# panthuncia/BasicRenderer

Measured on AMD Instinct MI355X. Metric: shaded Mpixels/s @4K (vis-buffer+resolve), higher is better.
Workload: dtype f32; 1 GPU; bistro-class procedural frame, 3840x2160, 1 directional + 256 point lights, 22669824 instanced tris, 2017 instances (2614016 in 150 meshes), LOD DAGs from the library's cluster-LOD builder, relief slope 1.5; pixels_per_gpu=8294400, visible_clusters_rank0=10118, occlusion_culling=True, visible_clusters_phase2_rank0=0, meshlets_tested_rank0=26713, partition=single GPU, frames_in_flight=3

## Files before the change

basicrenderer_amd/csrc/brmi_api.hip:

```cpp
#include <hip/hip_runtime.h>

#include <algorithm>
#include <cmath>
#include <cstdarg>
#include <cstddef>
#include <cstdio>
#include <cstdlib>
#include <cstring>

#include "brmi_device.h"
#include "brmi_internal.h"

namespace brmi {

__global__ void k_debug_arith(const float* a, const float* b, float* outDiv, float* outSqrt, uint32_t* outHalf, uint32_t n) {
    const uint32_t i = blockIdx.x * blockDim.x + threadIdx.x;
    if (i >= n) return;
    outDiv[i] = a[i] / b[i];
    outSqrt[i] = sqrtf(fabsf(a[i]));
    outHalf[i] = f32_to_f16_bits(a[i]);
}

__global__ void k_debug_arith_in_range(const float* a, float* outRcp, float* outSqrt, float* outNorm, uint32_t n) {
    const uint32_t i = blockIdx.x * blockDim.x + threadIdx.x;
// ... 81 lines not shown
    w.pageTotal = take(16);
    w.lightHitMasks = take((uint64_t)p->numLightClusters * ((std::max(1u, p->scene.lightCount) + 63u) / 64u) * 8);
    p->binsX = (c.width + 255) / 256; p->binsY = (c.height + 15) / 16;
    w.binCounts = take((uint64_t)p->binsX * p->binsY * 4 * BRMI_BIN_COUNT_STRIDE);
    w.binRecords = take((uint64_t)p->binsX * p->binsY * p->binCapacity * 64);
    w.binOverflow = take((uint64_t)CNT_STRIPE_COUNT * p->binOverflowPerStripe * 64);
    p->binItemCapacity = p->binsX * p->binsY * std::max(1u, (p->binCapacity + 31u) / 32u > 256u ? 256u : (p->binCapacity + 31u) / 32u);
    p->binItemCapacity = std::min<uint32_t>(p->binItemCapacity, 1u << 22);
    p->binScratchTiles = (uint32_t)std::max(0l, tuning("bin_scratch_tiles", p->binScratchTiles));
    w.binPlan = take((uint64_t)(16 + 3 * p->binsX * p->binsY) * 4);
    w.binItems = take((uint64_t)p->binItemCapacity * 4);
    w.binScratch = take((uint64_t)std::max(1u, p->binScratchTiles) * 4096 * 8);
    w.clusterSetup = take((uint64_t)c.maxVisibleClusters * sizeof(ClusterSetup));
    p->resolveCapacity = (uint32_t)std::min<uint64_t>((uint64_t)c.maxVisibleClusters, 1ull << 20) * BRMI_MESHLET_MAX_TRIS;
    if (const long v = tuning("resolve_capacity", 0)) p->resolveCapacity = (uint32_t)std::max(1l, v);
    w.resolveVerts = take((uint64_t)p->resolveCapacity * sizeof(ResolveVertex));
    w.resolveTris = take((uint64_t)p->resolveCapacity * sizeof(ResolveTriangle));
    w.shadeTables = take(((uint64_t)2 * c.width + 2 * c.height + 64) * 4);
    w.matWords = take((uint64_t)std::max(1u, p->scene.materialCount) * sizeof(MaterialWords));
    w.layerUniform = take(sizeof(LayerUniform));
    w.frameConst = take(4 * 64);
    w.frameSnapshot = take(sizeof(FrameSnapshot));
    w.matConst = take((uint64_t)std::max(1u, p->scene.openpbrMaterialCount) * sizeof(MatConst));
    w.objConst = take((uint64_t)std::max(1u, p->scene.perObjectCount) * OBJ_CONST_FLOATS * 4);
    p->deferredStripeCapacity = (uint32_t)((((c.dynamicBand ? p->paddedPixels : p->bandPixelCount) / 4096 + CNT_STRIPE_COUNT) / CNT_STRIPE_COUNT) * 4096);
    w.deferredPixels = take((uint64_t)3 * CNT_STRIPE_COUNT * p->deferredStripeCapacity * 4);
    w.lutF = take((uint64_t)(32768 + 1024 + 1024 + 32 + 256) * 4);
    w.shadeRows = take((uint64_t)std::max(1u, p->scene.openpbrMaterialCount) * 256 * 512);
    w.shadeAvgs = take((uint64_t)std::max(1u, p->scene.openpbrMaterialCount) * 256 * 8);
    w.ggxQuads = take(256 * 48);
    w.shadeLights = take((uint64_t)std::max(1u, p->scene.lightCount) * 64);
    w.clusterList = take((uint64_t)p->numLightClusters * 8);
    w.listEntries = take((uint64_t)p->lightPagePool * BRMI_LIGHTS_PER_PAGE * 4 + 256);
    w.listRecords = take((uint64_t)p->lightPagePool * BRMI_LIGHTS_PER_PAGE * 64 + 4096);
    const bool uvs = p->tables.hasTextures || p->tables.hasAlphaTest || p->tables.hasVertexColors;
    w.clusterUv = take(uvs ? (uint64_t)c.maxVisibleClusters * 32 : 16);
    w.resolveColors = take(p->tables.hasVertexColors ? (uint64_t)p->resolveCapacity * 4 : 16);
    w.resolveUVs = take(p->tables.hasTextures ? (uint64_t)p->resolveCapacity * 8 * p->tables.uvSets : 16);
    w.binAlpha = take(p->tables.hasAlphaTest ? (uint64_t)p->binsX * p->binsY * p->binCapacity * 48 : 16);
    w.overflowAlpha = take(p->tables.hasAlphaTest ? (uint64_t)CNT_STRIPE_COUNT * p->binOverflowPerStripe * 48 : 16);
    w.alphaMats = take(p->tables.hasAlphaTest ? (uint64_t)std::max(1u, p->scene.materialCount) * 128 : 16);
    w.meshletBoxes = take((uint64_t)std::max(1u, p->tables.totalBoxes) * sizeof(MeshletBox));
    w.pageBoxBase = take((uint64_t)std::max<size_t>(1, p->tables.pageBoxBase.size()) * 4);
    w.pageRefs = take((uint64_t)std::max<size_t>(1, p->tables.pageRefs.size()) * sizeof(PageRef));
    w.drawList = take(p->holdEnabled ? (uint64_t)c.maxVisibleClusters * 4 : 16);
    w.generalList = take(p->leanMinClusters != 0u ? (uint64_t)c.maxVisibleClusters * 4 : 16);
    w.bigQueue = take(p->leanMinClusters != 0u ? (uint64_t)p->leanQueue * 96 : 16);
    w.bigRuns = take(p->leanMinClusters != 0u ? (uint64_t)p->leanQueue * 8 : 16);
    w.heldRecords = take(p->holdEnabled ? (uint64_t)c.maxVisibleClusters * sizeof(HeldRecord) : 16);
    w.lateList = take(p->holdEnabled ? (uint64_t)c.maxVisibleClusters * 4 : 16);
    w.wideQueue = take((uint64_t)std::max(1u, p->wideCapacity) * 96);
    w.wideAlpha = take(p->tables.hasAlphaTest ? (uint64_t)std::max(1u, p->wideCapacity) * 48 : 16);
    w.total = off;
    p->resNeed[BRMI_RES_WORKSPACE] = w.total;
}

template <typename T>
static int read_back(brmi_pass* p, std::vector<T>& dst, const T* src, size_t n) {
    dst.resize(n);
    if (n == 0) return BRMI_OK;
    if (!src) return fail(p, BRMI_ERR_INVALID, "scene buffer missing");
    BRMI_HIP(p, hipMemcpy(dst.data(), src, n * sizeof(T), hipMemcpyDeviceToHost));
    return BRMI_OK;
}

}

brmi::HzbDesc brmi_pass::hzbDesc() const {
    brmi::HzbDesc d{};
    d.depth = static_cast<const float*>(res[BRMI_RES_LINEAR_DEPTH]); d.mips = static_cast<float*>(res[BRMI_RES_HZB]);
    d.width = cfg.width; d.height = cfg.height; d.tilesX = tilesX; d.mipCount = hzbMipCount; d.rowLo = bandY0; d.rowHi = bandY1; d.stripes = stripes;
    d.paddedW = hzbMipCount ? hzbMipW[0] : 1; d.paddedH = hzbMipCount ? hzbMipH[0] : 1;
    for (uint32_t i = 0; i < brmi::kMaxHzbMips; i++) d.mipOffset[i] = i < hzbMipCount ? (uint32_t)hzbMipOffsets[i] : 0u;
    return d;
}

using namespace brmi;

extern "C" {

uint32_t brmi_abi_version(void) { return BRMI_ABI_VERSION; }
uint32_t brmi_abi_minor(void) { return BRMI_ABI_MINOR; }

void brmi_default_config(brmi_config* cfg, uint32_t width, uint32_t height) {
    if (!cfg) return;
    std::memset(cfg, 0, sizeof(*cfg));
    cfg->structSize = sizeof(brmi_config);
    cfg->width = width; cfg->height = height;
    cfg->maxVisibleClusters = 1u << 22;
    cfg->maxTraversalRecords = 1u << 22;
    cfg->enableOcclusionCulling = 0;
    cfg->enableClusteredLighting = 1;
    cfg->enablePunctualLights = 1;
    cfg->lightClusterSize[0] = 12; cfg->lightClusterSize[1] = 12; cfg->lightClusterSize[2] = 24;
    cfg->phase2ExpansionFactor = 2;
    cfg->collectPassStatistics = 0;
    cfg->maxBvhLevels = 64;
    cfg->keepUniformLayerPlanes = 0;
}

}
namespace brmi {
static bool tuning_lookup(const char* key, long* out) {
    const char* e = std::getenv("BRMI_TUNING");
    if (!e) return false;
    const size_t n = std::strlen(key);
    for (const char* q = e; *q; ) {
        while (*q == ',' || *q == ' ') q++;
        const char* end = std::strchr(q, ',');
        const size_t len = end ? (size_t)(end - q) : std::strlen(q);
        if (len > n && std::strncmp(q, key, n) == 0 && q[n] == '=') { *out = std::strtol(q + n + 1, nullptr, 0); return true; }
        q += len;
    }
    return false;
}
long tuning(const char* key, long def) { long v; return tuning_lookup(key, &v) ? v : def; }
}
extern "C" {

int brmi_create(const brmi_config* cfg, brmi_pass** out) {
    if (!cfg || !out || cfg->structSize != sizeof(brmi_config) || cfg->width == 0 || cfg->height == 0) return BRMI_ERR_INVALID;
    if (cfg->maxVisibleClusters == 0 || cfg->maxVisibleClusters > (1u << 25) - 1u || cfg->maxTraversalRecords == 0) return BRMI_ERR_INVALID;
    if (cfg->lightClusterSize[0] == 0 || cfg->lightClusterSize[1] == 0 || cfg->lightClusterSize[2] == 0) return BRMI_ERR_INVALID;
    if (cfg->lightClusterSize[2] > 62u) return BRMI_ERR_INVALID;
    if ((uint64_t)((cfg->width + 255u) / 256u) * ((cfg->height + 15u) / 16u) > 65535ull) return BRMI_ERR_INVALID;
    if (cfg->stripeCount > 1u) {
        if (cfg->stripeRows == 0u || cfg->stripeRows % 16u || cfg->stripeIndex >= cfg->stripeCount || cfg->bandY0 != 0u || (cfg->bandY1 != 0u && cfg->bandY1 != cfg->height)) return BRMI_ERR_INVALID;
        if (cfg->fullHeight == 0u || cfg->fullHeight % (cfg->stripeRows * cfg->stripeCount) || cfg->height != cfg->fullHeight / cfg->stripeCount) return BRMI_ERR_INVALID;
        if (cfg->dynamicBand) return BRMI_ERR_INVALID;
    }
    if (cfg->dynamicBand && (cfg->bandY0 % 8u || (cfg->bandY1 % 8u && cfg->bandY1 < cfg->height))) return BRMI_ERR_INVALID;
    brmi_pass* p = new brmi_pass();
    p->cfg = *cfg;
    p->totalWords = 1; p->scanBlocks = 1;
    p->forceLevelKernels = tuning("cull_level_kernels", 0) != 0;
    p->packedFlat = tuning("flat_packed", 1) != 0;
    p->flatLevelsMinDraws = (uint32_t)std::max(0l, tuning("flat_levels_min_draws", p->flatLevelsMinDraws));
    p->phase2DirectMax = (uint32_t)std::max(0l, tuning("phase2_direct_max", p->phase2DirectMax));
    p->resolveInlineMode = (int)tuning("resolve_inline", -1);
    p->wideCapacity = (uint32_t)std::min(1l << 20, std::max(0l, tuning("wide_capacity", p->wideCapacity)));
    p->wideMinTriangles = (uint32_t)std::max(0l, tuning("wide_min_triangles", p->wideMinTriangles));
    p->leanMinClusters = (uint32_t)std::max(0l, tuning("lean_min_clusters", p->leanMinClusters));
    if (p->leanMinClusters > cfg->maxVisibleClusters) p->leanMinClusters = 0u;
    p->leanMaxGeneralPct = (uint32_t)std::max(0l, std::min(100l, tuning("lean_max_general_pct", p->leanMaxGeneralPct)));
    p->leanGrid = (uint32_t)std::max(64l, tuning("lean_grid", p->leanGrid));
    p->leanQueue = (uint32_t)std::max(64l, std::min(1l << 24, tuning("lean_queue", p->leanQueue))) & ~63u;
    p->leanWideEntries = (uint32_t)std::max(1l, tuning("lean_wide_entries", p->leanWideEntries));
    p->leanEmitGrid = (uint32_t)std::max(64l, std::min(65536l, tuning("lean_emit_grid", p->leanEmitGrid))) & ~63u;
    p->wideEntries = (uint32_t)std::max(1l, tuning("wide_entries", p->wideEntries));
    p->binMinSlice = (uint32_t)std::max(32l, tuning("bin_min_slice", p->binMinSlice));
    p->binSharedSlice = (uint32_t)std::max(32l, tuning("bin_shared_slice", p->binSharedSlice));
    p->binGrid = (uint32_t)std::min(65535l, std::max(1l, tuning("bin_grid", p->binGrid)));
    p->binOverflowPerStripe = (uint32_t)std::max(0l, tuning("bin_overflow", p->binOverflowPerStripe));
    p->binCapacity = (uint32_t)std::min(65536l, std::max(1l, tuning("bin_capacity", p->binCapacity)));
    if (const long v = tuning("big_tri_area", 0)) p->bigTriArea = p->bigTriAreaAlpha = p->bigTriAreaDense = (int)std::max(1l, v);
    compute_sizes(p);
    *out = p;
    return BRMI_OK;
}

void brmi_destroy(brmi_pass* p) {
    if (!p) return;
    if (p->eventsCreated) for (int i = 0; i < BRMI_STAGE_COUNT; i++) for (uint32_t k = 0; k < brmi_pass::kEventRing; k++) { (void)hipEventDestroy(p->evStart[i][k]); (void)hipEventDestroy(p->evStop[i][k]); }
    (void)brmi_set_history_source(p, nullptr);
    for (brmi_pass* user : p->historyUsers) user->history = nullptr;
    if (p->chainReady) (void)hipEventDestroy(p->chainReady);
    if (p->geometryDone) (void)hipEventDestroy(p->geometryDone);
    if (p->cullDone) (void)hipEventDestroy(p->cullDone);
    if (p->frameDone) (void)hipEventDestroy(p->frameDone);
    if (p->phase2FeedbackHost) (void)hipHostFree(p->phase2FeedbackHost);
    delete p;
}

const char* brmi_last_error(const brmi_pass* p) { return p ? p->err.c_str() : "null pass"; }

int brmi_set_scene(brmi_pass* p, const brmi_scene_buffers* scene) {
    if (!p || !scene) return BRMI_ERR_INVALID;
    p->scene = *scene; p->haveScene = false; p->setupDone = false;
    p->streaming.on = false;
    p->samplerAniso = nullptr;
    const brmi_scene_buffers& sc = p->scene;
    if (!sc.slabs || !sc.perObject || !sc.perMesh || !sc.perMeshInstance || !sc.clodOffsets || !sc.meshMetadata || !sc.lodNodes || !sc.lodGroups ||
        !sc.lodSegments || !sc.groupPageMap || !sc.materials || !sc.openpbrMaterials || !sc.cameras || !sc.cullingCameras || !sc.viewRasterInfo || !sc.perFrame ||
        !sc.normalMatrices || (sc.activeDrawCount && !sc.activeDraws) || (sc.lightCount && (!sc.lights || !sc.activeLightIndices)))
        return fail(p, BRMI_ERR_INVALID, "brmi_set_scene: a required scene buffer is null");
    if (!sc.lutOpaqueDielectricEnergyComplement || !sc.lutOpaqueDielectricAvgEnergyComplement || !sc.lutIdealMetalEnergyComplement || !sc.lutIdealMetalAvgEnergyComplement || !sc.lutFuzzLTC)
        return fail(p, BRMI_ERR_INVALID, "brmi_set_scene: OpenPBR lookup tables must be provided");
    HostScene hs; int rc;
    if ((rc = read_back(p, hs.meshMetadata, sc.meshMetadata, sc.meshMetadataCount))) return rc;
    if ((rc = read_back(p, hs.clodOffsets, sc.clodOffsets, sc.perMeshInstanceCount))) return rc;
    if ((rc = read_back(p, hs.lodNodes, sc.lodNodes, sc.lodNodeCount))) return rc;
    if ((rc = read_back(p, hs.lodSegments, sc.lodSegments, sc.lodSegmentCount))) return rc;
    if ((rc = read_back(p, hs.openpbrMaterials, sc.openpbrMaterials, sc.openpbrMaterialCount))) return rc;
    if ((rc = read_back(p, hs.materials, sc.materials, sc.materialCount))) return rc;
    if ((rc = read_back(p, hs.perMesh, sc.perMesh, sc.perMeshCount))) return rc;
    if ((rc = read_back(p, hs.perMeshInstance, sc.perMeshInstance, sc.perMeshInstanceCount))) return rc;
    if ((rc = read_back(p, hs.activeDraws, sc.activeDraws, sc.activeDrawCount))) return rc;
    if ((rc = read_back(p, hs.groupPageMap, sc.groupPageMap, sc.groupPageMapCount))) return rc;
    if ((rc = read_back(p, hs.lodGroups, sc.lodGroups, sc.lodGroupCount))) return rc;
    if ((rc = read_back(p, hs.slabs, sc.slabs, sc.slabCount))) return rc;
    hs.perObjectCount = sc.perObjectCount; hs.skinningMatrixCount = sc.skinningMatrixCount;
    hs.textureTables = sc.textures && sc.samplers && sc.srgbToLinear && sc.textureCount != 0 && sc.samplerCount != 0;
    const bool flatOn = tuning("flat_traversal", 1) != 0;
    const bool boxesOn = tuning("hold_clusters", 1) != 0 && p->cfg.enableOcclusionCulling && sc.slabCount <= 4096u;
    const auto pageMeshlets = [&](uint32_t slab, uint32_t byteOffset, uint32_t* meshlets) -> int { BRMI_HIP(p, hipMemcpy(meshlets, hs.slabs[slab] + byteOffset, 4, hipMemcpyDeviceToHost)); return BRMI_OK; };
    if ((rc = analyse_scene(hs, flatOn, p->cfg.maxBvhLevels, boxesOn, pageMeshlets, p->tables, p->err))) return rc;
    p->holdEnabled = boxesOn && p->tables.totalBoxes != 0u && p->stripes.count <= 1u;
    p->holdMinClusters = (uint32_t)std::max(0l, tuning("hold_min_clusters", p->holdMinClusters));
    p->lateDirectMax = (uint32_t)std::max(0l, tuning("late_direct_max", p->lateDirectMax));
    p->holdStillMax = (uint32_t)std::max(0l, tuning("hold_still_max", p->holdStillMax));
    p->holdFloor = (uint32_t)std::max(0l, tuning("hold_floor", p->holdFloor));
    p->holdMaxTexels = (uint32_t)std::min(16l, std::max(1l, tuning("hold_max_texels", p->holdMaxTexels)));
    p->retestMaxTexels = (uint32_t)std::min(16l, std::max(1l, tuning("retest_max_texels", p->retestMaxTexels)));
    p->totalWords = (uint32_t)std::max<uint64_t>(1, (p->tables.totalBits + 31) / 32);
    p->scanBlocks = (p->totalWords + 2047u) / 2048u;
    p->maxLevels = std::min(std::max(1u, p->tables.maxDepth), std::max(1u, p->cfg.maxBvhLevels));
    compute_sizes(p);
    p->haveScene = true;
    p->updateSerial++;
    return BRMI_OK;
}

int brmi_set_band(brmi_pass* p, uint32_t bandY0, uint32_t bandY1) {
    if (!p) return BRMI_ERR_INVALID;
    if (!p->cfg.dynamicBand) return fail(p, BRMI_ERR_STATE, "brmi_set_band: the pass was created without brmi_config::dynamicBand");
    if (bandY1 > p->cfg.height) bandY1 = p->cfg.height;
    if (bandY0 % 8u || (bandY1 % 8u && bandY1 != p->cfg.height) || bandY0 >= bandY1) return fail(p, BRMI_ERR_INVALID, "brmi_set_band: rows [%u, %u) -- multiples of 8 inside the frame's %u rows", bandY0, bandY1, p->cfg.height);
    p->bandY0 = bandY0; p->bandY1 = bandY1;
    const uint32_t t0 = bandY0 / 8u, t1 = (bandY1 + 7u) / 8u;
    p->bandFirstPixel = (uint64_t)t0 * p->tilesX * 64; p->bandPixelCount = (uint64_t)(t1 - t0) * p->tilesX * 64;
    p->updated = false;
    return BRMI_OK;
}

int brmi_declare(brmi_pass* p, brmi_declare_cb cb, void* user) {
    if (!p || !cb) return BRMI_ERR_INVALID;
    if (!p->haveScene) return fail(p, BRMI_ERR_STATE, "brmi_declare: call brmi_set_scene first (workspace size depends on the scene)");
    for (uint32_t i = 0; i < BRMI_RES_COUNT; i++) {
        brmi_resource_desc d{};
        d.id = i; d.name = kResNames[i]; d.bytes = p->resNeed[i];
        const bool image = i <= BRMI_RES_HDR_COLOR;
        d.usage = BRMI_USAGE_UNORDERED_ACCESS | BRMI_USAGE_SHADER_RESOURCE | ((i == BRMI_RES_WORKSPACE || i == BRMI_RES_HZB) ? BRMI_USAGE_INTERNAL : 0u);
        d.width = image ? p->cfg.width : 0; d.height = image ? p->cfg.height : 0; d.bytesPerPixel = kResBpp[i];
        d.tileW = image ? 8 : 0; d.tileH = image ? 8 : 0;
        cb(user, &d);
    }
    return BRMI_OK;
}

int brmi_setup(brmi_pass* p, const brmi_resource_binding* b, uint32_t n, brmi_stream stream) {
    if (!p || (!b && n)) return BRMI_ERR_INVALID;
    if (!p->haveScene) return fail(p, BRMI_ERR_STATE, "brmi_setup: call brmi_set_scene first");
    hipStream_t s = static_cast<hipStream_t>(stream);
    for (uint32_t i = 0; i < n; i++) {
        if (b[i].id >= BRMI_RES_COUNT) return fail(p, BRMI_ERR_INVALID, "brmi_setup: unknown resource id %u", b[i].id);
        p->res[b[i].id] = b[i].ptr; p->resBytes[b[i].id] = b[i].bytes;
    }
    for (uint32_t i = 0; i < BRMI_RES_COUNT; i++) {
        if (!p->res[i]) return fail(p, BRMI_ERR_INVALID, "brmi_setup: resource %s not bound", kResNames[i]);
        if (p->resBytes[i] < p->resNeed[i]) return fail(p, BRMI_ERR_CAPACITY, "brmi_setup: resource %s is %llu B, needs %llu B", kResNames[i], (unsigned long long)p->resBytes[i], (unsigned long long)p->resNeed[i]);
        if ((reinterpret_cast<uintptr_t>(p->res[i]) & 15u) != 0) return fail(p, BRMI_ERR_INVALID, "brmi_setup: resource %s must be 16-byte aligned", kResNames[i]);
    }
    BRMI_HIP(p, hipMemsetAsync(p->res[BRMI_RES_WORKSPACE], 0, p->ws.total, s));
    if (p->cfg.enableOcclusionCulling && p->resNeed[BRMI_RES_HZB] >= 4) BRMI_HIP(p, hipMemsetD32Async(reinterpret_cast<hipDeviceptr_t>(p->res[BRMI_RES_HZB]), (int)BRMI_DEPTH_EMPTY_BITS, p->resNeed[BRMI_RES_HZB] / 4, s));
    p->hzbValid = false;
    if (!p->tables.instanceBitBase.empty()) BRMI_HIP(p, hipMemcpyAsync(p->wsPtr<uint32_t>(p->ws.instanceBitBase), p->tables.instanceBitBase.data(), p->tables.instanceBitBase.size() * 4, hipMemcpyHostToDevice, s));
    if (!p->tables.segPrefix.empty()) BRMI_HIP(p, hipMemcpyAsync(p->wsPtr<uint32_t>(p->ws.segPrefix), p->tables.segPrefix.data(), p->tables.segPrefix.size() * 4, hipMemcpyHostToDevice, s));
    if (!p->tables.meshLevelWidth.empty()) BRMI_HIP(p, hipMemcpyAsync(p->wsPtr<uint32_t>(p->ws.meshLevelWidth), p->tables.meshLevelWidth.data(), p->tables.meshLevelWidth.size() * 4, hipMemcpyHostToDevice, s));
    if (!p->tables.flatNodes.empty()) BRMI_HIP(p, hipMemcpyAsync(p->wsPtr<FlatNode>(p->ws.flatNodes), p->tables.flatNodes.data(), p->tables.flatNodes.size() * sizeof(FlatNode), hipMemcpyHostToDevice, s));
    if (!p->tables.flatLeaves.empty()) BRMI_HIP(p, hipMemcpyAsync(p->wsPtr<FlatLeaf>(p->ws.flatLeaves), p->tables.flatLeaves.data(), p->tables.flatLeaves.size() * sizeof(FlatLeaf), hipMemcpyHostToDevice, s));
    if (!p->tables.instanceWalk.empty()) BRMI_HIP(p, hipMemcpyAsync(p->wsPtr<InstanceWalk>(p->ws.instanceWalk), p->tables.instanceWalk.data(), p->tables.instanceWalk.size() * sizeof(InstanceWalk), hipMemcpyHostToDevice, s));
    if (!p->tables.pageBoxBase.empty()) BRMI_HIP(p, hipMemcpyAsync(p->wsPtr<uint32_t>(p->ws.pageBoxBase), p->tables.pageBoxBase.data(), p->tables.pageBoxBase.size() * 4, hipMemcpyHostToDevice, s));
    if (!p->tables.pageRefs.empty()) BRMI_HIP(p, hipMemcpyAsync(p->wsPtr<PageRef>(p->ws.pageRefs), p->tables.pageRefs.data(), p->tables.pageRefs.size() * sizeof(PageRef), hipMemcpyHostToDevice, s));
    { int rc = launch_expand_luts(p, s); if (rc) return rc; }
    { int rc = launch_meshlet_boxes(p, s); if (rc) return rc; }
    BRMI_HIP(p, hipStreamSynchronize(s));
    if (p->cfg.collectPassStatistics && !p->eventsCreated) {
        for (int i = 0; i < BRMI_STAGE_COUNT; i++) for (uint32_t k = 0; k < brmi_pass::kEventRing; k++) { BRMI_HIP(p, hipEventCreate(&p->evStart[i][k])); BRMI_HIP(p, hipEventCreate(&p->evStop[i][k])); }
        p->eventsCreated = true;
    }
    p->setupDone = true;
    p->layerPlanesDirty = true;
    p->constantsSerial = 0;
    return BRMI_OK;
}

int brmi_update(brmi_pass* p, const brmi_frame_update* u, brmi_stream stream) {
    if (!p || !u || !u->mainCameraHost || !u->perFrameHost) return BRMI_ERR_INVALID;
    if (!p->setupDone) return fail(p, BRMI_ERR_STATE, "brmi_update: call brmi_setup first");
    if (p->env.on && u->perFrameHost->activeEnvironmentIndex >= p->env.b.environmentCount)
        return fail(p, BRMI_ERR_INVALID, "brmi_update: perFrame.activeEnvironmentIndex %u, the bound environment table has %u entries", u->perFrameHost->activeEnvironmentIndex, p->env.b.environmentCount);
    p->camHost = *u->mainCameraHost; p->pfHost = *u->perFrameHost;
    const brmi_per_frame& pf = p->pfHost;
    if (pf.lightClusterGridSizeX != p->cfg.lightClusterSize[0] || pf.lightClusterGridSizeY != p->cfg.lightClusterSize[1] || pf.lightClusterGridSizeZ != p->cfg.lightClusterSize[2])
        return fail(p, BRMI_ERR_INVALID, "brmi_update: per-frame light cluster grid differs from the configured lightClusterSize");
    if (pf.screenResX != p->cfg.width || pf.screenResY != p->frameHeight()) return fail(p, BRMI_ERR_INVALID, "brmi_update: per-frame screen size differs from the configured target size");
    const float zNear = p->camHost.zNear, zFar = p->camHost.zFar, zSplit = pf.clusterZSplitDepth;
    const uint32_t gz = pf.lightClusterGridSizeZ, nearSlices = pf.nearClusterCount;
    p->planesHost.resize(2 * gz);
    for (uint32_t sliceZ = 0; sliceZ < gz; sliceZ++) {
        float pn, pfar;
        if (sliceZ < nearSlices) {
            const float sliceSize = (zSplit - zNear) / (float)nearSlices;
            pn = -(zNear + (float)sliceZ * sliceSize);
            pfar = -(zNear + (float)(sliceZ + 1) * sliceSize);
        } else {
// ... 112 lines not shown
    if ((!e->environments && e->environmentCount) || (!e->cubemaps && e->cubemapCount)) return brmi::fail(p, BRMI_ERR_INVALID, "brmi_set_environment: a null table with a non-zero count");
    if (e->environmentCount == 0u || !e->environments) return brmi::fail(p, BRMI_ERR_INVALID, "brmi_set_environment: environmentCount is 0 (NULL unbinds)");
    if (p->updated && p->pfHost.activeEnvironmentIndex >= e->environmentCount)
        return brmi::fail(p, BRMI_ERR_INVALID, "brmi_set_environment: the last brmi_update's activeEnvironmentIndex is %u, the table has %u entries", p->pfHost.activeEnvironmentIndex, e->environmentCount);
    p->env.b = environment_struct_of(e); p->env.on = true;
    p->updateSerial++;
    return BRMI_OK;
}
static int skybox_refusal(brmi_pass* p) {
    if (!p->setupDone) return brmi::fail(p, BRMI_ERR_STATE, "brmi_skybox: call brmi_setup first");
    if (!p->updated) return brmi::fail(p, BRMI_ERR_STATE, "brmi_skybox: call brmi_update first (the environment is perFrame.activeEnvironmentIndex of the last update)");
    if (!p->env.on || !p->env.b.skybox) return brmi::fail(p, BRMI_ERR_STATE, "brmi_skybox: no environment with `skybox` set is bound (brmi_set_environment)");
    if (!p->res[BRMI_RES_LINEAR_DEPTH] || !p->res[BRMI_RES_HDR_COLOR] || !p->res[BRMI_RES_GBUF_MOTION_VECTORS]) return brmi::fail(p, BRMI_ERR_STATE, "brmi_skybox: the depth, HDR or motion-vector surface is not bound");
    return BRMI_OK;
}
int brmi_skybox(brmi_pass* p, brmi_stream stream) {
    if (!p) return BRMI_ERR_INVALID;
    if (int rc = skybox_refusal(p)) return rc;
    return brmi::launch_skybox(p, static_cast<hipStream_t>(stream));
}

static bool env_size_ok(uint32_t size) { return size != 0u && size <= 16384u; }
int brmi_env_convert(const brmi_texture_desc* equirect, const brmi_texture_desc* cube, uint32_t size, uint32_t cubeFormat, brmi_stream stream) {
    if (!equirect || !cube || !env_size_ok(size) || cubeFormat != BRMI_TEXTURE_FORMAT_RGBA16_FLOAT) return BRMI_ERR_INVALID;
    return brmi::launch_env_convert(equirect, cube, size, static_cast<hipStream_t>(stream));
}
int brmi_env_project_sh(const brmi_texture_desc* cubemaps, uint32_t cubemapCount, brmi_environment_info* environments, uint32_t environmentCount, uint32_t environmentIndex, uint32_t size, brmi_stream stream) {
    if (!cubemaps || cubemapCount == 0u || !environments || environmentIndex >= environmentCount || !env_size_ok(size)) return BRMI_ERR_INVALID;
    return brmi::launch_env_project_sh(cubemaps, cubemapCount, environments + environmentIndex, size, static_cast<hipStream_t>(stream));
}
int brmi_env_prefilter(const brmi_texture_desc* sourceCube, const brmi_texture_desc* prefiltered, uint32_t size, uint32_t levels, uint32_t prefilteredFormat, brmi_stream stream) {
    if (!sourceCube || !prefiltered || !env_size_ok(size) || levels == 0u || levels > BRMI_TEXTURE_MAX_MIPS || prefilteredFormat != BRMI_TEXTURE_FORMAT_RGBA8_UNORM) return BRMI_ERR_INVALID;
    return brmi::launch_env_prefilter(sourceCube, prefiltered, size, levels, static_cast<hipStream_t>(stream));
}
uint64_t brmi_env_build_bytes(uint32_t size, uint32_t levels, uint64_t* cubeBytes, uint64_t* prefilteredBytes) {
    if (cubeBytes) *cubeBytes = 0; if (prefilteredBytes) *prefilteredBytes = 0;
    if (!env_size_ok(size) || levels == 0u || levels > BRMI_TEXTURE_MAX_MIPS) return 0;
    const uint64_t cube = 6ull * size * size * 8ull;
    uint64_t chain = 0;
    for (uint32_t m = 0; m < levels; m++) { const uint64_t s = std::max(1u, size >> m); chain += s * s; }
    chain *= 6ull * 4ull;
    if (cubeBytes) *cubeBytes = cube; if (prefilteredBytes) *prefilteredBytes = chain;
    return cube + chain;
}
int brmi_debug_env_lookup(const brmi_texture_desc* cubemaps, uint32_t cubemapCount, uint32_t cubemapIndex, const float* directions, const float* lods, float* outRGBA, uint32_t n, brmi_stream stream) {
    if (!cubemaps || !directions || !lods || !outRGBA) return BRMI_ERR_INVALID;
    if (n == 0u) return BRMI_OK;
    return brmi::launch_debug_env_lookup(cubemaps, cubemapCount, cubemapIndex, directions, lods, outRGBA, n, static_cast<hipStream_t>(stream));
}
int brmi_streaming_feedback(brmi_pass* p, brmi_stream stream) {
    CHECK_READY(p);
    if (!p->streaming.on) return brmi::fail(p, BRMI_ERR_STATE, "brmi_streaming_feedback: no streaming buffers bound (brmi_set_streaming)");
    return brmi::launch_streaming_feedback(p, static_cast<hipStream_t>(stream));
}
uint64_t brmi_debug_view_bytes(uint32_t width, uint32_t height) { return (uint64_t)((width + 7u) / 8u) * ((height + 7u) / 8u) * 64u * 8u; }
int brmi_set_debug_view(brmi_pass* p, const brmi_debug_view_buffers* b) {
    if (!p) return BRMI_ERR_INVALID;
    if (!b) { p->debugView.on = false; return BRMI_OK; }
    if (b->structSize != sizeof(brmi_debug_view_buffers)) return brmi::fail(p, BRMI_ERR_INVALID, "brmi_set_debug_view: structSize %u, expected %zu", b->structSize, sizeof(brmi_debug_view_buffers));
    if (p->stripes.count > 1u) return brmi::fail(p, BRMI_ERR_INVALID, "brmi_set_debug_view: not with the interleaved partition (stripeCount %u): the compact surfaces' pixel rows are not the frame's", p->stripes.count);
    if (!b->payload) return brmi::fail(p, BRMI_ERR_INVALID, "brmi_set_debug_view: the payload pointer is null");
    if (reinterpret_cast<uintptr_t>(b->payload) & 15u) return brmi::fail(p, BRMI_ERR_INVALID, "brmi_set_debug_view: the payload must be 16 B aligned");
    const uint64_t need = brmi_debug_view_bytes(p->cfg.width, p->cfg.height), needImage = (uint64_t)p->cfg.width * p->cfg.height * 4u;
    if (b->payloadBytes < need) return brmi::fail(p, BRMI_ERR_INVALID, "brmi_set_debug_view: the payload holds %llu bytes, %u x %u pixels need %llu", (unsigned long long)b->payloadBytes, p->cfg.width, p->cfg.height, (unsigned long long)need);
    if (b->image && ((reinterpret_cast<uintptr_t>(b->image) & 3u) || b->imageBytes < needImage))
        return brmi::fail(p, BRMI_ERR_INVALID, "brmi_set_debug_view: the image holds %llu bytes (4 B aligned), %u x %u pixels need %llu", (unsigned long long)b->imageBytes, p->cfg.width, p->cfg.height, (unsigned long long)needImage);
    p->debugView.b = *b; p->debugView.on = true;
    return BRMI_OK;
}
static int debug_view_refusal(brmi_pass* p) {
    const uint32_t mode = p->pfHost.outputType;
    if (!brmi::debug_view_mode_built(mode)) return brmi::fail(p, BRMI_ERR_INVALID, "brmi_debug_view: outputType %u is not a debug view of this path (brmi_output_type lists the ones it builds)", mode);
    if ((mode == BRMI_OUTPUT_LIGHT_CLUSTER_ID || mode == BRMI_OUTPUT_LIGHT_CLUSTER_LIGHT_COUNT) && !p->cfg.enableClusteredLighting)
        return brmi::fail(p, BRMI_ERR_INVALID, "brmi_debug_view: outputType %u needs enableClusteredLighting", mode);
    if (!p->debugView.on) return brmi::fail(p, BRMI_ERR_STATE, "brmi_debug_view: no debug target bound (brmi_set_debug_view)");
    if (p->stripes.count > 1u) return brmi::fail(p, BRMI_ERR_INVALID, "brmi_debug_view: not with the interleaved partition");
    return BRMI_OK;
}
int brmi_debug_view(brmi_pass* p, brmi_stream stream) {
    if (!p) return BRMI_ERR_INVALID;
    if (!p->setupDone) return brmi::fail(p, BRMI_ERR_STATE, "brmi_debug_view: call brmi_setup first");
    if (!p->updated) return brmi::fail(p, BRMI_ERR_STATE, "brmi_debug_view: call brmi_update first (the view is perFrame.outputType of the last update)");
    if (p->pfHost.outputType == BRMI_OUTPUT_COLOR) return BRMI_OK;
    if (int rc = debug_view_refusal(p)) return rc;
    return brmi::launch_debug_view(p, static_cast<hipStream_t>(stream));
}
int brmi_build_hzb(brmi_pass* p, brmi_stream stream) {
    CHECK_READY(p); hipStream_t s = static_cast<hipStream_t>(stream);
    if (!p->cfg.enableOcclusionCulling) return brmi::fail(p, BRMI_ERR_STATE, "brmi_build_hzb: the pass was created without enableOcclusionCulling");
    STAGE_BEGIN(p, BRMI_STAGE_HZB, s); int rc = launch_hzb(p, s, false, false); STAGE_END(p, BRMI_STAGE_HZB, s);
    if (rc == BRMI_OK) p->hzbValid = true;
    return rc;
}
static int build_hzb_fused(brmi_pass* p, hipStream_t s, bool fromVisibility, bool onlyIfPhase2Drew) {
    STAGE_BEGIN(p, BRMI_STAGE_HZB, s); int rc = launch_hzb(p, s, fromVisibility, onlyIfPhase2Drew); STAGE_END(p, BRMI_STAGE_HZB, s);
    if (rc == BRMI_OK) p->hzbValid = true;
    return rc;
}
int brmi_invalidate_hzb(brmi_pass* p) {
    if (!p) return BRMI_ERR_INVALID;
    p->hzbValid = false;
    if (p->history) p->history->hzbValid = false;
    return BRMI_OK;
}
int brmi_set_history_source(brmi_pass* p, brmi_pass* source) {
    if (!p) return BRMI_ERR_INVALID;
    if (source == p) source = nullptr;
    if (source) {
        if (!p->setupDone || !source->setupDone) return brmi::fail(p, BRMI_ERR_STATE, "brmi_set_history_source: both passes need brmi_setup first");
        if (!p->cfg.enableOcclusionCulling || !source->cfg.enableOcclusionCulling) return brmi::fail(p, BRMI_ERR_STATE, "brmi_set_history_source: both passes need enableOcclusionCulling (there is no history otherwise)");
        if (p->cfg.width != source->cfg.width || p->cfg.height != source->cfg.height || ((p->bandY0 != source->bandY0 || p->bandY1 != source->bandY1) && !(p->cfg.dynamicBand && source->cfg.dynamicBand)))
            return brmi::fail(p, BRMI_ERR_INVALID, "brmi_set_history_source: the passes differ in size or band (%ux%u rows %u-%u against %ux%u rows %u-%u)", p->cfg.width, p->cfg.height, p->bandY0, p->bandY1,
                              source->cfg.width, source->cfg.height, source->bandY0, source->bandY1);
    }
    if (p->history) { auto& u = p->history->historyUsers; u.erase(std::remove(u.begin(), u.end(), p), u.end()); }
    p->history = source;
    if (source) source->historyUsers.push_back(p);
    return BRMI_OK;
}
int brmi_gbuffer(brmi_pass* p, brmi_stream stream) {
    CHECK_READY(p); hipStream_t s = static_cast<hipStream_t>(stream);
    STAGE_BEGIN(p, BRMI_STAGE_GBUFFER, s); int rc = launch_gbuffer(p, s); STAGE_END(p, BRMI_STAGE_GBUFFER, s); return rc;
}
int brmi_light_clustering(brmi_pass* p, brmi_stream stream) {
    CHECK_READY(p); hipStream_t s = static_cast<hipStream_t>(stream);
    STAGE_BEGIN(p, BRMI_STAGE_LIGHT_CLUSTER, s); int rc = launch_light_clustering(p, s); STAGE_END(p, BRMI_STAGE_LIGHT_CLUSTER, s); return rc;
}
int brmi_set_shade_slabs(brmi_pass* p, uint32_t slabs, brmi_slab_fn fn, void* user) {
    if (!p) return BRMI_ERR_INVALID;
    p->shadeSlabs = (fn && slabs > 1u) ? slabs : 0u; p->shadeSlabFn = p->shadeSlabs ? fn : nullptr; p->shadeSlabUser = p->shadeSlabs ? user : nullptr;
    return BRMI_OK;
}
int brmi_shade(brmi_pass* p, brmi_stream stream) {
    CHECK_READY(p); hipStream_t s = static_cast<hipStream_t>(stream);
    STAGE_BEGIN(p, BRMI_STAGE_SHADE, s); int rc = launch_shade(p, s); STAGE_END(p, BRMI_STAGE_SHADE, s); return rc;
}

int brmi_execute(brmi_pass* p, brmi_stream stream) { return brmi_execute_split(p, stream, stream); }

int brmi_execute_split(brmi_pass* p, brmi_stream stream, brmi_stream shadeStream) {
    CHECK_READY(p);
    int rc;
    const bool debugView = p->debugView.on && p->pfHost.outputType != BRMI_OUTPUT_COLOR;
    if (debugView && (rc = debug_view_refusal(p))) return rc;
    const bool skybox = p->env.on && p->env.b.skybox;
    if (skybox && (rc = skybox_refusal(p))) return rc;
    p->executesSinceTimes++;
    const bool split = shadeStream != stream;
    p->splitFrame = split;
    struct FrameScope { brmi_pass* p; ~FrameScope() { p->splitFrame = false; p->shadeSharesChip = false; p->frameWaitsIssued = false; p->clearFrameStateWithConstants = false; p->fuseFrameClear = false; p->seedInHzbTail = false; } } frameScope{p};
    p->resolveSetupDone = false; p->depthFinal = false;
    if ((rc = wait_for_frames_in_flight(p, stream))) return rc;
    p->frameWaitsIssued = true;
    const bool rides = p->constantsSerial != p->updateSerial && p->tables.minLevelWidth <= 1024u  && !p->forceLevelKernels && p->scene.activeDrawCount != 0u;
    p->lightGridDone = false;
    const bool sideRiders = rides && split && (p->bandPixelCount & 1ull) == 0ull;
    if (sideRiders) {
        p->clearFrameStateWithConstants = true; p->clearVisibilityWithClusterCull = true;
        rc = brmi_cull(p, 1, stream);
        p->clearFrameStateWithConstants = false;
        if (rc == BRMI_OK && p->clearVisibilityWithClusterCull) { p->clearVisibilityWithClusterCull = false; return brmi::fail(p, BRMI_ERR_STATE, "brmi_execute: the cluster culling did not carry the visibility clear"); }
        if (rc) { p->clearVisibilityWithClusterCull = false; return rc; }
    } else if (rides) {
        p->clearFrameStateWithConstants = true; p->clearVisibilityWithTraversal = true;
        rc = brmi_cull(p, 1, stream);
        p->clearFrameStateWithConstants = false;
        if (rc == BRMI_OK && p->clearVisibilityWithTraversal) { p->clearVisibilityWithTraversal = false; return brmi::fail(p, BRMI_ERR_STATE, "brmi_execute: the traversal did not carry the visibility clear"); }
        if (rc) { p->clearVisibilityWithTraversal = false; return rc; }
    } else {
    p->fuseFrameClear = true;
    rc = brmi_clear_visibility(p, stream);
    p->fuseFrameClear = false;
    if (rc) return rc;
    if ((rc = brmi_cull(p, 1, stream))) return rc;
    }
    if (split) {
        if (!p->cullDone) BRMI_HIP(p, hipEventCreateWithFlags(&p->cullDone, hipEventDisableTiming));
        BRMI_HIP(p, hipEventRecord(p->cullDone, static_cast<hipStream_t>(stream)));
        BRMI_HIP(p, hipStreamWaitEvent(static_cast<hipStream_t>(shadeStream), p->cullDone, 0));
        if (sideRiders) { if ((rc = brmi::launch_light_clustering(p, static_cast<hipStream_t>(shadeStream)))) return rc; p->lightGridDone = true; }
        if ((rc = launch_resolve_setup(p, static_cast<hipStream_t>(shadeStream), 1u))) return rc;
    }
    if ((rc = brmi_raster(p, 1, stream))) return rc;
    if (p->cfg.enableOcclusionCulling) {
        p->seedInHzbTail = true;
        rc = build_hzb_fused(p, static_cast<hipStream_t>(stream), true, false);
        p->seedInHzbTail = false;
        if (rc) return rc;
        if ((rc = brmi_cull(p, 2, stream))) return rc;
        if ((rc = brmi_raster(p, 2, stream))) return rc;
        if ((rc = build_hzb_fused(p, static_cast<hipStream_t>(stream), true, true))) return rc;
        if (!p->chainReady) BRMI_HIP(p, hipEventCreateWithFlags(&p->chainReady, hipEventDisableTiming));
        BRMI_HIP(p, hipEventRecord(p->chainReady, static_cast<hipStream_t>(stream)));
        p->chainRecorded = true; p->chainStream = stream;
    }
    if (p->streaming.on && (rc = brmi_streaming_feedback(p, stream))) return rc;
    if (split) {
        if ((rc = launch_resolve_setup(p, static_cast<hipStream_t>(stream), 2u))) return rc;
        p->resolveSetupDone = true;
        if (!p->geometryDone) BRMI_HIP(p, hipEventCreateWithFlags(&p->geometryDone, hipEventDisableTiming));
        if (!p->frameDone) BRMI_HIP(p, hipEventCreateWithFlags(&p->frameDone, hipEventDisableTiming));
        BRMI_HIP(p, hipEventRecord(p->geometryDone, static_cast<hipStream_t>(stream)));
        BRMI_HIP(p, hipStreamWaitEvent(static_cast<hipStream_t>(shadeStream), p->geometryDone, 0));
        stream = shadeStream;
    }
    const bool lightsDone = p->lightGridDone;
    p->lightGridDone = false;
    p->depthFinal = p->cfg.enableOcclusionCulling != 0;
    p->shadeSharesChip = split;
    rc = brmi_gbuffer(p, stream);
    p->shadeSharesChip = false;
    p->depthFinal = false;
    if (rc) return rc;
    if (!lightsDone && (rc = brmi_light_clustering(p, stream))) return rc;
    p->shadeSharesChip = split;
    rc = brmi_shade(p, stream);
    p->shadeSharesChip = false;
    if (rc) return rc;
    if (skybox && (rc = brmi_skybox(p, stream))) return rc;
    if (debugView && (rc = brmi_debug_view(p, stream))) return rc;
    if (split) { BRMI_HIP(p, hipEventRecord(p->frameDone, static_cast<hipStream_t>(stream))); p->frameDoneRecorded = true; }
    p->splitFrame = false;
    return BRMI_OK;
}

int brmi_read_counters(brmi_pass* p, brmi_counters* out, brmi_stream stream) {
    if (!p || !out) return BRMI_ERR_INVALID;
    if (!p->setupDone) return brmi::fail(p, BRMI_ERR_STATE, "brmi_read_counters: setup not done");
    hipStream_t s = static_cast<hipStream_t>(stream);
    uint32_t c[CNT_WORDS];
    BRMI_HIP(p, hipMemcpyAsync(c, p->counters(), sizeof(c), hipMemcpyDeviceToHost, s));
    BRMI_HIP(p, hipStreamSynchronize(s));
    std::memset(out, 0, sizeof(*out));
    out->instancesTested = c[CNT_INSTANCES_TESTED]; out->instancesVisible = c[CNT_INSTANCES_VISIBLE];
    out->nodesVisited = c[CNT_NODES_VISITED];
    uint32_t overflowQueued = 0;
    for (uint32_t st = 0; st < CNT_STRIPE_COUNT; st++) {
        const uint32_t* sp = c + CNT_STRIPES + st * CNT_STRIPE_WORDS;
        out->instancesTested += sp[0]; out->instancesVisible += sp[1]; out->nodesVisited += sp[2];
        overflowQueued += sp[STRIPE_OVERFLOW];
    } out->bucketRecords = c[CNT_BUCKETS]; out->meshletsTested = c[CNT_MESHLETS_TESTED];
    for (uint32_t st = 0; st < CNT_STRIPE_COUNT; st++) out->meshletsTested += c[CNT_STRIPES + st * CNT_STRIPE_WORDS + STRIPE_MESHLETS_TESTED];
    out->visibleClusters = c[CNT_VISIBLE]; out->visibleClustersPhase2 = c[CNT_VISIBLE2];
    out->droppedRecords = c[CNT_DROPPED_RECORDS]; out->droppedClusters = c[CNT_DROPPED_CLUSTERS]; out->lightPagesUsed = c[CNT_LIGHT_PAGES];
    out->reserved[0] = c[CNT_SUM_VERTS_LO]; out->reserved[2] = c[CNT_SUM_VERTS_HI];
    out->reserved[1] = std::min(c[CNT_HELD1], p->cfg.maxVisibleClusters); out->reserved[3] = std::min(c[CNT_LATE1], p->cfg.maxVisibleClusters);
    out->reserved[4] = c[CNT_RASTER_CLUSTERS]; out->reserved[5] = c[CNT_BIN_OVERFLOW] + overflowQueued;
    out->replayNodes = c[CNT_REPLAY_NODES]; out->replayMeshlets = c[CNT_REPLAY_MESHLETS];
    return BRMI_OK;
}

int brmi_set_timed_stages(brmi_pass* p, uint32_t stageMask) {
    if (!p) return BRMI_ERR_INVALID;
    p->timedStages = stageMask;
    return BRMI_OK;
}

int brmi_stage_times(brmi_pass* p, float* ms) {
    if (!p || !ms) return BRMI_ERR_INVALID;
    if (!p->eventsCreated) return brmi::fail(p, BRMI_ERR_STATE, "brmi_stage_times: collectPassStatistics is off");
    for (int i = 0; i < BRMI_STAGE_COUNT; i++) {
        ms[i] = 0.0f;
        const uint32_t perFrame = (i == BRMI_STAGE_HZB && p->executesSinceTimes != 0u && p->evCount[i] == 2u * p->executesSinceTimes) ? 2u : 1u;
        uint32_t n = std::min(p->evCount[i], brmi_pass::kEventRing);
        n -= n % perFrame;
        if (n == 0) continue;
        double sum = 0.0;
        for (uint32_t k = 0; k < n; k++) {
            const uint32_t slot = (p->evCount[i] - 1 - k) % brmi_pass::kEventRing;
            float t = 0.0f;
            BRMI_HIP(p, hipEventSynchronize(p->evStop[i][slot]));
            BRMI_HIP(p, hipEventElapsedTime(&t, p->evStart[i][slot], p->evStop[i][slot]));
            sum += t;
        }
        ms[i] = (float)(sum / (n / perFrame));
        p->evCount[i] = 0;
    }
    p->executesSinceTimes = 0;
    return BRMI_OK;
}

int brmi_algorithmic_bytes(brmi_pass* p, uint64_t* perStage, uint64_t* total) {
    if (!p || !perStage || !total) return BRMI_ERR_INVALID;
    BRMI_HIP(p, hipDeviceSynchronize());
    brmi_counters c; int rc = brmi_read_counters(p, &c, nullptr); if (rc) return rc;
    const uint64_t P = (uint64_t)p->cfg.width * (p->bandY1 - p->bandY0);
    uint64_t sumV = c.reserved[0], sumT = c.reserved[2], nClusters = c.reserved[4];
    if (c.reserved[1] != 0u) {
        uint32_t vt[2];
        BRMI_HIP(p, hipMemcpy(vt, p->counters() + CNT_DRAWN_VT, 8, hipMemcpyDeviceToHost));
        sumV = vt[0]; sumT = vt[1]; nClusters -= c.reserved[1] - c.reserved[3];
    }
    for (int i = 0; i < BRMI_STAGE_COUNT; i++) perStage[i] = 0;
    perStage[BRMI_STAGE_CLEAR] = 8 * P;
    perStage[BRMI_STAGE_CULL] = 64ull * c.meshletsTested + 16ull * (c.visibleClusters + c.visibleClustersPhase2) + 64ull * c.nodesVisited;
    perStage[BRMI_STAGE_RASTER] = 8 * P + 144ull * nClusters + 12ull * sumV + 3ull * sumT;
    if (p->cfg.enableOcclusionCulling) {
        perStage[BRMI_STAGE_DEPTH_COPY] = 12 * P;
        perStage[BRMI_STAGE_HZB] = 2 * (4 * P + 4 * P / 3);
    }
    perStage[BRMI_STAGE_GBUFFER] = (8 + 52 + 4) * P;
    perStage[BRMI_STAGE_SHADE] = (4 + 48 + 8) * P;
    *total = 0; for (int i = 0; i < BRMI_STAGE_COUNT; i++) *total += perStage[i];
    return BRMI_OK;
}

int brmi_algorithmic_bytes_launched(brmi_pass* p, uint64_t* perStage, uint64_t* total) {
    if (int rc = brmi_algorithmic_bytes(p, perStage, total)) return rc;
    if (!p->tables.hasCoat && !p->tables.hasFuzz) {
        const uint64_t P = (uint64_t)p->cfg.width * (p->bandY1 - p->bandY0);
        *total -= perStage[BRMI_STAGE_SHADE]; perStage[BRMI_STAGE_SHADE] = 44ull * P; *total += perStage[BRMI_STAGE_SHADE];
    }
    return BRMI_OK;
}

int brmi_debug_read_held(brmi_pass* p, uint32_t* held, uint32_t heldCapacity, uint32_t* heldCount, uint32_t* late, uint32_t lateCapacity, uint32_t* lateCount) {
    if (!p || !heldCount || !lateCount || !p->setupDone) return BRMI_ERR_INVALID;
    BRMI_HIP(p, hipDeviceSynchronize());
    uint32_t nh = 0, nl = 0;
    BRMI_HIP(p, hipMemcpy(&nh, p->counters() + CNT_HELD1, 4, hipMemcpyDeviceToHost));
    BRMI_HIP(p, hipMemcpy(&nl, p->counters() + CNT_LATE1, 4, hipMemcpyDeviceToHost));
// ... 91 lines not shown
```

basicrenderer_amd/csrc/brmi_cull.hip:

```cpp
#include <type_traits>
#include "brmi_device.h"
#include "brmi_internal.h"
#include "brmi_lightgrid.h"
#include "brmi_texture.h"

namespace brmi {

struct CullArgs {
    brmi_scene_buffers sc;
    uint32_t* counters;
    const uint32_t* instanceBitBase;
    const uint32_t* segPrefix;
    uint32_t recordCapacity, visibleCapacity, factor, phase;
    uint32_t occlusion;
    uint32_t frontier0Counter, bucketCounter;
    NodeRecord* replayNodes; BucketRecord* replayBuckets;
    HzbDesc hzb;
    uint32_t bandActive; float bandTop[3], bandBottom[3];
    const float4* bandPlanes;
    StripeMap stripes;
    const uint32_t* meshLevelWidth; uint32_t levelKernelsWidthLo;
    const FlatNode* flatNodes; const FlatLeaf* flatLeaves; const InstanceWalk* instanceWalk;
    uint32_t* feedback;
    uint32_t wideFlat;
// ... 53 lines not shown
BRMI_DEV bool flat_refined_child_holds(const FlatNode& fn, const FlatLeaf& fl, const m4& model, float scale, f3 camPos, float zNear, float threshold, bool ortho) {
    if (!((fn.info >> 1) & 1u)) return false;
    const f3 cc = xyz(mul_point(f3{fl.child[0], fl.child[1], fl.child[2]}, model));
    const float ce = projected_error(cc, fl.child[3] * scale, fl.childParentError, scale, camPos, zNear, ortho);
    return !(ce < threshold);
}
template <typename Residency>
BRMI_DEV bool flat_leaf_cut(const Residency& res, const FlatNode& fn, const FlatLeaf& fl, const m4& model, float scale, f3 camPos, float zNear, float threshold, bool ortho) {
    if (!(flat_leaf_eod(fn, fl, model, scale, camPos, zNear, ortho) >= threshold)) return false;
    if (flat_refined_child_holds(fn, fl, model, scale, camPos, zNear, threshold, ortho) && res.resident(fl.childGlobal)) return false;
    return res.resident(fl.ownerGlobal);
}
BRMI_DEV void flat_leaf_touch(const StreamArgs& st, const FlatNode& fn, const FlatLeaf& fl, uint32_t instIndex, const m4& model, float scale, f3 camPos, float zNear, float threshold, bool ortho) {
    const float eod = flat_leaf_eod(fn, fl, model, scale, camPos, zNear, ortho);
    if (!(eod >= threshold)) return;
    st.touch(fl.ownerGlobal, instIndex, eod);
    if (flat_refined_child_holds(fn, fl, model, scale, camPos, zNear, threshold, ortho)) st.touch(fl.childGlobal, instIndex, eod);
}

BRMI_DEV uint32_t ceil_log2_clamped(float x, uint32_t maxMip) {
    if (!(x > 1.0f)) return 0u;
    const uint32_t u = __float_as_uint(x);
    const uint32_t m = ((u >> 23) & 0xFFu) - 127u + ((u & 0x7FFFFFu) ? 1u : 0u);
    return m < maxMip ? m : maxMip;
}

BRMI_DEV float hzb_load(const HzbDesc& h, uint32_t mip, uint32_t x, uint32_t y, uint32_t mipW) {
    if (mip == 0u) return (x < h.width && y >= h.rowLo && y < h.rowHi) ? h.depth[tiled_index(x, y, h.tilesX)] : __uint_as_float(BRMI_DEPTH_EMPTY_BITS);
    return h.mips[h.mipOffset[mip] + (size_t)y * mipW + x];
}

BRMI_DEV bool occlusion_culled(const HzbDesc& hzb, const brmi_camera* cam, float p00, float p11, f3 centerVS, float sphereDepth, float radius) {
    const float viewW = (float)cam->depthResX, viewH = (float)cam->depthResY;
    const float px = centerVS.x, py = -centerVS.y, pz = centerVS.z;
    const float rad2 = radius * radius, d = pz * radius;
    const float hv = sqrtf(px * px + pz * pz - rad2);
    const float ha = px * hv, hb = px * radius, hc = pz * hv;
    float L = (ha - d) * p00 / (hc + hb);
    float R = (ha + d) * p00 / (hc - hb);
    const float vv = sqrtf(py * py + pz * pz - rad2);
    const float va = py * vv, vb = py * radius, vc = pz * vv;
    const float B = (va - d) * p11 / (vc + vb);
    const float T = (va + d) * p11 / (vc - vb);
    L = -L; R = -R;
    const float u0 = sat(L * 0.5f + 0.5f), v0 = sat(T * -0.5f + 0.5f), u1 = sat(R * 0.5f + 0.5f), v1 = sat(B * -0.5f + 0.5f);
    const float ax0 = u0 * viewW, ay0 = v0 * viewH, ax1 = u1 * viewW, ay1 = v1 * viewH;
    const float ex = ax1 - ax0, ey = ay1 - ay0;
    const uint32_t mip = ceil_log2_clamped(max2(ex, ey), cam->numDepthMips - 1u);
    const float sx = cam->UVScaleToNextPowerOf2[0], sy = cam->UVScaleToNextPowerOf2[1];
    const float pu0 = u0 * sx, pv0 = v0 * sy, pu1 = u1 * sx, pv1 = v1 * sy;
    const float ssx = max2(sx, 1e-6f), ssy = max2(sy, 1e-6f);
    uint32_t hzbW = (uint32_t)rintf(viewW / ssx), hzbH = (uint32_t)rintf(viewH / ssy);
    hzbW = max(hzbW, 1u); hzbH = max(hzbH, 1u);
    const uint32_t mw = max(hzbW >> mip, 1u), mh = max(hzbH >> mip, 1u);
    uint32_t x0 = min((uint32_t)floorf(pu0 * (float)mw), mw - 1u), y0 = min((uint32_t)floorf(pv0 * (float)mh), mh - 1u);
    uint32_t x1 = min((uint32_t)floorf(pu1 * (float)mw), mw - 1u), y1 = min((uint32_t)floorf(pv1 * (float)mh), mh - 1u);
    if (stripe_on(hzb.stripes)) {
        const uint32_t H = hzb.stripes.fullHeight;
        const uint32_t r0 = min((uint32_t)floorf(ay0), H - 1u), r1 = min((uint32_t)floorf(ay1), H - 1u);
        const uint32_t f = stripe_first_owned(hzb.stripes, r0), l = stripe_last_owned(hzb.stripes, r1);
        if (l == 0xFFFFFFFFu || f > l) return false;
        const uint32_t vy0 = stripe_vrow(hzb.stripes, f), vy1 = stripe_vrow(hzb.stripes, l);
        const uint32_t smip = ceil_log2_clamped(max2(fabsf(ex) + 1.0f, (float)(vy1 - vy0 + 1u)), hzb.mipCount - 1u);
        const uint32_t smw = max(hzb.paddedW >> smip, 1u), smh = max(hzb.paddedH >> smip, 1u);
        const uint32_t px0 = min((uint32_t)floorf(min2(ax0, ax1)), hzb.width - 1u), px1 = min((uint32_t)floorf(max2(ax0, ax1)), hzb.width - 1u);
        x0 = min(px0 >> smip, smw - 1u); x1 = min(px1 >> smip, smw - 1u); y0 = min(vy0 >> smip, smh - 1u); y1 = min(vy1 >> smip, smh - 1u);
        const float e0 = hzb_load(hzb, smip, x0, y0, smw), e1 = hzb_load(hzb, smip, x1, y0, smw), e2 = hzb_load(hzb, smip, x1, y1, smw), e3 = hzb_load(hzb, smip, x0, y1, smw);
        return max2(max2(e0, e1), max2(e2, e3)) < sphereDepth - radius;
    }
    if (mip >= hzb.mipCount) return false;
    const float d0 = hzb_load(hzb, mip, x0, y0, mw), d1 = hzb_load(hzb, mip, x1, y0, mw), d2 = hzb_load(hzb, mip, x1, y1, mw), d3 = hzb_load(hzb, mip, x0, y1, mw);
    const float mx = max2(max2(d0, d1), max2(d2, d3));
    return mx < sphereDepth - radius;
}

BRMI_DEV bool occlusion_test(const CullArgs& a, const brmi_camera* cam, bool replay, f3 localCenter, float localRadius, f3 currentVS, float currentRadius,
                             const brmi_per_object* obj) {
    if (replay) return occlusion_culled(a.hzb, cam, cam->projection[0][0], cam->projection[1][1], currentVS, -currentVS.z, currentRadius);
    const m4 prevModel = load_m4(&obj->prevModel[0][0]);
    const f3 pc = to_view_space(localCenter, prevModel, load_m4(&cam->prevView[0][0]));
    return occlusion_culled(a.hzb, cam, cam->prevUnjitteredProjection[0][0], cam->prevUnjitteredProjection[1][1], pc, -pc.z, localRadius * max_axis_scale(prevModel));
}

BRMI_DEV bool occlusion_test_prev(const CullArgs& a, const brmi_camera* cam, f3 localCenter, float localRadius, const m4& prevModel) {
    const f3 pc = to_view_space(localCenter, prevModel, load_m4(&cam->prevView[0][0]));
    return occlusion_culled(a.hzb, cam, cam->prevUnjitteredProjection[0][0], cam->prevUnjitteredProjection[1][1], pc, -pc.z, localRadius * max_axis_scale(prevModel));
}

BRMI_DEV void flat_internal_verdict(const CullArgs& a, const brmi_camera* cam, const FlatNode& fn, f3 cullC, float cullR, const m4& model, const m4& prevModel, float scale,
                                    f3 camPos, float zNear, float threshold, bool ortho, bool& pre, bool& hidden, bool& expand) {
    const f3 lc = xyz(mul_point(f3{fn.lod[0], fn.lod[1], fn.lod[2]}, model));
    const float e = projected_error(lc, fn.lod[3] * scale, fn.maxQuadricError, scale, camPos, zNear, ortho);
    pre = e >= threshold;
    if (pre) { hidden = a.occlusion && occlusion_test_prev(a, cam, cullC, cullR, prevModel); expand = !hidden; }
}

BRMI_DEV bool stripe_rejects(const StripeMap& m, const brmi_camera* cam, f3 centerVS, float radius) {
    const float pz = centerVS.z;
    if (!(-pz - radius > cam->zNear)) return false;
    const float py = -centerVS.y, p11 = cam->projection[1][1];
    const float rad2 = radius * radius, d = pz * radius;
    const float vv = sqrtf(py * py + pz * pz - rad2);
    const float va = py * vv, vb = py * radius, vc = pz * vv;
    const float B = (va - d) * p11 / (vc + vb), T = (va + d) * p11 / (vc - vb);
    const float v0 = sat(T * -0.5f + 0.5f), v1 = sat(B * -0.5f + 0.5f);
    if (!(v0 <= v1)) return false;
    const float H = (float)m.fullHeight;
    const int r0 = max(to_int_sat(floorf(v0 * H)) - 2, 0), r1 = min(to_int_sat(floorf(v1 * H)) + 2, (int)m.fullHeight - 1);
    return stripe_first_owned(m, (uint32_t)r0) > (uint32_t)r1;
}

BRMI_DEV bool sphere_culled(const CullArgs& a, const brmi_camera* cam, f3 c, float r) {
    if (sphere_outside_frustum(c, r, cam->clippingPlanes)) return true;
    if (a.bandActive) {
        const float4 top = a.bandPlanes[0], bottom = a.bandPlanes[1];
        if ((top.x * c.x + top.y * c.y) + top.z * c.z < -r || (bottom.x * c.x + bottom.y * c.y) + bottom.z * c.z < -r) return true;
    }
    return stripe_on(a.stripes) && stripe_rejects(a.stripes, cam, c, r);
}

__global__ void __launch_bounds__(256) k_cull_instances(CullArgs a, NodeRecord* frontier0) {
    const brmi_scene_buffers& sc = a.sc;
    const uint32_t viewId = sc.perFrame->mainCameraIndex;
    const brmi_camera* cam = sc.cameras + viewId;
    const m4 view = load_m4(&cam->view[0][0]);
    for (uint32_t d = blockIdx.x * blockDim.x + threadIdx.x; d < ((sc.activeDrawCount + 63u) & ~63u); d += gridDim.x * blockDim.x) {
        bool visible = false;
        uint32_t ii = 0, root = 0;
        if (d < sc.activeDrawCount && (a.levelKernelsWidthLo == 0u || a.meshLevelWidth[sc.clodOffsets[sc.activeDraws[d]].clodMeshMetadataIndex] >= a.levelKernelsWidthLo)) {
            ii = sc.activeDraws[d];
            const brmi_per_mesh_instance inst = sc.perMeshInstance[ii];
            const m4 model = load_m4(&sc.perObject[inst.perObjectBufferIndex].model[0][0]);
            const f3 c = to_view_space(f3{inst.boundingSphere[0], inst.boundingSphere[1], inst.boundingSphere[2]}, model, view);
            const float r = inst.boundingSphere[3] * max_axis_scale(model);
            const bool bad = isnan(c.x) || isnan(c.y) || isnan(c.z) || isinf(c.x) || isinf(c.y) || isinf(c.z) || isnan(r) || isinf(r);
            visible = !bad && !sphere_culled(a, cam, c, r);
            root = sc.meshMetadata[sc.clodOffsets[ii].clodMeshMetadataIndex].rootNode;
            atomicAdd(&a.counters[CNT_INSTANCES_TESTED], 1u);
            if (visible) atomicAdd(&a.counters[CNT_INSTANCES_VISIBLE], 1u);
        }
        const uint32_t slot = wave_append(&a.counters[CNT_FRONTIER0], visible);
        if (visible) {
            if (slot < a.recordCapacity) frontier0[slot] = NodeRecord{ii, (1u << 30) | (root & 0x3FFFFFFFu)};
            else atomicAdd(&a.counters[CNT_DROPPED_RECORDS], 1u);
        }
    }
}

#ifndef BRMI_HIER_STAGE_WIDE
#define BRMI_HIER_STAGE_WIDE 128
#endif
constexpr uint32_t HIER_CAP_MAX = 1024;
struct NoSide {};
struct SideJobs { ulonglong2* vis2; uint64_t n2; uint32_t walkBlocks, clearBlocks; ClusterArgs lc; };
constexpr uint32_t FLAT_WIDE_MAX = 8192;
struct LcRide { uint32_t mainBlocks; ClusterArgs lc; };
struct ClearRide { uint32_t mainBlocks; ulonglong2* vis2; uint64_t n2; uint32_t clearBlocks; };

BRMI_DEV float4 skinned_meshlet_bounds(const brmi_scene_buffers& sc, const brmi_meshlet_descriptor* desc, const brmi_page_header* hdr, const uint8_t* page, uint32_t slot, float4 staticBounds) {
    const uint32_t boneCount = desc->boneCount;
    if (slot == 0xFFFFFFFFu || boneCount == 0u || sc.skinningMatrices == nullptr) return staticBounds;
    const uint32_t* boneList = reinterpret_cast<const uint32_t*>(page + hdr->boneIndexStreamOffset + desc->boneListOffset * 4u);
    const f3 c0{staticBounds.x, staticBounds.y, staticBounds.z};
    f3 mc{0.0f, 0.0f, 0.0f}; float mr = 0.0f; bool init = false;
    for (uint32_t b = 0; b < boneCount; b++) {
        const m4 m = load_bone_skin_matrix(sc.skinningMatrices, slot, boneList[b]);
        const f3 tc = xyz(mul_point(c0, m));
        const float tr = staticBounds.w * max_axis_scale(m);
        if (!init) { mc = tc; mr = tr; init = true; continue; }
        const f3 delta = tc - mc;
        const float dist = length3(delta);
        if (dist + tr <= mr) continue;
        if (dist + mr <= tr) { mc = tc; mr = tr; continue; }
        const float newRadius = 0.5f * (dist + mr + tr);
        const float t = (newRadius - mr) / max2(dist, 1e-12f);
        mc = mc + delta * t;
        mr = newRadius;
    }
    if (!init) return staticBounds;
    return make_float4(mc.x, mc.y, mc.z, mr * (1.0f + 1e-5f));
}

template <typename Residency>
__global__ void __launch_bounds__(256) k_traverse(CullArgs a, uint32_t level, const NodeRecord* frontierIn, NodeRecord* frontierOut, BucketRecord* buckets, Residency res) {
    const brmi_scene_buffers& sc = a.sc;
    const uint32_t inputCount = min(a.counters[level == 0 ? a.frontier0Counter : CNT_FRONTIER0 + level], a.recordCapacity);
    const uint32_t viewId = sc.perFrame->mainCameraIndex;
    const brmi_camera* cam = sc.cameras + viewId;
    const brmi_culling_camera* lodCam = sc.cullingCameras + viewId;
    const bool ortho = cam->isOrtho != 0;
    const f3 camPos{lodCam->positionWorldSpace[0], lodCam->positionWorldSpace[1], lodCam->positionWorldSpace[2]};
    const float zNear = lodCam->zNear, threshold = lodCam->errorOverDistanceThreshold;
    const m4 view = load_m4(&cam->view[0][0]);
    uint32_t* nextCount = &a.counters[CNT_FRONTIER0 + level + 1];
    const uint32_t rounded = (inputCount + 63u) & ~63u;
    for (uint32_t idx = blockIdx.x * blockDim.x + threadIdx.x; idx < rounded; idx += gridDim.x * blockDim.x) {
        bool have = idx < inputCount;
        if (have && level == 0u && a.phase == 2u && a.levelKernelsWidthLo != 0u &&
            a.meshLevelWidth[sc.clodOffsets[frontierIn[idx].instanceIndex].clodMeshMetadataIndex] < a.levelKernelsWidthLo) have = false;
        bool isInternal = false, emitLeaf = false, replay = false, occluded = false;
        uint32_t occludedNode = 0;
        uint32_t instIndex = 0, childBase = 0, childCount = 0, lodNodesBase = 0;
        uint32_t segFirst = 0, segCount = 0, ownerGroup = 0, slabDesc = 0, slabOff = 0, firstBit = 0;
        bool skinned = false;
        m4 model{}; float scale = 0.0f;
        f3 instC{0, 0, 0}; float instR = 0.0f;
        if (have) {
            const NodeRecord rec = frontierIn[idx];
            instIndex = rec.instanceIndex;
            replay = (rec.nodeIdPacked >> 31) != 0;
            const bool allowRefine = ((rec.nodeIdPacked >> 30) & 1u) != 0;
            const uint32_t nodeId = rec.nodeIdPacked & 0x3FFFFFFFu;
            const brmi_per_mesh_instance inst = sc.perMeshInstance[instIndex];
            const brmi_clod_mesh_metadata md = sc.meshMetadata[sc.clodOffsets[instIndex].clodMeshMetadataIndex];
            skinned = (sc.perMesh[inst.perMeshBufferIndex].vertexFlags & BRMI_VERTEX_SKINNED) != 0;
            model = load_m4(&sc.perObject[inst.perObjectBufferIndex].model[0][0]);
            scale = max_axis_scale(model);
            instC = f3{inst.boundingSphere[0], inst.boundingSphere[1], inst.boundingSphere[2]}; instR = inst.boundingSphere[3];
            lodNodesBase = md.lodNodesBase;
            const brmi_lod_node node = sc.lodNodes[md.lodNodesBase + nodeId];
            const f3 cullC = skinned ? instC : f3{node.cullCenterAndRadius[0], node.cullCenterAndRadius[1], node.cullCenterAndRadius[2]};
            const float cullR = skinned ? instR : node.cullCenterAndRadius[3];
            const f3 cVS = to_view_space(cullC, model, view);
            const float rW = cullR * scale;
            const bool culled = !replay && sphere_culled(a, cam, cVS, rW);
            if (!culled) {
                if (node.isLeaf != BRMI_NODE_INTERNAL) {
                    if (node_leaf_cut(res, sc, md, node, instIndex, model, scale, camPos, zNear, threshold, ortho, allowRefine)) {
                        const brmi_lod_segment seg = sc.lodSegments[md.segmentsBase + node.indexOrOffset];
                        const brmi_group_page_map_entry pe = sc.groupPageMap[md.pageMapBase + seg.pageIndex];
                        if (seg.meshletCount != 0u && pe.slabDescriptorIndex != 0u) {
                            emitLeaf = true;
                            segFirst = seg.firstMeshletInPage; segCount = seg.meshletCount; ownerGroup = node.ownerGroupId;
                            slabDesc = pe.slabDescriptorIndex; slabOff = pe.slabByteOffset;
                            firstBit = a.instanceBitBase[instIndex] + a.segPrefix[md.segmentsBase + node.indexOrOffset];
                        }
                    }
                } else {
                    const f3 lc = xyz(mul_point(f3{node.lodCenterAndRadius[0], node.lodCenterAndRadius[1], node.lodCenterAndRadius[2]}, model));
                    const float lr = node.lodCenterAndRadius[3] * scale;
                    const float nodeEod = projected_error(lc, lr, node.maxQuadricError, scale, camPos, zNear, ortho);
                    if (allowRefine && (nodeEod >= threshold)) {
                        if (a.occlusion && occlusion_test(a, cam, replay, cullC, cullR, cVS, rW, sc.perObject + inst.perObjectBufferIndex)) {
                            occluded = !replay; occludedNode = nodeId;
                        } else {
                            isInternal = true;
                            childBase = node.indexOrOffset;
                            childCount = min(node.countMinusOne + 1u, BRMI_BVH_MAX_CHILDREN);
                        }
                    }
                }
            }
        }
        {
            const uint64_t hm = __ballot(have);
            if (hm != 0ull && (threadIdx.x & 63u) == 0u) atomicAdd(&a.counters[CNT_STRIPES + (blockIdx.x & (CNT_STRIPE_COUNT - 1u)) * CNT_STRIPE_WORDS + 2u], (uint32_t)__popcll(hm));
        }
        if (a.occlusion && a.phase == 1u) {
            const uint32_t slot = wave_append(&a.counters[CNT_REPLAY_NODES], occluded);
            if (occluded) {
                if (slot < a.recordCapacity) a.replayNodes[slot] = NodeRecord{instIndex, 0x80000000u | (1u << 30) | (occludedNode & 0x3FFFFFFFu)};
                else atomicAdd(&a.counters[CNT_DROPPED_RECORDS], 1u);
            }
        }
        {
            const uint32_t nChunks = emitLeaf ? (segCount + a.factor - 1u) / a.factor : 0u;
            uint32_t waveMax = nChunks;
#pragma unroll
            for (int o = 32; o > 0; o >>= 1) waveMax = max(waveMax, (uint32_t)__shfl_xor((int)waveMax, o));
            for (uint32_t k = 0; k < waveMax; k++) {
                const bool emit = k < nChunks;
                const uint32_t slot = wave_append(&a.counters[a.bucketCounter], emit);
                if (emit) {
                    if (slot < a.recordCapacity) {
                        const uint32_t first = segFirst + k * a.factor;
                        const uint32_t cnt = min(a.factor, segCount - k * a.factor);
                        BucketRecord b;
                        b.instanceIndex = instIndex; b.groupIdPacked = (replay ? 0x80000000u : 0u) | (ownerGroup & 0x7FFFFFFFu);
                        b.meshletIndexAndCount = (cnt << 16) | (first & 0xFFFFu);
                        b.pageSlabDescriptorIndex = slabDesc; b.pageSlabByteOffset = slabOff;
                        b.firstBit = firstBit + k * a.factor; b.pad0 = 0; b.pad1 = 0;
                        buckets[slot] = b;
                    } else atomicAdd(&a.counters[CNT_DROPPED_RECORDS], 1u);
                }
            }
        }
        {
            uint32_t waveMax = isInternal ? childCount : 0u;
#pragma unroll
            for (int o = 32; o > 0; o >>= 1) waveMax = max(waveMax, (uint32_t)__shfl_xor((int)waveMax, o));
            for (uint32_t k = 0; k < waveMax; k++) {
                bool emit = false;
                uint32_t childId = 0;
                if (isInternal && k < childCount) {
                    childId = childBase + k;
                    const brmi_lod_node* ch = sc.lodNodes + (lodNodesBase + childId);
                    const f3 cc = skinned ? instC : f3{ch->cullCenterAndRadius[0], ch->cullCenterAndRadius[1], ch->cullCenterAndRadius[2]};
                    const float cr = skinned ? instR : ch->cullCenterAndRadius[3];
                    const f3 ccVS = to_view_space(cc, model, view);
                    emit = replay || !sphere_culled(a, cam, ccVS, cr * scale);
                    if (emit && ch->isLeaf == BRMI_NODE_INTERNAL) {
                        const f3 wc = xyz(mul_point(f3{ch->lodCenterAndRadius[0], ch->lodCenterAndRadius[1], ch->lodCenterAndRadius[2]}, model));
                        const float e = projected_error(wc, ch->lodCenterAndRadius[3] * scale, ch->maxQuadricError, scale, camPos, zNear, ortho);
                        if (e < threshold) emit = false;
                    }
                }
                const uint32_t slot = wave_append(nextCount, emit);
                if (emit) {
                    if (slot < a.recordCapacity) frontierOut[slot] = NodeRecord{instIndex, (replay ? 0x80000000u : 0u) | (1u << 30) | (childId & 0x3FFFFFFFu)};
                    else atomicAdd(&a.counters[CNT_DROPPED_RECORDS], 1u);
                }
            }
        }
    }
}

template <bool REPLAY, uint32_t HIER_CAP, uint32_t HIER_STAGE, bool SIDE, typename Residency>
__global__ void __launch_bounds__(64) k_cull_hierarchy(CullArgs a, BucketRecord* buckets, const uint32_t* meshLevelWidth, uint32_t widthLo, uint32_t widthHi, uint32_t spillAbove, NodeRecord* spillOut,
                                                       typename std::conditional<SIDE, SideJobs, NoSide>::type sj, Residency res) {
    uint32_t walkBlocks = gridDim.x;
    if constexpr (SIDE) {
        walkBlocks = sj.walkBlocks;
        if (blockIdx.x >= sj.walkBlocks + sj.clearBlocks) { lc_count_wave(sj.lc, blockIdx.x - sj.walkBlocks - sj.clearBlocks, threadIdx.x); return; }
        if (blockIdx.x >= sj.walkBlocks) {
            const uint64_t stride = (uint64_t)sj.clearBlocks * 64u;
            for (uint64_t i = (uint64_t)(blockIdx.x - sj.walkBlocks) * 64u + threadIdx.x; i < sj.n2; i += stride) sj.vis2[i] = make_ulonglong2(BRMI_VIS_EMPTY, BRMI_VIS_EMPTY);
            return;
        }
    }
    __shared__ uint32_t frontier[2][HIER_CAP];
    __shared__ uint32_t counts[2];
    __shared__ uint32_t childOff[65], childFirst[64];
    __shared__ BucketRecord stage[HIER_STAGE];
    const brmi_scene_buffers& sc = a.sc;
    const uint32_t lane = threadIdx.x;
    const uint32_t viewId = sc.perFrame->mainCameraIndex;
    const brmi_camera* cam = sc.cameras + viewId;
    const brmi_culling_camera* lodCam = sc.cullingCameras + viewId;
    const bool ortho = cam->isOrtho != 0;
    const f3 camPos{lodCam->positionWorldSpace[0], lodCam->positionWorldSpace[1], lodCam->positionWorldSpace[2]};
    const float zNear = lodCam->zNear, threshold = lodCam->errorOverDistanceThreshold;
    const m4 view = load_m4(&cam->view[0][0]);
    const uint32_t seeds = REPLAY ? min(a.counters[CNT_REPLAY_NODES], a.recordCapacity) : sc.activeDrawCount;
    uint32_t nTested = 0, nVisible = 0, nNodes = 0;
    uint32_t staged = 0;
    auto flush = [&]() {
        if (staged == 0u) return;
        uint32_t baseSlot = 0;
        if (lane == 0) baseSlot = atomicAdd(&a.counters[a.bucketCounter], staged);
        baseSlot = (uint32_t)__shfl((int)baseSlot, 0);
        __syncthreads();
        for (uint32_t k = lane; k < staged; k += 64u) {
            if (baseSlot + k < a.recordCapacity) buckets[baseSlot + k] = stage[k];
            else atomicAdd(&a.counters[CNT_DROPPED_RECORDS], 1u);
        }
        __syncthreads();
        staged = 0u;
    };
    uint32_t firstSeed = blockIdx.x, seedStride = walkBlocks;
    if (!REPLAY && a.packedFlat) {
        const uint32_t packedWaves = (seeds + 7u) >> 3;
        if (blockIdx.x < packedWaves) {
            const uint32_t g8 = lane & ~7u, j = lane & 7u;
            const uint32_t seed = blockIdx.x * 8u + (lane >> 3);
            const bool haveSeed = seed < seeds;
            const uint32_t instIndex = haveSeed ? sc.activeDraws[seed] : 0u;
            brmi_per_mesh_instance inst{}; InstanceWalk iw{0u, 0u, 0u, 0u};
            if (haveSeed) { inst = sc.perMeshInstance[instIndex]; iw = a.instanceWalk[instIndex]; }
            const bool small = haveSeed && iw.flatCount >= 1u && iw.flatCount <= 8u;
            const brmi_per_object* obj = sc.perObject + (small ? inst.perObjectBufferIndex : 0u);
            const bool mine = small && j < iw.flatCount;
            FlatNode fn{}; FlatLeaf fl{};
            if (mine) { fn = a.flatNodes[iw.flatBase + j]; fl = a.flatLeaves[iw.flatBase + j]; }
            m4 model = load_m4(&obj->model[0][0]);
            m4 prevModel = model;
            if (a.occlusion && mine && ((fn.info & 1u))) prevModel = load_m4(&obj->prevModel[0][0]);
            const float scale = max_axis_scale(model);
            const f3 instC{inst.boundingSphere[0], inst.boundingSphere[1], inst.boundingSphere[2]}; const float instR = inst.boundingSphere[3];
            bool instVisible = false;
            {
                const f3 c = to_view_space(instC, model, view);
                const float r = instR * scale;
                const bool bad = isnan(c.x) || isnan(c.y) || isnan(c.z) || isinf(c.x) || isinf(c.y) || isinf(c.z) || isnan(r) || isinf(r);
                instVisible = small && !bad && !sphere_culled(a, cam, c, r);
            }
            nTested += (uint32_t)__popcll(__ballot(small && j == 0u)); nVisible += (uint32_t)__popcll(__ballot(instVisible && j == 0u));
            const bool skinned = iw.skinned != 0u;
            const bool internal = (fn.info & 1u);
            const f3 cullC = skinned ? instC : f3{fn.cull[0], fn.cull[1], fn.cull[2]};
            const float cullR = skinned ? instR : fn.cull[3];
            const f3 cVS = to_view_space(cullC, model, view);
            const float rW = cullR * scale;
            const bool inFrustum = mine && instVisible && !sphere_culled(a, cam, cVS, rW);
            bool pre = inFrustum, expand = false, hidden = false, leafOk = false;
            uint32_t slabDesc = 0, slabOff = 0;
            if (inFrustum && internal) flat_internal_verdict(a, cam, fn, cullC, cullR, model, prevModel, scale, camPos, zNear, threshold, ortho, pre, hidden, expand);
            else if (inFrustum && flat_leaf_cut(res, fn, fl, model, scale, camPos, zNear, threshold, ortho) && ((fn.info >> 2) & 1u)) {
                const brmi_group_page_map_entry pe = sc.groupPageMap[fn.pageMapIndex];
                slabDesc = pe.slabDescriptorIndex; slabOff = pe.slabByteOffset;
                leafOk = slabDesc != 0u;
            }
            const uint64_t expandM = __ballot(expand);
            const uint32_t parentLane = g8 | ((fn.info >> 8) & 7u);
            uint64_t reached = __ballot(mine && instVisible && j == 0u);
            for (;;) {
                const bool r = mine && instVisible && (j == 0u || (pre && ((reached >> parentLane) & 1ull) && ((expandM >> parentLane) & 1ull)));
                const uint64_t next = __ballot(r);
                if (next == reached) break;
                reached = next;
            }
            const bool here = (reached >> lane) & 1ull;
            nNodes += here ? 1u : 0u;
            if constexpr (Residency::kTracks) { if (here && inFrustum && !internal) flat_leaf_touch(res, fn, fl, instIndex, model, scale, camPos, zNear, threshold, ortho); }
            const bool replayIt = a.occlusion && here && hidden;
            const uint64_t replayM = __ballot(replayIt);
            const bool emitLeaf = here && leafOk;
            const uint32_t segFirst = fn.segFirstCount & 0xFFFFu, segCount = fn.segFirstCount >> 16;
            const uint32_t nChunks = emitLeaf ? (segCount + a.factor - 1u) / a.factor : 0u;
            uint32_t incl = nChunks;
#pragma unroll
            for (int o = 1; o < 64; o <<= 1) { const uint32_t v = (uint32_t)__shfl_up((int)incl, o); if (lane >= (uint32_t)o) incl += v; }
            const uint32_t nBuckets = (uint32_t)__shfl((int)incl, 63), nReplay = (uint32_t)__popcll(replayM);
            uint32_t replayBase = 0, bucketBase = 0;
            if (lane == 0) {
                if (nReplay != 0u) replayBase = atomicAdd(&a.counters[CNT_REPLAY_NODES], nReplay);
                if (nBuckets != 0u) bucketBase = atomicAdd(&a.counters[a.bucketCounter], nBuckets);
            }
            replayBase = (uint32_t)__shfl((int)replayBase, 0); bucketBase = (uint32_t)__shfl((int)bucketBase, 0);
            if (replayIt) {
                const uint32_t slot = replayBase + (uint32_t)__popcll(replayM & ((1ull << lane) - 1ull));
                if (slot < a.recordCapacity) a.replayNodes[slot] = NodeRecord{instIndex, 0x80000000u | (1u << 30) | (fn.nodeId & 0x3FFFFFFFu)};
                else atomicAdd(&a.counters[CNT_DROPPED_RECORDS], 1u);
            }
            for (uint32_t k = 0; k < nChunks; k++) {
                const uint32_t slot = bucketBase + (incl - nChunks) + k;
                if (slot >= a.recordCapacity) { atomicAdd(&a.counters[CNT_DROPPED_RECORDS], 1u); continue; }
                BucketRecord b;
                b.instanceIndex = instIndex; b.groupIdPacked = fn.ownerGroup & 0x7FFFFFFFu;
                b.meshletIndexAndCount = (min(a.factor, segCount - k * a.factor) << 16) | ((segFirst + k * a.factor) & 0xFFFFu);
                b.pageSlabDescriptorIndex = slabDesc; b.pageSlabByteOffset = slabOff;
                b.firstBit = iw.bitBase + fn.firstBitRel + k * a.factor; b.pad0 = 0; b.pad1 = 0;
                buckets[slot] = b;
            }
            firstSeed = seeds;
        } else { firstSeed = blockIdx.x - packedWaves; seedStride = walkBlocks - packedWaves; }
    }
    for (uint32_t seed = firstSeed; seed < seeds; seed += seedStride) {
        uint32_t instIndex, startNode;
        if (REPLAY) { const NodeRecord rec = a.replayNodes[seed]; instIndex = rec.instanceIndex; startNode = rec.nodeIdPacked & 0x3FFFFFFFu; }
        else instIndex = sc.activeDraws[seed];
        const brmi_per_mesh_instance inst = sc.perMeshInstance[instIndex];
        if (!REPLAY) {
            const InstanceWalk iw = a.instanceWalk[instIndex];
            if (a.packedFlat && iw.flatCount >= 1u && iw.flatCount <= 8u) continue;
            if (iw.flatCount > 256u && a.wideFlat) continue;
            if (iw.flatCount != 0u && iw.flatCount <= 256u) {
                constexpr uint32_t FLAT_CHUNKS = 4;
                const uint32_t chunks = (iw.flatCount + 63u) >> 6;
                const brmi_per_object* obj = sc.perObject + inst.perObjectBufferIndex;
                uint32_t nodeIdA[FLAT_CHUNKS] = {}, parentA[FLAT_CHUNKS] = {}, ownerGroupA[FLAT_CHUNKS] = {}, segFirstCountA[FLAT_CHUNKS] = {}, firstBitRelA[FLAT_CHUNKS] = {};
                const m4 model = load_m4(&obj->model[0][0]);
                const m4 prevModel = a.occlusion ? load_m4(&obj->prevModel[0][0]) : model;
                const float scale = max_axis_scale(model);
                const f3 instC{inst.boundingSphere[0], inst.boundingSphere[1], inst.boundingSphere[2]}; const float instR = inst.boundingSphere[3];
                {
                    const f3 c = to_view_space(instC, model, view);
                    const float r = instR * scale;
                    const bool bad = isnan(c.x) || isnan(c.y) || isnan(c.z) || isinf(c.x) || isinf(c.y) || isinf(c.z) || isnan(r) || isinf(r);
                    nTested++;
                    if (bad || sphere_culled(a, cam, c, r)) continue;
                    nVisible++;
                }
                const bool skinned = iw.skinned != 0u;
                uint64_t preM[FLAT_CHUNKS] = {}, expandM[FLAT_CHUNKS] = {}, hiddenM[FLAT_CHUNKS] = {}, leafM[FLAT_CHUNKS] = {}, reached[FLAT_CHUNKS] = {};
                uint32_t slabDescA[FLAT_CHUNKS] = {}, slabOffA[FLAT_CHUNKS] = {};
                [[maybe_unused]] uint64_t seenLeafM[FLAT_CHUNKS] = {};
#pragma unroll
                for (uint32_t c = 0; c < FLAT_CHUNKS; c++) if (c < chunks) {
                    const bool mine = c * 64u + lane < iw.flatCount;
                    FlatNode fn{}; FlatLeaf fl{};
                    if (mine) { fn = a.flatNodes[iw.flatBase + c * 64u + lane]; fl = a.flatLeaves[iw.flatBase + c * 64u + lane]; }
// ... 365 lines not shown
                    buckets[slotB] = b;
                }
            }
        }
    }
#pragma unroll
    for (int o = 32; o > 0; o >>= 1) nNodes += (uint32_t)__shfl_xor((int)nNodes, o);
    if (lane == 0) {
        uint32_t* stripe = a.counters + CNT_STRIPES + ((blockIdx.x * 16u + wave) & (CNT_STRIPE_COUNT - 1u)) * CNT_STRIPE_WORDS;
        if (nTested) atomicAdd(&stripe[0], nTested);
        if (nVisible) atomicAdd(&stripe[1], nVisible);
        if (nNodes) atomicAdd(&stripe[2], nNodes);
    }
}

template <bool FIRST, typename Residency>
__global__ void __launch_bounds__(256) k_cull_flat_level(CullArgs a, uint32_t level, const NodeRecord* in, NodeRecord* out, BucketRecord* buckets, Residency res) {
    __shared__ uint32_t waveTot[3][4], bases[3];
    const brmi_scene_buffers& sc = a.sc;
    const uint32_t t = threadIdx.x, lane = t & 63u, wave = t >> 6;
    const uint32_t viewId = sc.perFrame->mainCameraIndex;
    const brmi_camera* cam = sc.cameras + viewId;
    const brmi_culling_camera* lodCam = sc.cullingCameras + viewId;
    const bool ortho = cam->isOrtho != 0;
    const f3 camPos{lodCam->positionWorldSpace[0], lodCam->positionWorldSpace[1], lodCam->positionWorldSpace[2]};
    const float zNear = lodCam->zNear, threshold = lodCam->errorOverDistanceThreshold;
    const m4 view = load_m4(&cam->view[0][0]);
    const uint32_t count = FIRST ? sc.activeDrawCount : min(a.counters[CNT_FRONTIER0 + level], a.recordCapacity);
    uint32_t* nextCount = &a.counters[CNT_FRONTIER0 + level + 1u];
    const uint32_t rounded = (count + 255u) & ~255u;
    uint32_t nTested = 0, nVisible = 0, nNodes = 0;
    for (uint32_t idx = blockIdx.x * 256u + t; idx < rounded; idx += gridDim.x * 256u) {
        bool have = idx < count;
        uint32_t instIndex = 0, pos = 0;
        InstanceWalk iw{0u, 0u, 0u, 0u}; brmi_per_mesh_instance inst{};
        if (have) {
            if (FIRST) instIndex = sc.activeDraws[idx];
            else { const NodeRecord rec = in[idx]; instIndex = rec.instanceIndex; pos = rec.nodeIdPacked; }
            iw = a.instanceWalk[instIndex]; inst = sc.perMeshInstance[instIndex];
            if (iw.flatCount == 0u) have = false;
        }
        bool hidden = false, leafOk = false;
        uint32_t childMask = 0, firstChild = 0, nChunks = 0, slabDesc = 0, slabOff = 0;
        FlatNode fn{};
        if (have) {
            const brmi_per_object* obj = sc.perObject + inst.perObjectBufferIndex;
            const m4 model = load_m4(&obj->model[0][0]);
            const float scale = max_axis_scale(model);
            const f3 instC{inst.boundingSphere[0], inst.boundingSphere[1], inst.boundingSphere[2]}; const float instR = inst.boundingSphere[3];
            if (FIRST) {
                const f3 c = to_view_space(instC, model, view);
                const float r = instR * scale;
                const bool bad = isnan(c.x) || isnan(c.y) || isnan(c.z) || isinf(c.x) || isinf(c.y) || isinf(c.z) || isnan(r) || isinf(r);
                nTested++;
                if (bad || sphere_culled(a, cam, c, r)) have = false; else nVisible++;
            }
            if (have) {
                nNodes++;
                fn = a.flatNodes[iw.flatBase + pos];
                const bool skinned = iw.skinned != 0u;
                const bool internal = (fn.info & 1u);
                const f3 cullC = skinned ? instC : f3{fn.cull[0], fn.cull[1], fn.cull[2]};
                const float cullR = skinned ? instR : fn.cull[3];
                const f3 cVS = to_view_space(cullC, model, view);
                const float rW = cullR * scale;
                const bool inFrustum = !sphere_culled(a, cam, cVS, rW);
                if (inFrustum && internal) {
                    const f3 lc = xyz(mul_point(f3{fn.lod[0], fn.lod[1], fn.lod[2]}, model));
                    const float e = projected_error(lc, fn.lod[3] * scale, fn.maxQuadricError, scale, camPos, zNear, ortho);
                    if (e >= threshold) {
                        hidden = a.occlusion && occlusion_test_prev(a, cam, cullC, cullR, load_m4(&obj->prevModel[0][0]));
                        if (!hidden) {
                            firstChild = fn.children & 0xFFFFu;
                            const uint32_t cc = min(fn.children >> 16, BRMI_BVH_MAX_CHILDREN);
#pragma unroll
                            for (uint32_t c = 0; c < BRMI_BVH_MAX_CHILDREN; c++) if (c < cc) {
                                const FlatNode* ch = a.flatNodes + (iw.flatBase + firstChild + c);
                                const float4 cs = *reinterpret_cast<const float4*>(ch->cull), ls = *reinterpret_cast<const float4*>(ch->lod);
                                const float chErr = ch->maxQuadricError; const uint32_t chInfo = ch->info;
                                const f3 ccVS = to_view_space(skinned ? instC : f3{cs.x, cs.y, cs.z}, model, view);
                                bool pre = !sphere_culled(a, cam, ccVS, (skinned ? instR : cs.w) * scale);
                                if (pre && (chInfo & 1u)) {
                                    const f3 wc = xyz(mul_point(f3{ls.x, ls.y, ls.z}, model));
                                    pre = projected_error(wc, ls.w * scale, chErr, scale, camPos, zNear, ortho) >= threshold;
                                }
                                childMask |= pre ? (1u << c) : 0u;
                            }
                        }
                    }
                } else if (inFrustum) {
                    const FlatLeaf fl = a.flatLeaves[iw.flatBase + pos];
                    if constexpr (Residency::kTracks) flat_leaf_touch(res, fn, fl, instIndex, model, scale, camPos, zNear, threshold, ortho);
                    if (flat_leaf_cut(res, fn, fl, model, scale, camPos, zNear, threshold, ortho) && ((fn.info >> 2) & 1u)) {
                        const brmi_group_page_map_entry pe = sc.groupPageMap[fn.pageMapIndex];
                        slabDesc = pe.slabDescriptorIndex; slabOff = pe.slabByteOffset;
                        leafOk = slabDesc != 0u;
                        nChunks = leafOk ? ((fn.segFirstCount >> 16) + a.factor - 1u) / a.factor : 0u;
                    }
                }
            }
        }
        const uint32_t mine[3] = {(uint32_t)__popc(childMask), nChunks, hidden ? 1u : 0u};
        uint32_t incl[3] = {mine[0], mine[1], mine[2]};
#pragma unroll
        for (int o = 1; o < 64; o <<= 1) {
#pragma unroll
            for (int q = 0; q < 3; q++) { const uint32_t v = (uint32_t)__shfl_up((int)incl[q], o); if (lane >= (uint32_t)o) incl[q] += v; }
        }
        __syncthreads();
        if (lane == 63u) { waveTot[0][wave] = incl[0]; waveTot[1][wave] = incl[1]; waveTot[2][wave] = incl[2]; }
        __syncthreads();
        if (t < 3u) {
            const uint32_t total = waveTot[t][0] + waveTot[t][1] + waveTot[t][2] + waveTot[t][3];
            uint32_t* counter = t == 0u ? nextCount : (t == 1u ? &a.counters[a.bucketCounter] : &a.counters[CNT_REPLAY_NODES]);
            bases[t] = total ? atomicAdd(counter, total) : 0u;
        }
        __syncthreads();
        uint32_t slot[3];
#pragma unroll
        for (int q = 0; q < 3; q++) { uint32_t wb = 0; for (uint32_t w = 0; w < 4u; w++) if (w < wave) wb += waveTot[q][w]; slot[q] = bases[q] + wb + incl[q] - mine[q]; }
        for (uint32_t m = childMask; m != 0u; m &= m - 1u, slot[0]++) {
            if (slot[0] < a.recordCapacity) out[slot[0]] = NodeRecord{instIndex, firstChild + (uint32_t)__ffs((int)m) - 1u};
            else atomicAdd(&a.counters[CNT_DROPPED_RECORDS], 1u);
        }
        if (nChunks != 0u) {
            const uint32_t segFirst = fn.segFirstCount & 0xFFFFu, segCount = fn.segFirstCount >> 16;
            for (uint32_t k = 0; k < nChunks; k++, slot[1]++) {
                if (slot[1] >= a.recordCapacity) { atomicAdd(&a.counters[CNT_DROPPED_RECORDS], 1u); continue; }
                BucketRecord b;
                b.instanceIndex = instIndex; b.groupIdPacked = fn.ownerGroup & 0x7FFFFFFFu;
                b.meshletIndexAndCount = (min(a.factor, segCount - k * a.factor) << 16) | ((segFirst + k * a.factor) & 0xFFFFu);
                b.pageSlabDescriptorIndex = slabDesc; b.pageSlabByteOffset = slabOff;
                b.firstBit = iw.bitBase + fn.firstBitRel + k * a.factor; b.pad0 = 0; b.pad1 = 0;
                buckets[slot[1]] = b;
            }
        }
        if (hidden) {
            if (slot[2] < a.recordCapacity) a.replayNodes[slot[2]] = NodeRecord{instIndex, 0x80000000u | (1u << 30) | (fn.nodeId & 0x3FFFFFFFu)};
            else atomicAdd(&a.counters[CNT_DROPPED_RECORDS], 1u);
        }
    }
#pragma unroll
    for (int o = 32; o > 0; o >>= 1) { nNodes += (uint32_t)__shfl_xor((int)nNodes, o); nTested += (uint32_t)__shfl_xor((int)nTested, o); nVisible += (uint32_t)__shfl_xor((int)nVisible, o); }
    if (lane == 0) {
        uint32_t* stripe = a.counters + CNT_STRIPES + ((blockIdx.x * 4u + wave) & (CNT_STRIPE_COUNT - 1u)) * CNT_STRIPE_WORDS;
        if (nTested) atomicAdd(&stripe[0], nTested);
        if (nVisible) atomicAdd(&stripe[1], nVisible);
        if (nNodes) atomicAdd(&stripe[2], nNodes);
    }
}

template <int SIDE, typename Residency>
__global__ void __launch_bounds__(256) k_cull_clusters(CullArgs a, const BucketRecord* buckets, TempVisible* temp, uint32_t* bitmask, uint8_t* blockDirty,
                                                       typename std::conditional<SIDE == 1, LcRide, typename std::conditional<SIDE == 2, ClearRide, NoSide>::type>::type ride, Residency res) {
    uint32_t mainBlocks = gridDim.x;
    if constexpr (SIDE == 1) {
        mainBlocks = ride.mainBlocks;
        if (blockIdx.x >= ride.mainBlocks) { lc_fill_block(ride.lc, blockIdx.x - ride.mainBlocks, threadIdx.x); return; }
    }
    if constexpr (SIDE == 2) {
        mainBlocks = ride.mainBlocks;
        if (blockIdx.x >= ride.mainBlocks) {
            const uint64_t stride = (uint64_t)ride.clearBlocks * 256u;
            for (uint64_t i = (uint64_t)(blockIdx.x - ride.mainBlocks) * 256u + threadIdx.x; i < ride.n2; i += stride) ride.vis2[i] = make_ulonglong2(BRMI_VIS_EMPTY, BRMI_VIS_EMPTY);
            return;
        }
    }
    const brmi_scene_buffers& sc = a.sc;
    const uint32_t bucketCount = min(a.counters[a.bucketCounter], a.recordCapacity);
    if (a.feedback && blockIdx.x == 0u && threadIdx.x == 0u) __hip_atomic_store(a.feedback + (a.phase == 1u ? 2 : 4), bucketCount, __ATOMIC_RELAXED, __HIP_MEMORY_SCOPE_SYSTEM);
    const uint32_t viewId = sc.perFrame->mainCameraIndex;
    const brmi_camera* cam = sc.cameras + viewId;
    const brmi_culling_camera* lodCam = sc.cullingCameras + viewId;
    const bool ortho = cam->isOrtho != 0;
    const f3 camPos{lodCam->positionWorldSpace[0], lodCam->positionWorldSpace[1], lodCam->positionWorldSpace[2]};
    const float zNear = lodCam->zNear, threshold = lodCam->errorOverDistanceThreshold;
    const m4 view = load_m4(&cam->view[0][0]);
    uint32_t* tempCount = &a.counters[a.phase == 2 ? CNT_TEMP_VISIBLE2 : CNT_TEMP_VISIBLE];
    const uint64_t totalLanes = (uint64_t)bucketCount * a.factor;
    const uint64_t rounded = (totalLanes + 255ull) & ~255ull;
    __shared__ uint32_t waveSurv[4], waveOccl[4], blockSlots[2];
    for (uint64_t idx = (uint64_t)blockIdx.x * blockDim.x + threadIdx.x; idx < rounded; idx += (uint64_t)mainBlocks * blockDim.x) {
        bool survives = false, occluded = false, tested = false;
        uint4 packed = make_uint4(0, 0, 0, 0);
        uint32_t bit = 0;
        uint4 againLo = make_uint4(0u, 0u, 0u, 0u); uint2 againHi = make_uint2(0u, 0u);
        if (idx < totalLanes) {
            const uint32_t bi = (uint32_t)(idx / a.factor), m = (uint32_t)(idx % a.factor);
            const BucketRecord b = buckets[bi];
            const uint32_t count = b.meshletIndexAndCount >> 16, first = b.meshletIndexAndCount & 0xFFFFu;
            if (m < count && b.pageSlabDescriptorIndex != 0u) {
                tested = true;
                const bool replay = (b.groupIdPacked >> 31) != 0;
                const uint32_t lm = first + m;
                const uint8_t* slab = sc.slabs[b.pageSlabDescriptorIndex];
                const brmi_page_header* hdr = reinterpret_cast<const brmi_page_header*>(slab + b.pageSlabByteOffset);
                if (lm < hdr->meshletCount) {
                    const brmi_meshlet_descriptor* desc = reinterpret_cast<const brmi_meshlet_descriptor*>(slab + b.pageSlabByteOffset + hdr->descriptorOffset + lm * 64u);
                    float4 bounds = *reinterpret_cast<const float4*>(desc->bounds);
                    const uint32_t triAndRefined = desc->triangleCountAndRefinedGroup;
                    const brmi_per_mesh_instance inst = sc.perMeshInstance[b.instanceIndex];
                    if ((sc.perMesh[inst.perMeshBufferIndex].vertexFlags & BRMI_VERTEX_SKINNED) != 0u)
                        bounds = skinned_meshlet_bounds(sc, desc, hdr, slab + b.pageSlabByteOffset, inst.skinningInstanceSlot, bounds);
                    const brmi_clod_mesh_metadata* md = sc.meshMetadata + sc.clodOffsets[b.instanceIndex].clodMeshMetadataIndex;
                    const m4 model = load_m4(&sc.perObject[inst.perObjectBufferIndex].model[0][0]);
                    const float scale = max_axis_scale(model);
                    const f3 cVS = to_view_space(f3{bounds.x, bounds.y, bounds.z}, model, view);
                    const float rW = bounds.w * scale;
                    survives = replay || !sphere_outside_frustum(cVS, rW, cam->clippingPlanes);
                    if (survives && refined_meshlets_replace(res, sc, md->groupsBase, triAndRefined >> 16, b.groupIdPacked & 0x7FFFFFFFu, b.instanceIndex, model, scale, camPos, zNear, threshold, ortho)) survives = false;
                    if (survives && a.bandActive) {
                        if (dot3(f3{a.bandTop[0], a.bandTop[1], a.bandTop[2]}, cVS) < -rW || dot3(f3{a.bandBottom[0], a.bandBottom[1], a.bandBottom[2]}, cVS) < -rW) survives = false;
                    }
                    if (survives && stripe_on(a.stripes) && stripe_rejects(a.stripes, cam, cVS, rW)) survives = false;
                    if (survives && a.occlusion &&
                        occlusion_test(a, cam, replay, f3{bounds.x, bounds.y, bounds.z}, bounds.w, cVS, rW, sc.perObject + inst.perObjectBufferIndex)) {
                        survives = false;
                        if (!replay) {
                            occluded = true;
                            againLo = make_uint4(b.instanceIndex, 0x80000000u | (b.groupIdPacked & 0x7FFFFFFFu), (1u << 16) | (lm & 0xFFFFu), b.pageSlabDescriptorIndex);
                            againHi = make_uint2(b.pageSlabByteOffset, b.firstBit + m);
                        }
                    }
                    if (survives) {
                        packed = pack_visible_cluster(viewId, b.instanceIndex, lm, b.groupIdPacked & 0x7FFFFFFFu, b.pageSlabDescriptorIndex, b.pageSlabByteOffset);
                        bit = b.firstBit + m;
                    }
                }
            }
        }
        {
            const uint64_t tm = __ballot(tested);
            if (tm != 0ull && (threadIdx.x & 63u) == 0u) atomicAdd(&a.counters[CNT_STRIPES + (blockIdx.x & (CNT_STRIPE_COUNT - 1u)) * CNT_STRIPE_WORDS + STRIPE_MESHLETS_TESTED], (uint32_t)__popcll(tm));
        }
        occluded = occluded && a.occlusion && a.phase == 1u;
        const uint64_t survM = __ballot(survives), occlM = __ballot(occluded);
        const uint32_t wv = threadIdx.x >> 6;
        __syncthreads();
        if ((threadIdx.x & 63u) == 0u) { waveSurv[wv] = (uint32_t)__popcll(survM); waveOccl[wv] = (uint32_t)__popcll(occlM); }
        __syncthreads();
        if (threadIdx.x < 2u) {
            const uint32_t* ws = threadIdx.x == 0u ? waveSurv : waveOccl;
            const uint32_t total = ws[0] + ws[1] + ws[2] + ws[3];
            blockSlots[threadIdx.x] = total ? atomicAdd(threadIdx.x == 0u ? tempCount : &a.counters[CNT_REPLAY_MESHLETS], total) : 0u;
        }
        __syncthreads();
        uint32_t slot = blockSlots[0] + lane_rank(survM), rs = blockSlots[1] + lane_rank(occlM);
        for (uint32_t w = 0; w < wv; w++) { slot += waveSurv[w]; rs += waveOccl[w]; }
        if (occluded) {
            if (rs < a.recordCapacity) { uint4* dst = reinterpret_cast<uint4*>(&a.replayBuckets[rs]); dst[0] = againLo; dst[1] = make_uint4(againHi.x, againHi.y, 0u, 0u); }
            else atomicAdd(&a.counters[CNT_DROPPED_RECORDS], 1u);
        }
        if (survives) {
            if (slot < a.visibleCapacity) {
                TempVisible t; t.packed = packed; t.bit = bit; t.pad0 = t.pad1 = t.pad2 = 0;
                temp[slot] = t;
                atomicOr(&bitmask[bit >> 5], 1u << (bit & 31u));
                blockDirty[bit >> 16] = 1;
            } else atomicAdd(&a.counters[CNT_DROPPED_CLUSTERS], 1u);
        }
    }
}

constexpr uint32_t SCAN_BLOCK_WORDS = 2048;

__global__ void __launch_bounds__(256) k_scan_reduce(const uint32_t* bitmask, uint32_t totalWords, uint32_t* blockSums, const uint8_t* blockDirty) {
    __shared__ uint32_t partial[4];
    if (blockDirty[blockIdx.x] == 0) { if (threadIdx.x == 0) blockSums[blockIdx.x] = 0u; return; }
    const uint32_t base = blockIdx.x * SCAN_BLOCK_WORDS;
    uint32_t s = 0;
    for (uint32_t i = threadIdx.x; i < SCAN_BLOCK_WORDS; i += 256) { const uint32_t w = base + i; if (w < totalWords) s += __popc(bitmask[w]); }
#pragma unroll
    for (int o = 32; o > 0; o >>= 1) s += __shfl_xor((int)s, o);
    if ((threadIdx.x & 63u) == 0) partial[threadIdx.x >> 6] = s;
    __syncthreads();
    if (threadIdx.x == 0) blockSums[blockIdx.x] = partial[0] + partial[1] + partial[2] + partial[3];
}

__global__ void __launch_bounds__(1024) k_scan_blocks(uint32_t* blockSums, uint32_t nBlocks, uint32_t* counters, uint32_t outIndex, uint32_t capacity, uint32_t usedIndex, uint32_t* hostFeedback) {
    __shared__ uint32_t waveTotals[16];
    __shared__ uint32_t carry;
    if (threadIdx.x == 0) carry = 0;
    __syncthreads();
    for (uint32_t base = 0; base < nBlocks; base += 1024) {
        const uint32_t i = base + threadIdx.x;
        const uint32_t v = i < nBlocks ? blockSums[i] : 0u;
        uint32_t incl = v;
#pragma unroll
        for (int o = 1; o < 64; o <<= 1) { const uint32_t t = (uint32_t)__shfl_up((int)incl, o); if ((threadIdx.x & 63u) >= (uint32_t)o) incl += t; }
        if ((threadIdx.x & 63u) == 63u) waveTotals[threadIdx.x >> 6] = incl;
        __syncthreads();
        uint32_t waveBase = 0;
        for (uint32_t w = 0; w < (threadIdx.x >> 6); w++) waveBase += waveTotals[w];
        const uint32_t c = carry;
        if (i < nBlocks) blockSums[i] = c + waveBase + incl - v;
        __syncthreads();
        if (threadIdx.x == 1023) carry = c + waveBase + incl;
        __syncthreads();
    }
    if (threadIdx.x == 0) {
        const uint32_t placed = min(carry, capacity - (usedIndex == 0xFFFFFFFFu ? 0u : min(counters[usedIndex], capacity)));
        counters[outIndex] = placed;
        if (hostFeedback) __hip_atomic_store(hostFeedback, placed, __ATOMIC_RELAXED, __HIP_MEMORY_SCOPE_SYSTEM);
    }
}

__global__ void __launch_bounds__(256) k_scan_words(const uint32_t* bitmask, uint32_t totalWords, const uint32_t* blockSums, uint32_t* wordPrefix, const uint8_t* blockDirty) {
    __shared__ uint32_t waveTotals[4];
    __shared__ uint32_t carry;
    if (blockDirty[blockIdx.x] == 0) return;
    if (threadIdx.x == 0) carry = blockSums[blockIdx.x];
    __syncthreads();
    const uint32_t base = blockIdx.x * SCAN_BLOCK_WORDS;
    for (uint32_t chunk = 0; chunk < SCAN_BLOCK_WORDS; chunk += 256) {
        const uint32_t w = base + chunk + threadIdx.x;
        const uint32_t v = w < totalWords ? __popc(bitmask[w]) : 0u;
        uint32_t incl = v;
#pragma unroll
        for (int o = 1; o < 64; o <<= 1) { const uint32_t t = (uint32_t)__shfl_up((int)incl, o); if ((threadIdx.x & 63u) >= (uint32_t)o) incl += t; }
        if ((threadIdx.x & 63u) == 63u) waveTotals[threadIdx.x >> 6] = incl;
        __syncthreads();
        uint32_t waveBase = 0;
        for (uint32_t k = 0; k < (threadIdx.x >> 6); k++) waveBase += waveTotals[k];
        const uint32_t c = carry;
        if (w < totalWords) wordPrefix[w] = c + waveBase + incl - v;
        __syncthreads();
        if (threadIdx.x == 255) carry = c + waveBase + incl;
        __syncthreads();
    }
}

constexpr uint32_t SCAN_CHAIN_BLOCKS = 64;
__global__ void __launch_bounds__(256) k_scan_chained(const uint32_t* bitmask, uint32_t totalWords, unsigned long long* agg, uint32_t epoch, uint32_t* wordPrefix,
                                                     uint32_t* counters, uint32_t outIndex, uint32_t capacity, uint32_t usedIndex, uint32_t* hostFeedback) {
    __shared__ uint32_t waveTotals[4];
    __shared__ uint32_t blockPrefix, ticket;
    if (threadIdx.x == 0) ticket = (uint32_t)__hip_atomic_fetch_add(&agg[SCAN_CHAIN_BLOCKS], 1ull, __ATOMIC_RELAXED, __HIP_MEMORY_SCOPE_AGENT);
    __syncthreads();
    const uint32_t block = ticket;
    const uint32_t base = block * SCAN_BLOCK_WORDS + threadIdx.x * 8u;
    uint32_t pc[8], sum = 0;
#pragma unroll
    for (uint32_t k = 0; k < 8u; k++) { const uint32_t w = base + k; pc[k] = w < totalWords ? (uint32_t)__popc(bitmask[w]) : 0u; sum += pc[k]; }
    uint32_t incl = sum;
#pragma unroll
    for (int o = 1; o < 64; o <<= 1) { const uint32_t t = (uint32_t)__shfl_up((int)incl, o); if ((threadIdx.x & 63u) >= (uint32_t)o) incl += t; }
    if ((threadIdx.x & 63u) == 63u) waveTotals[threadIdx.x >> 6] = incl;
    __syncthreads();
    uint32_t waveBase = 0, blockSum = 0;
    for (uint32_t k = 0; k < 4u; k++) { if (k < (threadIdx.x >> 6)) waveBase += waveTotals[k]; blockSum += waveTotals[k]; }
    if (threadIdx.x == 0) __hip_atomic_store(&agg[block], ((unsigned long long)epoch << 32) | blockSum, __ATOMIC_RELAXED, __HIP_MEMORY_SCOPE_AGENT);
    if (threadIdx.x < 64u) {
        uint32_t mine = 0;
        if (threadIdx.x < block) {
            unsigned long long v;
            do { v = __hip_atomic_load(&agg[threadIdx.x], __ATOMIC_RELAXED, __HIP_MEMORY_SCOPE_AGENT); } while ((uint32_t)(v >> 32) != epoch);
            mine = (uint32_t)v;
        }
#pragma unroll
        for (int o = 32; o > 0; o >>= 1) mine += (uint32_t)__shfl_xor((int)mine, o);
        if (threadIdx.x == 0) blockPrefix = mine;
    }
    __syncthreads();
    uint32_t run = blockPrefix + waveBase + incl - sum;
#pragma unroll
    for (uint32_t k = 0; k < 8u; k++) { const uint32_t w = base + k; if (w < totalWords) wordPrefix[w] = run; run += pc[k]; }
    if (block == gridDim.x - 1u && threadIdx.x == 0) {
        __hip_atomic_store(&agg[SCAN_CHAIN_BLOCKS], 0ull, __ATOMIC_RELAXED, __HIP_MEMORY_SCOPE_AGENT);
        const uint32_t placed = min(blockPrefix + blockSum, capacity - (usedIndex == 0xFFFFFFFFu ? 0u : min(counters[usedIndex], capacity)));
        counters[outIndex] = placed;
        if (hostFeedback) __hip_atomic_store(hostFeedback, placed, __ATOMIC_RELAXED, __HIP_MEMORY_SCOPE_SYSTEM);
    }
}

#ifndef BRMI_LOCAL_RANK_WORDS
#define BRMI_LOCAL_RANK_WORDS 8192
#endif
constexpr uint32_t LOCAL_RANK_WORDS = BRMI_LOCAL_RANK_WORDS;
struct LocalRank { uint32_t totalWords, outIndex, usedIndex; uint32_t* hostFeedback; };
struct DrawLists {
    uint32_t* drawList; HeldRecord* held; uint32_t countAll;
    const MeshletBox* boxes; const uint32_t* pageBoxBase; const float* objConst; uint32_t maxTexels; BoxViewport vp; HzbDesc hzb;
};
template <bool LOCAL_RANK, bool HOLD>
__global__ void __launch_bounds__(256) k_scatter_visible(const TempVisible* temp, uint32_t* counters, uint32_t tempCountIndex, const uint32_t* bitmask,
                                                        const uint32_t* wordPrefix, uint4* visible, uint32_t baseIndexCounter, uint32_t capacity, uint32_t visibleCapacity,
                                                        brmi_scene_buffers sc, ClusterSetup* setup, uint32_t resolveCapacity, ClusterUv* clusterUv, LocalRank lr, DrawLists dl) {
    const uint8_t* const* slabs = sc.slabs;
    const uint32_t n = min(counters[tempCountIndex], visibleCapacity);
    const uint32_t base = baseIndexCounter == 0xFFFFFFFFu ? 0u : counters[baseIndexCounter];
    const uint32_t rounded = (n + 63u) & ~63u;
    __shared__ uint32_t prefixLds[LOCAL_RANK ? LOCAL_RANK_WORDS : 1];
    __shared__ uint32_t waveTotals[4];
    if (LOCAL_RANK) {
        if (blockIdx.x != 0u && blockIdx.x * blockDim.x >= rounded) return;
        const uint32_t span = (lr.totalWords + 255u) / 256u;
        const uint32_t w0 = threadIdx.x * span, w1 = min(w0 + span, lr.totalWords);
        uint32_t sum = 0;
        for (uint32_t w = w0; w < w1; w++) sum += __popc(bitmask[w]);
        uint32_t incl = sum;
#pragma unroll
        for (int o = 1; o < 64; o <<= 1) { const uint32_t t = (uint32_t)__shfl_up((int)incl, o); if ((threadIdx.x & 63u) >= (uint32_t)o) incl += t; }
        if ((threadIdx.x & 63u) == 63u) waveTotals[threadIdx.x >> 6] = incl;
        __syncthreads();
        uint32_t waveBase = 0, all = 0;
        for (uint32_t w = 0; w < 4; w++) { if (w < (threadIdx.x >> 6)) waveBase += waveTotals[w]; all += waveTotals[w]; }
        uint32_t run = waveBase + incl - sum;
        for (uint32_t w = w0; w < w1; w++) { prefixLds[w] = run; run += __popc(bitmask[w]); }
        if (blockIdx.x == 0u && threadIdx.x == 0u) {
            const uint32_t placed = min(all, capacity - (lr.usedIndex == 0xFFFFFFFFu ? 0u : min(counters[lr.usedIndex], capacity)));
            counters[lr.outIndex] = placed;
            if (lr.hostFeedback) __hip_atomic_store(lr.hostFeedback, placed, __ATOMIC_RELAXED, __HIP_MEMORY_SCOPE_SYSTEM);
        }
        __syncthreads();
    }
    __shared__ unsigned long long blockBase;
    __shared__ uint32_t waveV[4], waveT[4], waveD[4], waveH[4], blockDraw, blockHeld;
    unsigned long long drawnVT = 0ull;
    if (blockIdx.x == 0u && threadIdx.x == 0u) { const uint32_t room = base < capacity ? capacity - base : 0u; atomicAdd(&counters[CNT_RASTER_CLUSTERS], min(n, room)); if (resolveCapacity == 0u && n != 0u) atomicOr(&counters[CNT_RESOLVE_SPILL], 1u); }
    const uint32_t rounded256 = (n + 255u) & ~255u;
    for (uint32_t i = blockIdx.x * blockDim.x + threadIdx.x; i < rounded256; i += gridDim.x * blockDim.x) {
        uint32_t verts = 0, tris = 0, placed = 0, dst = 0;
        TempVisible t{};
        const uint8_t* slab = nullptr; uint32_t pageOff = 0;
        const brmi_page_header* hdr = nullptr; const brmi_meshlet_descriptor* desc = nullptr;
        uint32_t held = 0u, boxIndex = 0xFFFFFFFFu, perObject = 0u;
        if (i < n) {
            t = temp[i];
            const uint32_t w = t.bit >> 5, b = t.bit & 31u;
            const uint32_t rank = (LOCAL_RANK ? prefixLds[w] : wordPrefix[w]) + __popc(bitmask[w] & ((1u << b) - 1u));
            dst = base + rank;
            if (dst < capacity) {
                visible[dst] = t.packed;
                slab = slabs[vc_slab(t.packed)];
                pageOff = vc_page_offset(t.packed);
                hdr = reinterpret_cast<const brmi_page_header*>(slab + pageOff);
                desc = reinterpret_cast<const brmi_meshlet_descriptor*>(slab + pageOff + hdr->descriptorOffset + vc_meshlet(t.packed) * 64u);
                verts = min((desc->bitsAndVertexCount >> 24) & 0xFFu, BRMI_MESHLET_MAX_VERTS);
                tris = min(desc->triangleCountAndRefinedGroup & 0xFFFFu, BRMI_MESHLET_MAX_TRIS);
                placed = 1;
                if (HOLD) {
                    const brmi_per_mesh_instance inst = sc.perMeshInstance[vc_instance(t.packed)];
                    perObject = inst.perObjectBufferIndex;
                    const uint32_t boxBase = dl.pageBoxBase[(size_t)vc_slab(t.packed) * 1024u + (pageOff >> 18)];
                    if (boxBase != 0xFFFFFFFFu && (sc.perMesh[inst.perMeshBufferIndex].vertexFlags & BRMI_VERTEX_SKINNED) == 0u) {
                        boxIndex = boxBase + vc_meshlet(t.packed);
                        const MeshletBox bx = dl.boxes[boxIndex];
                        const float* oc = dl.objConst + (size_t)perObject * OBJ_CONST_FLOATS;
                        if (bx.valid && box_behind_chain(dl.hzb, bx, oc + 36, oc + 52, dl.vp, dl.maxTexels)) held = 1u;
                    }
                }
            }
        }
        uint32_t inclV = verts, inclT = tris;
#pragma unroll
        for (int o = 1; o < 64; o <<= 1) {
            const uint32_t v = (uint32_t)__shfl_up((int)inclV, o), tt = (uint32_t)__shfl_up((int)inclT, o);
            if ((threadIdx.x & 63u) >= (uint32_t)o) { inclV += v; inclT += tt; }
        }
        const bool isHeld = HOLD && placed != 0u && held != 0u, isDraw = HOLD && placed != 0u && !isHeld;
        const uint64_t drawM = __ballot(isDraw), heldM = __ballot(isHeld);
        __syncthreads();
        if ((threadIdx.x & 63u) == 63u) { waveV[threadIdx.x >> 6] = inclV; waveT[threadIdx.x >> 6] = inclT; waveD[threadIdx.x >> 6] = (uint32_t)__popcll(drawM); waveH[threadIdx.x >> 6] = (uint32_t)__popcll(heldM); }
        __syncthreads();
        if (threadIdx.x == 0u) {
            const unsigned long long totV = (unsigned long long)waveV[0] + waveV[1] + waveV[2] + waveV[3], totT = (unsigned long long)waveT[0] + waveT[1] + waveT[2] + waveT[3];
            blockBase = (totV | totT) ? atomicAdd(reinterpret_cast<unsigned long long*>(&counters[CNT_SUM_VERTS_LO]), totV | (totT << 32)) : 0ull;
        }
        if (HOLD && threadIdx.x == 64u) { const uint32_t tot = waveD[0] + waveD[1] + waveD[2] + waveD[3]; blockDraw = tot ? atomicAdd(&counters[CNT_DRAW1], tot) : 0u; }
        if (HOLD && threadIdx.x == 128u) { const uint32_t tot = waveH[0] + waveH[1] + waveH[2] + waveH[3]; blockHeld = tot ? atomicAdd(&counters[CNT_HELD1], tot) : 0u; }
        __syncthreads();
        if (dl.countAll && placed) drawnVT += (unsigned long long)verts | ((unsigned long long)tris << 32);
        if (isDraw || isHeld) {
            uint32_t slot = (isDraw ? blockDraw : blockHeld) + lane_rank(isDraw ? drawM : heldM);
            for (uint32_t w = 0; w < (threadIdx.x >> 6); w++) slot += isDraw ? waveD[w] : waveH[w];
            if (isDraw) { dl.drawList[slot] = dst; drawnVT += (unsigned long long)verts | ((unsigned long long)tris << 32); }
            else dl.held[slot] = HeldRecord{dst, boxIndex, perObject, verts | (tris << 16)};
        }
        unsigned long long baseV = (uint32_t)blockBase, baseT = blockBase >> 32;
        for (uint32_t w = 0; w < (threadIdx.x >> 6); w++) { baseV += waveV[w]; baseT += waveT[w]; }
        if (placed) {
            const uint32_t instanceIndex = vc_instance(t.packed);
            const brmi_per_mesh_instance inst = sc.perMeshInstance[instanceIndex];
            const brmi_per_object* obj = sc.perObject + inst.perObjectBufferIndex;
            ClusterSetup cs;
            cs.posBase = slab + pageOff + hdr->positionBitstreamOffset + desc->positionBitOffset;
            cs.triBase = slab + pageOff + hdr->triangleStreamOffset + desc->triangleByteOffset;
            cs.nrmBase = slab + pageOff + hdr->normalArrayOffset + desc->vertexAttributeOffset * 4u;
            const brmi_per_mesh* pm = sc.perMesh + inst.perMeshBufferIndex;
            cs.counts = verts | (tris << 8) | ((hdr->compressedPositionQuantExp & 0xFFu) << 16) | (((obj->objectFlags & BRMI_OBJECT_FLAG_REVERSE_WINDING) != 0 ? 1u : 0u) << 24)
                      | ((pm->vertexFlags & BRMI_VERTEX_SKINNED) ? BRMI_CS_SKINNED : 0u) | ((hdr->attributeMask & BRMI_PAGE_ATTRIBUTE_JOINTS) ? BRMI_CS_JOINTS : 0u)
                      | ((hdr->attributeMask & BRMI_PAGE_ATTRIBUTE_WEIGHTS) ? BRMI_CS_WEIGHTS : 0u);
            if (clusterUv) {
                const uint32_t mflags = sc.materials[pm->materialDataIndex].materialFlags;
                const bool layerTextures = openpbr_has_textures(sc.openpbrMaterials + sc.materials[pm->materialDataIndex].openPBRMaterialDataIndex);
                cs.counts |= ((mflags & BRMI_MATERIAL_ALPHA_TEST) ? BRMI_CS_ALPHA : 0u) | (((mflags & BRMI_MATERIAL_ANY_TEXTURE) || layerTextures) ? BRMI_CS_TEXTURED : 0u);
                ClusterUv cu{nullptr, nullptr, nullptr, 0, 0u};
                if (hdr->attributeMask & BRMI_PAGE_ATTRIBUTE_COLOR) { cs.counts |= BRMI_CS_COLOR; cu.color = slab + pageOff + hdr->colorArrayOffset + desc->vertexAttributeOffset * 4u; }
                if (hdr->uvSetCount != 0u) {
                    cu.desc = slab + pageOff + hdr->uvDescriptorOffset + (vc_meshlet(t.packed) * hdr->uvSetCount) * 32u;
                    cu.stream = slab + pageOff + *reinterpret_cast<const uint32_t*>(slab + pageOff + hdr->uvBitstreamDirectoryOffset);
                    cu.directory = (int32_t)hdr->uvBitstreamDirectoryOffset - (int32_t)(hdr->uvDescriptorOffset + (vc_meshlet(t.packed) * hdr->uvSetCount) * 32u);
                    cu.setCount = hdr->uvSetCount;
                }
                clusterUv[dst] = cu;
            }
            cs.jointDelta = (int32_t)(hdr->jointArrayOffset + desc->vertexAttributeOffset * 32u) - (int32_t)(hdr->normalArrayOffset + desc->vertexAttributeOffset * 4u);
            cs.weightDelta = (int32_t)(hdr->weightArrayOffset + desc->vertexAttributeOffset * 32u) - (int32_t)(hdr->normalArrayOffset + desc->vertexAttributeOffset * 4u);
            cs.perObjectIndex = inst.perObjectBufferIndex; cs.instanceIndex = instanceIndex; cs.viewId = vc_view(t.packed);
            cs.materialDataIndex = pm->materialDataIndex; cs.normalMatrixIndex = obj->normalMatrixBufferIndex;
            const unsigned long long v0 = baseV + (inclV - verts), t0 = baseT + (inclT - tris);
            const bool fits = v0 + verts <= resolveCapacity && t0 + tris <= resolveCapacity;
            cs.vertBase = fits ? (uint32_t)v0 : BRMI_ARENA_NONE; cs.triBase32 = fits ? (uint32_t)t0 : BRMI_ARENA_NONE;
            if (!fits && resolveCapacity != 0u) atomicOr(&counters[CNT_RESOLVE_SPILL], 1u);
            setup[dst] = cs;
        }
    }
    if (HOLD || dl.countAll) {
#pragma unroll
        for (int o = 32; o > 0; o >>= 1) drawnVT += (unsigned long long)__shfl_xor((long long)drawnVT, o);
        if ((threadIdx.x & 63u) == 0u && drawnVT != 0ull) atomicAdd(reinterpret_cast<unsigned long long*>(&counters[CNT_DRAWN_VT]), drawnVT);
    }
}

static inline uint32_t grid_for(uint64_t items, uint32_t block, uint32_t maxBlocks) {
    uint64_t g = (items + block - 1) / block;
    if (g < 1) g = 1;
    if (g > maxBlocks) g = maxBlocks;
    return (uint32_t)g;
}

__global__ void k_seed_phase2(uint32_t* counters, uint32_t capacity) { seed_phase2(counters, capacity, threadIdx.x); }

int launch_cull(brmi_pass* p, uint32_t phase, hipStream_t s) {
    if (int rc = ensure_frame_constants(p, s)) return rc;
    if (phase != 1 && phase != 2) return fail(p, BRMI_ERR_INVALID, "brmi_cull: phase %u (1 or 2)", phase);
    if (phase == 2 && !p->cfg.enableOcclusionCulling) return fail(p, BRMI_ERR_STATE, "brmi_cull: phase 2 needs a pass created with enableOcclusionCulling");
    if (phase == 2 && !p->hzbValid) return fail(p, BRMI_ERR_STATE, "brmi_cull: phase 2 needs brmi_build_hzb on the phase-1 depth first");
    CullArgs a;
    a.sc = p->scene; a.counters = p->counters();
    a.instanceBitBase = p->wsPtr<uint32_t>(p->ws.instanceBitBase); a.segPrefix = p->wsPtr<uint32_t>(p->ws.segPrefix);
    a.flatNodes = p->wsPtr<FlatNode>(p->ws.flatNodes); a.flatLeaves = p->wsPtr<FlatLeaf>(p->ws.flatLeaves); a.instanceWalk = p->wsPtr<InstanceWalk>(p->ws.instanceWalk);
    a.recordCapacity = p->cfg.maxTraversalRecords; a.visibleCapacity = p->cfg.maxVisibleClusters;
    uint32_t f = p->cfg.phase2ExpansionFactor; f = f < 1 ? 1 : (f > 64 ? 64 : f);
    { uint32_t n = 1; for (uint32_t c = 2; c <= 64; c <<= 1) if (c <= f) n = c; f = n; }
    a.factor = f; a.phase = phase; a.packedFlat = 0u; a.wideFlat = 0u;
    a.feedback = p->ensureFeedback() ? p->phase2FeedbackDev : nullptr;

    const bool symmetricPerspective = p->camHost.isOrtho == 0 && p->camHost.projection[2][0] == 0.0f && p->camHost.projection[2][1] == 0.0f &&
                                      p->camHost.projection[3][0] == 0.0f && p->camHost.projection[3][1] == 0.0f;
    a.bandActive = ((p->bandY0 != 0 || p->bandY1 != p->cfg.height) && symmetricPerspective) ? 1u : 0u;
    for (int k = 0; k < 3; k++) { a.bandTop[k] = p->bandPlaneTop[k]; a.bandBottom[k] = p->bandPlaneBottom[k]; }
    a.bandPlanes = reinterpret_cast<const float4*>(p->wsPtr<m4>(p->ws.frameConst) + 3);
    a.stripes = p->stripes;
    const brmi_pass* chain = p->chainOwner(phase);
    a.occlusion = (p->cfg.enableOcclusionCulling && chain->hzbValid && p->camHost.isOrtho == 0) ? 1u : 0u;
    a.replayNodes = p->wsPtr<NodeRecord>(p->ws.replayNodes); a.replayBuckets = p->wsPtr<BucketRecord>(p->ws.replayBuckets);
    a.hzb = chain->hzbDesc();
    if (phase == 1) {
        const uint32_t lastVisible = p->phase2FeedbackHost ? reinterpret_cast<volatile uint32_t*>(p->phase2FeedbackHost)[3] : 0u;
        const uint32_t lastPhase2 = p->phase2FeedbackHost ? reinterpret_cast<volatile uint32_t*>(p->phase2FeedbackHost)[0] : 0xFFFFFFFFu;
        p->holdThisFrame = p->holdEnabled && a.occlusion != 0u && (p->holdMinClusters == 0u || (lastVisible != 0xFFFFFFFFu && lastVisible >= p->holdMinClusters) ||
                                                                  (p->holdStillMax != 0u && lastPhase2 < p->holdStillMax && lastVisible != 0xFFFFFFFFu && lastVisible >= p->holdFloor));
    }
    a.frontier0Counter = phase == 1 ? (uint32_t)CNT_FRONTIER0 : (uint32_t)CNT_REPLAY_NODES;
    a.bucketCounter = CNT_BUCKETS;
    NodeRecord* fa = p->wsPtr<NodeRecord>(p->ws.frontierA); NodeRecord* fb = p->wsPtr<NodeRecord>(p->ws.frontierB);
    BucketRecord* buckets = phase == 1 ? p->wsPtr<BucketRecord>(p->ws.buckets) : a.replayBuckets;
    TempVisible* temp = p->wsPtr<TempVisible>(p->ws.tempVisible);
    uint32_t* bitmask = p->wsPtr<uint32_t>(phase == 1 ? p->ws.bitmask1 : p->ws.bitmask2);
    uint8_t* blockDirty = p->wsPtr<uint8_t>(p->ws.blockDirty) + (phase == 1 ? 0u : p->scanBlocks + 1u);
    uint32_t* wordPrefix = p->wsPtr<uint32_t>(p->ws.wordPrefix); uint32_t* blockSums = p->wsPtr<uint32_t>(p->ws.blockSums);

    auto with_residency = [&](auto launch) { if (p->streaming.on) launch(stream_args_of(p)); else launch(AllResident{}); };
    const uint32_t maxBlocks = 1024;
    bool lightGridRides = false;
    bool flatLevels = false;
    const bool hierarchy = p->tables.minLevelWidth <= HIER_CAP_MAX && !p->forceLevelKernels;
    const bool levelKernels = p->tables.maxLevelWidth > p->tables.spillWidth || p->forceLevelKernels;
    const uint32_t* meshWidth = p->wsPtr<uint32_t>(p->ws.meshLevelWidth);
    const bool spillMode = hierarchy && levelKernels;
    a.meshLevelWidth = meshWidth; a.levelKernelsWidthLo = 0u;
    if (spillMode) a.frontier0Counter = CNT_FRONTIER0;
    const uint32_t widthAll = spillMode ? 0xFFFFFFFFu : 0u, spillAbove = spillMode ? p->tables.spillWidth : 0xFFFFFFFFu;
    if (phase == 1) {
        if (!p->frameStateCleared) BRMI_HIP(p, hipMemsetAsync(p->counters(), 0, p->ws.frameClearBytes, s));
        p->frameStateCleared = false;
        if (p->streaming.on) BRMI_HIP(p, hipMemsetAsync(p->streaming.b.scratch, 0, stream_scratch_layout(p->streaming.groupCount).frameBytes, s));
        a.packedFlat = (hierarchy && !p->tables.flatNodes.empty() && p->packedFlat) ? 1u : 0u;
        a.wideFlat = (hierarchy && p->tables.anyWideFlat && !p->splitFrame) ? 1u : 0u;
        const uint32_t draws = p->scene.activeDrawCount, minDraws = std::max(1u, p->flatLevelsMinDraws);
        flatLevels = hierarchy && p->tables.allMeshesFlat && !p->forceLevelKernels && (draws >= minDraws || (p->splitFrame && p->tables.maxLevelWidth > 256u && draws >= std::max(1u, minDraws / 4u)));
        if (flatLevels) {
            if (p->clearVisibilityWithTraversal && (p->bandPixelCount & 1ull) == 0ull) { p->clearVisibilityWithTraversal = false; p->clearVisibilityWithClusterCull = true; }
            else if (p->clearVisibilityWithTraversal) flatLevels = false;
        }
        if (flatLevels) {
            with_residency([&](auto res) { hipLaunchKernelGGL((k_cull_flat_level<true, decltype(res)>), dim3(grid_for(p->scene.activeDrawCount, 256, 8192)), dim3(256), 0, s, a, 0u, (const NodeRecord*)nullptr, fb, buckets, res); });
            for (uint32_t level = 1; level < p->tables.flatMaxDepth; level++)
                with_residency([&](auto res) { hipLaunchKernelGGL((k_cull_flat_level<false, decltype(res)>), dim3(2048), dim3(256), 0, s, a, level, (const NodeRecord*)((level & 1u) ? fb : fa), (level & 1u) ? fa : fb, buckets, res); });
            BRMI_LAUNCH_CHECK(p, "k_cull_flat_level");
        }
        const dim3 hgrid(std::min(std::max(1u, p->scene.activeDrawCount), 16384u) + (a.packedFlat ? (p->scene.activeDrawCount + 7u) / 8u : 0u));
        if (hierarchy && !flatLevels) {
            const bool wide = p->tables.maxLevelWidth > 256u;
            const uint32_t widthHi = spillMode ? widthAll : (wide ? HIER_CAP_MAX : 256u);
            if (p->clearVisibilityWithTraversal) {
                SideJobs sj{reinterpret_cast<ulonglong2*>(static_cast<unsigned long long*>(p->res[BRMI_RES_VISIBILITY]) + p->bandFirstPixel), p->bandPixelCount >> 1, hgrid.x, p->clearRiderBlocks, cluster_args_of(p)};
                const dim3 grid(hgrid.x + sj.clearBlocks + p->numLightClusters);
                if (wide) with_residency([&](auto res) { hipLaunchKernelGGL((k_cull_hierarchy<false, 1024, BRMI_HIER_STAGE_WIDE, true, decltype(res)>), grid, dim3(64), 0, s, a, buckets, meshWidth, 0u, widthHi, spillAbove, fa, sj, res); });
                else with_residency([&](auto res) { hipLaunchKernelGGL((k_cull_hierarchy<false, 256, 128, true, decltype(res)>), grid, dim3(64), 0, s, a, buckets, meshWidth, 0u, widthHi, spillAbove, fa, sj, res); });
                p->clearVisibilityWithTraversal = false; lightGridRides = true;
            } else if (wide) with_residency([&](auto res) { hipLaunchKernelGGL((k_cull_hierarchy<false, 1024, BRMI_HIER_STAGE_WIDE, false, decltype(res)>), hgrid, dim3(64), 0, s, a, buckets, meshWidth, 0u, widthHi, spillAbove, fa, NoSide{}, res); });
            else with_residency([&](auto res) { hipLaunchKernelGGL((k_cull_hierarchy<false, 256, 128, false, decltype(res)>), hgrid, dim3(64), 0, s, a, buckets, meshWidth, 0u, widthHi, spillAbove, fa, NoSide{}, res); });
        }
        if (a.wideFlat && !flatLevels) with_residency([&](auto res) { hipLaunchKernelGGL((k_cull_flat_wide<decltype(res)>), dim3(std::min(std::max(1u, p->scene.activeDrawCount), 4096u)), dim3(1024), 0, s, a, buckets, res); });
        if (levelKernels && !spillMode && !flatLevels) hipLaunchKernelGGL(k_cull_instances, dim3(grid_for(p->scene.activeDrawCount, 256, maxBlocks)), dim3(256), 0, s, a, fa);
        BRMI_LAUNCH_CHECK(p, "k_cull_instances");
    } else {
        if (!p->phase2Seeded) hipLaunchKernelGGL(k_seed_phase2, dim3(1), dim3(128), 0, s, p->counters(), a.recordCapacity);
        p->phase2Seeded = false;
        const NoSide none{};
        if (hierarchy && p->tables.maxLevelWidth <= 256u) with_residency([&](auto res) { hipLaunchKernelGGL((k_cull_hierarchy<true, 256, 128, false, decltype(res)>), dim3(2048), dim3(64), 0, s, a, buckets, meshWidth, 0u, 256u, spillAbove, fa, none, res); });
        else if (hierarchy) with_residency([&](auto res) { hipLaunchKernelGGL((k_cull_hierarchy<true, 1024, BRMI_HIER_STAGE_WIDE, false, decltype(res)>), dim3(2048), dim3(64), 0, s, a, buckets, meshWidth, 0u, spillMode ? widthAll : HIER_CAP_MAX, spillAbove, fa, none, res); });
    }
    const uint32_t travGrid = grid_for(std::min<uint64_t>(p->cfg.maxTraversalRecords, (uint64_t)p->scene.lodNodeCount * 4 + 4096), 256, maxBlocks);
    const uint32_t levelLaunches = spillMode ? std::min(p->maxLevels, std::max(1u, p->tables.spillLevels)) : p->maxLevels;
    const bool flatCoversPhase1 = phase == 1 && hierarchy && spillMode && p->tables.allMeshesFlat && a.wideFlat != 0u && !p->forceLevelKernels;
    for (uint32_t level = 0; level < levelLaunches && levelKernels && !flatCoversPhase1 && !flatLevels; level++) {
        const NodeRecord* in = level == 0 ? ((phase == 1 || spillMode) ? fa : a.replayNodes) : ((level & 1u) ? fb : fa);
        with_residency([&](auto res) { hipLaunchKernelGGL((k_traverse<decltype(res)>), dim3(travGrid), dim3(256), 0, s, a, level, in, (level & 1u) ? fa : fb, buckets, res); });
        BRMI_LAUNCH_CHECK(p, "k_traverse");
    }
    uint32_t smallGrid = phase == 1 ? 512u : 128u, scatterGrid = smallGrid;
    if (p->phase2FeedbackHost) {
        const uint32_t lastBuckets = reinterpret_cast<volatile uint32_t*>(p->phase2FeedbackHost)[phase == 1 ? 2 : 4];
        const uint32_t lastVisible = reinterpret_cast<volatile uint32_t*>(p->phase2FeedbackHost)[phase == 1 ? 3 : 0];
        smallGrid = std::max(smallGrid, grid_for((uint64_t)std::min<uint32_t>(lastBuckets, p->cfg.maxTraversalRecords) * f, 256, 8192));
        scatterGrid = std::max(scatterGrid, grid_for(std::min<uint32_t>(lastVisible, p->cfg.maxVisibleClusters), 256, 8192));
    }
    if (lightGridRides) {
        with_residency([&](auto res) { hipLaunchKernelGGL((k_cull_clusters<1, decltype(res)>), dim3(smallGrid + (p->numLightClusters + 3u) / 4u), dim3(256), 0, s, a, (const BucketRecord*)buckets, temp, bitmask, blockDirty, LcRide{smallGrid, cluster_args_of(p)}, res); });
        p->lightGridDone = true;
    } else if (phase == 1 && p->clearVisibilityWithClusterCull) {
        const uint32_t clearBlocks = 2048;
        with_residency([&](auto res) { hipLaunchKernelGGL((k_cull_clusters<2, decltype(res)>), dim3(smallGrid + clearBlocks), dim3(256), 0, s, a, (const BucketRecord*)buckets, temp, bitmask, blockDirty, ClearRide{smallGrid, reinterpret_cast<ulonglong2*>(static_cast<unsigned long long*>(p->res[BRMI_RES_VISIBILITY]) + p->bandFirstPixel), p->bandPixelCount >> 1, clearBlocks}, res); });
        p->clearVisibilityWithClusterCull = false;
    } else with_residency([&](auto res) { hipLaunchKernelGGL((k_cull_clusters<0, decltype(res)>), dim3(smallGrid), dim3(256), 0, s, a, (const BucketRecord*)buckets, temp, bitmask, blockDirty, NoSide{}, res); });
    BRMI_LAUNCH_CHECK(p, "k_cull_clusters");
    const uint32_t outIndex = phase == 1 ? CNT_VISIBLE : CNT_VISIBLE2, usedIndex = phase == 1 ? 0xFFFFFFFFu : (uint32_t)CNT_VISIBLE;
    if (phase == 2 && p->phase2DirectMax != 0u) (void)p->ensureFeedback();
    uint32_t* feedback = phase == 2 ? p->phase2FeedbackDev : (p->phase2FeedbackDev ? p->phase2FeedbackDev + 3 : nullptr);
    const bool localRank = p->totalWords <= LOCAL_RANK_WORDS && !p->forceLevelKernels;
    if (localRank) {
    } else {
        if (p->scanBlocks <= SCAN_CHAIN_BLOCKS) {
            if (++p->scanEpoch == 0u) p->scanEpoch = 1u;
            hipLaunchKernelGGL(k_scan_chained, dim3(p->scanBlocks), dim3(256), 0, s, bitmask, p->totalWords, p->wsPtr<unsigned long long>(p->ws.scanAgg), p->scanEpoch, wordPrefix,
                               p->counters(), outIndex, p->cfg.maxVisibleClusters, usedIndex, feedback);
        } else {
            hipLaunchKernelGGL(k_scan_reduce, dim3(p->scanBlocks), dim3(256), 0, s, bitmask, p->totalWords, blockSums, blockDirty);
            hipLaunchKernelGGL(k_scan_blocks, dim3(1), dim3(1024), 0, s, blockSums, p->scanBlocks, p->counters(), outIndex, p->cfg.maxVisibleClusters, usedIndex, feedback);
            hipLaunchKernelGGL(k_scan_words, dim3(p->scanBlocks), dim3(256), 0, s, bitmask, p->totalWords, blockSums, wordPrefix, blockDirty);
        }
    }
    if (phase == 1) p->inlineResolve = resolve_inline_frame(p);
    const uint32_t arenaCapacity = p->inlineResolve ? 0u : p->resolveCapacity;
    auto scatter = [&](auto kernel) {
        hipLaunchKernelGGL(kernel, dim3(scatterGrid), dim3(256), 0, s, temp, p->counters(), (uint32_t)(phase == 1 ? CNT_TEMP_VISIBLE : CNT_TEMP_VISIBLE2), bitmask, wordPrefix,
                           static_cast<uint4*>(p->res[BRMI_RES_VISIBLE_CLUSTERS]), phase == 1 ? 0xFFFFFFFFu : (uint32_t)CNT_VISIBLE, p->cfg.maxVisibleClusters, p->cfg.maxVisibleClusters, p->scene, p->wsPtr<ClusterSetup>(p->ws.clusterSetup), arenaCapacity,
                           (p->tables.hasTextures || p->tables.hasAlphaTest || p->tables.hasVertexColors) ? p->wsPtr<ClusterUv>(p->ws.clusterUv) : nullptr, LocalRank{p->totalWords, outIndex, usedIndex, feedback},
                           (phase == 1 && p->holdThisFrame) ? DrawLists{p->wsPtr<uint32_t>(p->ws.drawList), p->wsPtr<HeldRecord>(p->ws.heldRecords), 0u, p->wsPtr<MeshletBox>(p->ws.meshletBoxes), p->wsPtr<uint32_t>(p->ws.pageBoxBase),
                                                                      p->wsPtr<float>(p->ws.objConst), p->holdMaxTexels, BoxViewport{(float)p->cfg.width, (float)p->cfg.height, 0.0f, 0.0f, 0, (int)p->bandY0, (int)p->cfg.width - 1, (int)p->bandY1 - 1}, a.hzb}
                                                          : DrawLists{nullptr, nullptr, p->holdThisFrame ? 1u : 0u, nullptr, nullptr, nullptr, 0u, BoxViewport{}, HzbDesc{}});
    };
    const bool holdLists = phase == 1 && p->holdThisFrame;
    if (localRank) { if (holdLists) scatter(k_scatter_visible<true, true>); else scatter(k_scatter_visible<true, false>); }
    else { if (holdLists) scatter(k_scatter_visible<false, true>); else scatter(k_scatter_visible<false, false>); }
    BRMI_LAUNCH_CHECK(p, "compaction");
    return BRMI_OK;
}


__global__ void __launch_bounds__(256) k_meshlet_boxes(const uint8_t* const* slabs, const PageRef* pages, MeshletBox* boxes) {
    const PageRef pr = pages[blockIdx.x];
    const uint8_t* page = slabs[pr.slab] + pr.byteOffset;
    const brmi_page_header* hdr = reinterpret_cast<const brmi_page_header*>(page);
    const uint32_t lane = threadIdx.x & 63u;
    const bool float3 = (hdr->compressedPositionQuantExp & 0xFFu) == BRMI_POSITION_FORMAT_FLOAT3;
    for (uint32_t m = threadIdx.x >> 6; m < pr.meshletCount; m += 4u) {
        const brmi_meshlet_descriptor* desc = reinterpret_cast<const brmi_meshlet_descriptor*>(page + hdr->descriptorOffset + m * 64u);
        const uint32_t verts = min((desc->bitsAndVertexCount >> 24) & 0xFFu, BRMI_MESHLET_MAX_VERTS);
        f3 lo{3.0e38f, 3.0e38f, 3.0e38f}, hi{-3.0e38f, -3.0e38f, -3.0e38f};
        bool finite = true;
        if (float3) for (uint32_t v = lane; v < verts; v += 64u) {
            const float* pp = reinterpret_cast<const float*>(page + hdr->positionBitstreamOffset + desc->positionBitOffset + v * 12u);
            const f3 q{pp[0], pp[1], pp[2]};
            finite = finite && fabsf(q.x) < 1.0e30f && fabsf(q.y) < 1.0e30f && fabsf(q.z) < 1.0e30f;
            lo = min3v(lo, q); hi = max3v(hi, q);
        }
#pragma unroll
        for (int o = 32; o > 0; o >>= 1) {
            lo.x = min2(lo.x, __shfl_xor(lo.x, o)); lo.y = min2(lo.y, __shfl_xor(lo.y, o)); lo.z = min2(lo.z, __shfl_xor(lo.z, o));
            hi.x = max2(hi.x, __shfl_xor(hi.x, o)); hi.y = max2(hi.y, __shfl_xor(hi.y, o)); hi.z = max2(hi.z, __shfl_xor(hi.z, o));
        }
        finite = __all(finite);
        if (lane == 0u) boxes[pr.boxBase + m] = MeshletBox{{lo.x, lo.y, lo.z}, (float3 && verts != 0u && finite) ? 1u : 0u, {hi.x, hi.y, hi.z}, 0u};
    }
}

int launch_meshlet_boxes(brmi_pass* p, hipStream_t s) {
    if (p->tables.pageRefs.empty()) return BRMI_OK;
    hipLaunchKernelGGL(k_meshlet_boxes, dim3((uint32_t)p->tables.pageRefs.size()), dim3(256), 0, s, p->scene.slabs, p->wsPtr<PageRef>(p->ws.pageRefs), p->wsPtr<MeshletBox>(p->ws.meshletBoxes));
    BRMI_LAUNCH_CHECK(p, "k_meshlet_boxes");
    return BRMI_OK;
}

BRMI_DEV uint32_t block_exclusive_scan_1024(uint32_t v, uint32_t* waveTotals , uint32_t& total) {
    const uint32_t lane = threadIdx.x & 63u, wave = threadIdx.x >> 6;
    uint32_t incl = v;
#pragma unroll
    for (int o = 1; o < 64; o <<= 1) { const uint32_t t = (uint32_t)__shfl_up((int)incl, o); if (lane >= (uint32_t)o) incl += t; }
    __syncthreads();
    if (lane == 63u) waveTotals[wave] = incl;
    __syncthreads();
    uint32_t base = 0, all = 0;
    for (uint32_t w = 0; w < 16u; w++) { if (w < wave) base += waveTotals[w]; all += waveTotals[w]; }
    total = all;
    return base + incl - v;
}

__global__ void __launch_bounds__(1024) k_stream_feedback(StreamArgs st, uint32_t* listA, uint32_t* listB, brmi_streaming_request* loadRequests, uint32_t requestCapacity,
                                                          uint32_t* touchedGroups, uint32_t touchedCapacity, uint32_t* counts, const brmi_per_mesh_instance* instances, uint32_t instanceCount,
                                                          const brmi_per_frame* perFrame) {
    __shared__ uint32_t waveTotals[17], digitBase[256], digitHist[256];
    __shared__ uint16_t waveDigit[16][256];
    const uint32_t t = threadIdx.x, lane = t & 63u, wave = t >> 6;
    const uint32_t groups = st.groupCount, words = (groups + 31u) >> 5;
    uint32_t carry = 0;
    for (uint32_t base = 0; base < words; base += 1024u) {
        const uint32_t w = base + t;
        uint32_t bits = w < words ? st.touchedBits[w] : 0u;
        if (w == words - 1u && (groups & 31u)) bits &= (1u << (groups & 31u)) - 1u;
        uint32_t total;
        uint32_t slot = carry + block_exclusive_scan_1024((uint32_t)__popc(bits), waveTotals, total);
        for (; bits != 0u; bits &= bits - 1u, slot++) if (slot < touchedCapacity) touchedGroups[slot] = w * 32u + (uint32_t)__ffs((int)bits) - 1u;
        carry += total;
    }
    if (t == 0) counts[1] = carry;
    uint32_t requests = 0;
    for (uint32_t base = 0; base < groups; base += 1024u) {
        const uint32_t g = base + t;
        const bool has = g < groups && st.requestKeys[g] != 0ull;
        uint32_t total;
        const uint32_t slot = requests + block_exclusive_scan_1024(has ? 1u : 0u, waveTotals, total);
        if (has) listA[slot] = g;
        requests += total;
    }
    if (t == 0) counts[0] = requests;
    uint32_t* src = listA; uint32_t* dst = listB;
    for (uint32_t shift = 0; shift < 16u; shift += 8u) {
        __syncthreads();
        __threadfence_block();
        if (t < 256u) digitHist[t] = 0u;
        __syncthreads();
        for (uint32_t i = t; i < requests; i += 1024u) atomicAdd(&digitHist[((0xFFFFu - ((uint32_t)(st.requestKeys[src[i]] >> 32) & 0xFFFFu)) >> shift) & 0xFFu], 1u);
        __syncthreads();
        if (wave == 0u) {
            const uint32_t c0 = digitHist[lane * 4u], c1 = digitHist[lane * 4u + 1u], c2 = digitHist[lane * 4u + 2u], c3 = digitHist[lane * 4u + 3u];
            uint32_t incl = c0 + c1 + c2 + c3;
#pragma unroll
            for (int o = 1; o < 64; o <<= 1) { const uint32_t v = (uint32_t)__shfl_up((int)incl, o); if (lane >= (uint32_t)o) incl += v; }
            const uint32_t excl = incl - (c0 + c1 + c2 + c3);
            digitBase[lane * 4u] = excl; digitBase[lane * 4u + 1u] = excl + c0; digitBase[lane * 4u + 2u] = excl + c0 + c1; digitBase[lane * 4u + 3u] = excl + c0 + c1 + c2;
        }
        for (uint32_t base = 0; base < requests; base += 1024u) {
            __syncthreads();
            for (uint32_t k = t; k < 16u * 256u; k += 1024u) (&waveDigit[0][0])[k] = 0;
            __syncthreads();
            const uint32_t i = base + t;
            const bool valid = i < requests;
            const uint32_t g = valid ? src[i] : 0u;
            const uint32_t d = valid ? ((0xFFFFu - ((uint32_t)(st.requestKeys[g] >> 32) & 0xFFFFu)) >> shift) & 0xFFu : 0u;
            uint64_t same = __ballot(valid);
#pragma unroll
            for (uint32_t b = 0; b < 8u; b++) { const uint64_t m = __ballot(valid && ((d >> b) & 1u)); same &= ((d >> b) & 1u) ? m : ~m; }
            const uint32_t rankInWave = (uint32_t)__popcll(same & ((1ull << lane) - 1ull));
            if (valid && rankInWave == 0u) waveDigit[wave][d] = (uint16_t)__popcll(same);
            __syncthreads();
            if (valid) {
                uint32_t before = 0;
                for (uint32_t w = 0; w < wave; w++) before += waveDigit[w][d];
                dst[digitBase[d] + before + rankInWave] = g;
            }
            __syncthreads();
            if (t < 256u) { uint32_t all = 0; for (uint32_t w = 0; w < 16u; w++) all += waveDigit[w][t]; digitBase[t] += all; }
        }
        uint32_t* x = src; src = dst; dst = x;
    }
    __syncthreads();
    __threadfence_block();
    const uint32_t view = perFrame->mainCameraIndex;
    for (uint32_t i = t; i < min(requests, requestCapacity); i += 1024u) {
        const uint32_t g = src[i];
        const unsigned long long key = st.requestKeys[g];
        const uint32_t inst = ~(uint32_t)key, priority16 = (uint32_t)(key >> 32) & 0xFFFFu;
        brmi_streaming_request r;
        r.groupGlobalIndex = g; r.meshInstanceIndex = inst; r.meshBufferIndex = inst < instanceCount ? instances[inst].perMeshBufferIndex : 0u;
        r.viewId = (priority16 << 16) | (view & 0xFFFFu);
        loadRequests[i] = r;
    }
}

int launch_streaming_feedback(brmi_pass* p, hipStream_t s) {
    const StreamScratchLayout l = stream_scratch_layout(p->streaming.groupCount);
    uint8_t* scratch = static_cast<uint8_t*>(p->streaming.b.scratch);
    hipLaunchKernelGGL(k_stream_feedback, dim3(1), dim3(1024), 0, s, stream_args_of(p), reinterpret_cast<uint32_t*>(scratch + l.listA), reinterpret_cast<uint32_t*>(scratch + l.listB),
                       p->streaming.b.loadRequests, p->streaming.b.requestCapacity, p->streaming.b.touchedGroups, p->streaming.b.touchedCapacity, p->streaming.b.counts,
                       p->scene.perMeshInstance, p->scene.perMeshInstanceCount, p->scene.perFrame);
    BRMI_LAUNCH_CHECK(p, "k_stream_feedback");
    return BRMI_OK;
}

}
```

basicrenderer_amd/csrc/brmi_internal.h:

```cpp
#ifndef BRMI_INTERNAL_H
#define BRMI_INTERNAL_H

#include <hip/hip_runtime.h>

#include <string>
#include <vector>

#include "brmi.h"
#include "brmi_device.h"
#include "brmi_scene_tables.h"

#ifndef BRMI_BIN_COUNT_STRIDE
#define BRMI_BIN_COUNT_STRIDE 32
#endif
namespace brmi {

enum CounterIndex : uint32_t {
    CNT_VISIBLE = 3,
    CNT_VISIBLE2,
    CNT_DROPPED_RECORDS,
    CNT_DROPPED_CLUSTERS,
    CNT_INSTANCES_TESTED,
    CNT_INSTANCES_VISIBLE,
    CNT_NODES_VISITED,
    CNT_MESHLETS_TESTED,
    CNT_LIGHT_PAGES,
    CNT_SUM_VERTS_LO = 14, CNT_SUM_VERTS_HI,
    CNT_SUM_TRIS_LO, CNT_SUM_TRIS_HI,
    CNT_RASTER_CLUSTERS,
    CNT_BIN_OVERFLOW,
    CNT_DEFERRED_PIXELS_B,
    CNT_DEFERRED_PIXELS,
    CNT_RESOLVE_SPILL,
    CNT_RESERVED_37,
    CNT_DEFERRED_DROPPED,
    CNT_TILE_OVERFLOW,
    CNT_STRIPE_COUNT = 64, CNT_STRIPE_WORDS = 32,
    STRIPE_DEFERRED_A = 4, STRIPE_DEFERRED_B = 8,
    STRIPE_OVERFLOW = 3,
    STRIPE_MESHLETS_TESTED = 12,
    CNT_BUCKETS = 128 + 64 * 32,
    CNT_TEMP_VISIBLE = CNT_BUCKETS + 32,
    CNT_TEMP_VISIBLE2 = CNT_BUCKETS + 64,
    CNT_REPLAY_NODES = CNT_BUCKETS + 96,
    CNT_REPLAY_MESHLETS = CNT_BUCKETS + 128,
    CNT_DRAW1 = CNT_BUCKETS + 160,
    CNT_HELD1 = CNT_BUCKETS + 192,
    CNT_LATE1 = CNT_BUCKETS + 224,
    CNT_DRAWN_VT = CNT_BUCKETS + 256,
    CNT_WIDE1 = CNT_BUCKETS + 288, CNT_WIDE1B = CNT_BUCKETS + 320, CNT_WIDE2 = CNT_BUCKETS + 352,
    CNT_GENERAL1 = CNT_BUCKETS + 384,
    CNT_BIG1 = CNT_BUCKETS + 416,
    CNT_WORDS = CNT_BUCKETS + 416 + 64 * 32
};
static_assert((CNT_DRAWN_VT & 1u) == 0u, "64-bit counter");

__device__ inline void seed_phase2(uint32_t* counters, uint32_t capacity, uint32_t t) {
    if (t == 0) { counters[CNT_REPLAY_NODES] = min(counters[CNT_REPLAY_NODES], capacity); counters[CNT_BUCKETS] = min(counters[CNT_REPLAY_MESHLETS], capacity); counters[CNT_TEMP_VISIBLE2] = 0; counters[CNT_VISIBLE2] = 0; }
    if (t < CNT_STRIPES - CNT_FRONTIER0) counters[CNT_FRONTIER0 + t] = 0;
    if (t < CNT_STRIPE_COUNT) {
        uint32_t* q = &counters[CNT_STRIPES + t * CNT_STRIPE_WORDS + STRIPE_OVERFLOW];
        if (*q) atomicAdd(&counters[CNT_BIN_OVERFLOW], *q);
        *q = 0u;
    }
}

struct NodeRecord { uint32_t instanceIndex, nodeIdPacked; };
struct BucketRecord {
    uint32_t instanceIndex, groupIdPacked, meshletIndexAndCount, pageSlabDescriptorIndex;
    uint32_t pageSlabByteOffset, firstBit, pad0, pad1;
};
struct TempVisible { uint4 packed; uint32_t bit, pad0, pad1, pad2; };
struct MeshletBox { float lo[3]; uint32_t valid; float hi[3]; uint32_t pad; };
struct HeldRecord { uint32_t clusterIndex, boxIndex, perObjectIndex, vertsTris ; };
static_assert(sizeof(MeshletBox) == 32 && sizeof(HeldRecord) == 16, "draw-list records");
constexpr uint32_t OBJ_CONST_FLOATS = 56;

struct ClusterSetup {
    const uint8_t* posBase; const uint8_t* triBase; const uint8_t* nrmBase;
    uint32_t counts;
    uint32_t perObjectIndex, instanceIndex, viewId, materialDataIndex, normalMatrixIndex;
    uint32_t vertBase, triBase32;
    int32_t jointDelta, weightDelta;
};
constexpr uint32_t BRMI_CS_SKINNED = 1u << 25, BRMI_CS_JOINTS = 1u << 26, BRMI_CS_WEIGHTS = 1u << 27;
constexpr uint32_t BRMI_CS_ALPHA = 1u << 28, BRMI_CS_TEXTURED = 1u << 29, BRMI_CS_COLOR = 1u << 30;
struct AxisEntry { float uv; uint32_t tile; };
struct ShadeTables { AxisEntry* x; AxisEntry* y; float* sliceStart; };
struct MatConst {
    float baseWeight, specularWeight, specR, specG, specB, weightedSpecularIor, dielF0Scalar, coatF0Scalar, coatIor, coatDarkening, baseDiffuseRoughness, f90Diel;
    float fonA, fonK[4], eonSingleScale , eonAvgE, eonOneMinusAvgE, eonInvDen , dielF0[3];
};
static_assert(sizeof(MatConst) == 96, "six float4");
constexpr uint32_t BRMI_ARENA_NONE = 0xFFFFFFFFu;
struct ResolveVertex { float px, py, pz, nx, ny, nz; };
struct ResolveTriangle { float n0x, n0y, invW0, ddx[3], ddy[3], ddxSum, ddySum; uint32_t indices; };
struct MaterialWords { uint32_t albedo, metallicRoughness; unsigned long long coat, emissive, fuzz; float opIndexF; uint32_t pad; };
static_assert(sizeof(ResolveVertex) == 24 && sizeof(ResolveTriangle) == 48 && sizeof(MaterialWords) == 40, "table layouts");
static_assert(sizeof(ClusterSetup) == 64, "one cache line");

constexpr uint32_t kMaxHzbMips = 16;
struct HzbDesc {
    const float* depth; float* mips;
    uint32_t width, height, tilesX, mipCount, paddedW, paddedH;
    uint32_t rowLo, rowHi;
    StripeMap stripes;
    uint32_t mipOffset[kMaxHzbMips];
};

#ifndef BRMI_BOX_ROWS
#define BRMI_BOX_ROWS 2
#endif
struct BoxViewport { float width, height, minX, minY; int x0, y0, x1, y1; };
__device__ __forceinline__ bool box_behind_chain(const HzbDesc& hzb, const MeshletBox& bx, const float* mvpRows , const float* mvzRow ,
                                                 const BoxViewport& vp, uint32_t maxTexels) {
    float X[2][4], Y[2][4], Z[2][4];
    const int col[3] = {0, 1, 3};
    float magC = 0.0f, mag = fabsf(mvzRow[3]);
#pragma unroll
    for (int s = 0; s < 2; s++) {
        const float px = s ? bx.hi[0] : bx.lo[0], py = s ? bx.hi[1] : bx.lo[1], pz = s ? bx.hi[2] : bx.lo[2];
#pragma unroll
        for (int c = 0; c < 3; c++) {
            X[s][c] = px * mvpRows[0 + col[c]]; Y[s][c] = py * mvpRows[4 + col[c]]; Z[s][c] = pz * mvpRows[8 + col[c]] + mvpRows[12 + col[c]];
            magC = fmaxf(magC, fmaxf(fmaxf(fabsf(X[s][c]), fabsf(Y[s][c])), fmaxf(fabsf(pz * mvpRows[8 + col[c]]), fabsf(mvpRows[12 + col[c]]))));
        }
        X[s][3] = px * mvzRow[0]; Y[s][3] = py * mvzRow[1]; Z[s][3] = pz * mvzRow[2] + mvzRow[3];
        mag = fmaxf(mag, fmaxf(fmaxf(fabsf(X[s][3]), fabsf(Y[s][3])), fabsf(pz * mvzRow[2])));
    }
    float sx0 = 3.0e38f, sy0 = 3.0e38f, sx1 = -3.0e38f, sy1 = -3.0e38f, d = 3.0e38f, w = 3.0e38f;
#pragma unroll
    for (int k = 0; k < 8; k++) {
        const int i = k & 1, j = (k >> 1) & 1, l = k >> 2;
        const float cx = (X[i][0] + Y[j][0]) + Z[l][0], cy = (X[i][1] + Y[j][1]) + Z[l][1], cw = (X[i][2] + Y[j][2]) + Z[l][2];
        const float inv = __builtin_amdgcn_rcpf(cw);
        const float sx = (cx * inv + 1.0f) * 0.5f * vp.width + vp.minX, sy = (1.0f - cy * inv) * 0.5f * vp.height + vp.minY;
        sx0 = fminf(sx0, sx); sx1 = fmaxf(sx1, sx); sy0 = fminf(sy0, sy); sy1 = fmaxf(sy1, sy);
        d = fminf(d, -((X[i][3] + Y[j][3]) + Z[l][3])); w = fminf(w, cw);
    }
    if (!(w > 1e-6f && d > 0.0f && fabsf(sx0) < 1.0e9f && fabsf(sx1) < 1.0e9f && fabsf(sy0) < 1.0e9f && fabsf(sy1) < 1.0e9f)) return false;
    const float guard = 0.25f + magC * __builtin_amdgcn_rcpf(w) * 9.5367431640625e-7f * (vp.width + vp.height);
    const int x0 = max((int)floorf(fmaxf(sx0 - guard, -1.0e9f)), vp.x0), y0 = max((int)floorf(fmaxf(sy0 - guard, -1.0e9f)), vp.y0);
    const int x1 = min((int)floorf(fminf(sx1 + guard, 1.0e9f)), vp.x1), y1 = min((int)floorf(fminf(sy1 + guard, 1.0e9f)), vp.y1);
    const float nearSafe = d - (d * 7.62939453125e-6f + mag * 3.814697265625e-6f);
    if (!(nearSafe > 0.0f)) return false;
    if (x0 > x1 || y0 > y1) return true;
    uint32_t mip = 1u;
    while (mip + 1u < hzb.mipCount && (((x1 >> mip) - (x0 >> mip) + 1) > (int)maxTexels || ((y1 >> mip) - (y0 >> mip) + 1) > (int)maxTexels)) mip++;
    if (mip >= hzb.mipCount) return false;
    const uint32_t mw = max(hzb.paddedW >> mip, 1u), mh = max(hzb.paddedH >> mip, 1u);
    if (((x1 >> mip) - (x0 >> mip) + 1) > (int)maxTexels || ((y1 >> mip) - (y0 >> mip) + 1) > (int)maxTexels) return false;
    const float* m = hzb.mips + hzb.mipOffset[mip];
    const int tx0 = x0 >> mip, tx1 = min(x1 >> mip, (int)mw - 1), ty1 = min(y1 >> mip, (int)mh - 1);
    for (int y = y0 >> mip; y <= ty1; y += BRMI_BOX_ROWS) {
        float farthest = 0.0f;
#pragma unroll
        for (int r = 0; r < BRMI_BOX_ROWS; r++) {
            const int yy = min(y + r, ty1);
            for (int x = tx0; x <= tx1; x++) farthest = fmaxf(farthest, m[(size_t)yy * mw + (uint32_t)x]);
        }
        if (!(farthest < nearSafe)) return false;
    }
    return true;
}

__host__ __device__ inline uint32_t stream_priority16(float errorOverDistance) {
    float c = errorOverDistance * 1024.0f;
    c = c > 0.0f ? c : 0.0f;
    c = c < 65535.0f ? c : 65535.0f;
    return (uint32_t)(c + 0.5f);
}
struct StreamArgs {
    const uint32_t* nonResidentBits; uint32_t* touchedBits; unsigned long long* requestKeys; uint32_t activeGroupScanCount , groupCount;
    static constexpr bool kTracks = true;
    BRMI_DEV bool resident(uint32_t group) const {
        return group < activeGroupScanCount && ((nonResidentBits[group >> 5] >> (group & 31u)) & 1u) == 0u;
    }
    BRMI_DEV bool touch(uint32_t group, uint32_t instanceIndex, float errorOverDistance) const {
        if (group >= groupCount) return false;
        const uint32_t bit = 1u << (group & 31u);
        if ((__hip_atomic_load(&touchedBits[group >> 5], __ATOMIC_RELAXED, __HIP_MEMORY_SCOPE_AGENT) & bit) == 0u) atomicOr(&touchedBits[group >> 5], bit);
        if (resident(group)) return true;
        if (group < activeGroupScanCount) {
            const unsigned long long key = (1ull << 63) | ((unsigned long long)stream_priority16(errorOverDistance) << 32) | (unsigned long long)(~instanceIndex);
            if (__hip_atomic_load(&requestKeys[group], __ATOMIC_RELAXED, __HIP_MEMORY_SCOPE_AGENT) < key) atomicMax(&requestKeys[group], key);
        }
        return false;
    }
};
struct AllResident {
    static constexpr bool kTracks = false;
    BRMI_DEV bool resident(uint32_t) const { return true; }
    BRMI_DEV bool touch(uint32_t, uint32_t, float) const { return true; }
};
struct StreamScratchLayout { uint64_t touchedBits, requestKeys, frameBytes, listA, listB, total; };
inline StreamScratchLayout stream_scratch_layout(uint32_t groupCount) {
    StreamScratchLayout l{};
    const uint64_t g = groupCount ? groupCount : 1u;
    l.touchedBits = 0; l.requestKeys = (((g + 31u) / 32u * 4u) + 15u) & ~15ull; l.frameBytes = l.requestKeys + g * 8u;
    l.listA = (l.frameBytes + 15u) & ~15ull; l.listB = l.listA + ((g * 4u + 15u) & ~15ull); l.total = l.listB + ((g * 4u + 15u) & ~15ull);
    return l;
}

struct FrameSnapshot { brmi_per_frame perFrame; brmi_camera camera; float envSH[28]; };

struct LayerUniform { unsigned long long coatWord, fuzzWord, coatFilledWord, fuzzFilledWord; uint32_t coatUniform, fuzzUniform, coatFilled, fuzzFilled; };

struct Workspace {
    uint64_t counters, frontierA, frontierB, buckets, tempVisible, bitmask1, bitmask2, blockDirty, chainDirty, wordPrefix, blockSums,
             instanceBitBase, segPrefix, meshLevelWidth, scanAgg, flatNodes, flatLeaves, instanceWalk, planes, replayNodes, replayBuckets, lightVS, lightMeta, clusterPages, clusterHits, pageTotal, lightHitMasks, binCounts, binRecords, binOverflow, binPlan, binItems, binScratch, clusterSetup, resolveVerts, resolveTris, matWords, shadeTables, lutF, frameConst, objConst, matConst, deferredPixels,
             frameSnapshot, clusterUv, binAlpha, overflowAlpha, resolveUVs, resolveColors, alphaMats, shadeRows, shadeAvgs, ggxQuads, shadeLights, clusterList, listEntries, listRecords, layerUniform,
             meshletBoxes, pageBoxBase, pageRefs, drawList, heldRecords, lateList, wideQueue, wideAlpha, generalList, bigQueue, bigRuns, frameClearBytes, total;
};

}

struct brmi_pass {
    brmi_config cfg{};
    brmi_scene_buffers scene{};
    bool haveScene = false, setupDone = false, updated = false;
    void* res[BRMI_RES_COUNT] = {};
    uint64_t resBytes[BRMI_RES_COUNT] = {};
    uint64_t resNeed[BRMI_RES_COUNT] = {};
    uint32_t tilesX = 0, tilesY = 0;
    uint64_t paddedPixels = 0;
    uint32_t bandY0 = 0, bandY1 = 0;
    brmi::StripeMap stripes{0, 0, 0, 0};
    uint32_t frameHeight() const { return stripes.count > 1u ? stripes.fullHeight : cfg.height; }
    float bandPlaneTop[3] = {0, 0, 0}, bandPlaneBottom[3] = {0, 0, 0};
    uint64_t bandFirstPixel = 0, bandPixelCount = 0;
    uint32_t maxLevels = 1;
    brmi::SceneTables tables;
    bool holdEnabled = false;
    bool holdThisFrame = false;
    uint32_t holdMinClusters = 16384;
    uint32_t lateDirectMax = 128;
    uint32_t holdFloor = 512;
    uint32_t holdStillMax = 8;
    uint32_t holdMaxTexels = 8;
    uint32_t retestMaxTexels = 8;
    uint32_t chainStripLo = 0xFFFFFFFFu, chainStripHi = 0u;
    uint32_t wideCapacity = 16384;
    uint32_t wideEntries = 128;
    uint32_t leanMinClusters = 32768, leanMaxGeneralPct = 40, leanGrid = 24576, leanEmitGrid = 4096, leanWideEntries = 16, leanQueue = 1u << 20;
    bool leanActive = false, leanLastLaunch = false; uint32_t leanRetryIn = 0;
    uint32_t wideMinTriangles = 4;
    bool chainBuiltInRaster = false;
    std::vector<float> sliceStartHost; float sliceKey[3] = {0, 0, 0}; uint32_t sliceKeyN[2] = {0, 0};
    uint32_t* phase2FeedbackHost = nullptr; uint32_t* phase2FeedbackDev = nullptr;
    bool ensureFeedback() {
        if (phase2FeedbackHost) return true;
        if (hipHostMalloc(reinterpret_cast<void**>(&phase2FeedbackHost), 64, hipHostMallocMapped) != hipSuccess) { phase2FeedbackHost = nullptr; return false; }
        phase2FeedbackHost[0] = 0xFFFFFFFFu; phase2FeedbackHost[1] = 0u;
        for (int k = 2; k < 16; k++) phase2FeedbackHost[k] = 0u;
        if (hipHostGetDevicePointer(reinterpret_cast<void**>(&phase2FeedbackDev), phase2FeedbackHost, 0) != hipSuccess) { (void)hipHostFree(phase2FeedbackHost); phase2FeedbackHost = nullptr; phase2FeedbackDev = nullptr; return false; }
        return true;
    }
    uint32_t phase2DirectMax = 128;
    static constexpr uint32_t clearRiderBlocks = 8192;
    bool splitFrame = false;
    uint32_t shadeSlabs = 0; brmi_slab_fn shadeSlabFn = nullptr; void* shadeSlabUser = nullptr;
    bool frameWaitsIssued = false;
    uint32_t flatLevelsMinDraws = 16384;
    uint32_t scanEpoch = 0;
    bool packedFlat = true;
    static constexpr uint32_t shadeGridShared = 10240;
    static constexpr uint32_t gbufferGridShared = 4096;
    bool shadeSharesChip = false;
    bool lightGridDone = false;
    bool clearVisibilityWithClusterCull = false;
    bool clearFrameStateWithConstants = false, clearVisibilityWithTraversal = false;
    bool seedInHzbTail = false, phase2Seeded = false;
    bool fuseFrameClear = false, frameStateCleared = false;
    bool forceLevelKernels = false;
    uint32_t totalWords = 0, scanBlocks = 0;
    uint32_t numLightClusters = 0, lightPagePool = 0;
    uint32_t binOverflowPerStripe = 1u << 14;
    uint32_t binMinSlice = 1024, binSharedSlice = 512, binGrid = 1024;
    uint32_t binScratchTiles = 2048, binItemCapacity = 0;
    uint32_t binsX = 0, binsY = 0, binCapacity = 16384;
    uint32_t deferredStripeCapacity = 0;
    uint32_t resolveCapacity = 0;
    static constexpr uint32_t rasterGrid = 8192;
    int bigTriAreaDense = 32; uint32_t denseClusterCount = 6144;
    int bigTriArea = 32, bigTriAreaAlpha = 32;
    uint32_t hzbMipCount = 0; std::vector<uint64_t> hzbMipOffsets; std::vector<uint32_t> hzbMipW, hzbMipH;
    bool hzbValid = false;
    brmi_pass* history = nullptr;
    hipEvent_t chainReady = nullptr;
    bool chainRecorded = false;
    brmi_stream chainStream = nullptr;
    hipEvent_t cullDone = nullptr;
    hipEvent_t geometryDone = nullptr, frameDone = nullptr;
    bool frameDoneRecorded = false;
    std::vector<brmi_pass*> historyUsers;
    bool layerPlanesDirty = false;
    bool layerPlanesUniform = false;
    bool chainDirtyTracked = false;
    int resolveInlineMode = -1;
    bool inlineResolve = false;
    bool resolveSetupDone = false;
    bool depthFinal = false;
    const brmi_pass* chainOwner(uint32_t phase) const { return (phase == 1 && history) ? history : this; }
    brmi::HzbDesc hzbDesc() const;
    brmi::Workspace ws{};
    struct { bool on = false; brmi_streaming_buffers b{}; uint32_t groupCount = 0, activeGroupScanCount = 0; } streaming;
    struct { bool on = false; brmi_debug_view_buffers b{}; } debugView;
    struct { bool on = false; brmi_environment_buffers b{}; } env;
    const uint32_t* samplerAniso = nullptr;
    brmi_camera camHost{};
    brmi_per_frame pfHost{};
    std::vector<float> planesHost;
    static constexpr uint32_t kEventRing = 32;
    hipEvent_t evStart[BRMI_STAGE_COUNT][kEventRing] = {}, evStop[BRMI_STAGE_COUNT][kEventRing] = {};
    uint32_t evCount[BRMI_STAGE_COUNT] = {};
    uint32_t executesSinceTimes = 0;
    uint32_t updateSerial = 1, constantsSerial = 0;
    uint32_t shadeSerial = 0;
    bool eventsCreated = false;
    uint32_t timedStages = 0xFFFFFFFFu;
    std::string err;

    template <typename T> T* wsPtr(uint64_t off) const { return reinterpret_cast<T*>(static_cast<uint8_t*>(res[BRMI_RES_WORKSPACE]) + off); }
    uint32_t* counters() const { return wsPtr<uint32_t>(ws.counters); }
};

namespace brmi {

int fail(brmi_pass* p, int code, const char* fmt, ...);
long tuning(const char* key, long def);
#define BRMI_HIP(p, call) do { hipError_t e_ = (call); if (e_ != hipSuccess) return brmi::fail((p), BRMI_ERR_HIP, "%s: %s", #call, hipGetErrorString(e_)); } while (0)
#define BRMI_LAUNCH_CHECK(p, what) do { hipError_t e_ = hipGetLastError(); if (e_ != hipSuccess) return brmi::fail((p), BRMI_ERR_HIP, "launch %s: %s", (what), hipGetErrorString(e_)); } while (0)

int ensure_frame_constants(brmi_pass* p, hipStream_t s);
brmi_scene_buffers shading_scene_of(const brmi_pass* p);
ShadeTables shade_tables_of(const brmi_pass* p);
int launch_clear(brmi_pass* p, hipStream_t s);
int launch_cull(brmi_pass* p, uint32_t phase, hipStream_t s);
int launch_raster(brmi_pass* p, uint32_t phase, hipStream_t s);
int launch_depth_copy(brmi_pass* p, hipStream_t s);
int launch_hzb(brmi_pass* p, hipStream_t s, bool fromVisibility, bool onlyIfPhase2Drew);
int launch_gbuffer(brmi_pass* p, hipStream_t s);
int launch_resolve_setup(brmi_pass* p, hipStream_t s, uint32_t part);
uint32_t resolve_inline_ratio(const brmi_pass* p);
bool resolve_inline_frame(brmi_pass* p);
int launch_light_clustering(brmi_pass* p, hipStream_t s);
int launch_expand_luts(brmi_pass* p, hipStream_t s);
int launch_meshlet_boxes(brmi_pass* p, hipStream_t s);
int launch_shade(brmi_pass* p, hipStream_t s);
int launch_streaming_feedback(brmi_pass* p, hipStream_t s);
bool debug_view_mode_built(uint32_t mode);
int launch_debug_view(brmi_pass* p, hipStream_t s);
int launch_debug_sample_grad(const brmi_scene_buffers& sc, const uint32_t* maxAnisotropy, uint32_t textureIndex, uint32_t samplerIndex, bool uniformBinding, const float* uv, const float* ddx, const float* ddy,
                             float* outRGBA, uint32_t n, hipStream_t s);
int launch_debug_ibl_lookup(const brmi_environment_buffers& env, uint32_t cubemap, const float* dirs, const float* lods, float* outRGBA, uint32_t n, hipStream_t s);
int launch_debug_ibl(brmi_pass* p, const brmi_environment_buffers& env, uint32_t environmentIndex, const float* normals, const uint32_t* albedo, const uint32_t* metallicRoughness, const uint64_t* coat,
                     const uint64_t* emissive, const uint64_t* fuzz, const float* viewWS, float* outDiffuse, float* outSpecular, uint32_t n, hipStream_t s);
int launch_skybox(brmi_pass* p, hipStream_t s);
int launch_env_convert(const brmi_texture_desc* equirect, const brmi_texture_desc* cube, uint32_t size, hipStream_t s);
int launch_env_project_sh(const brmi_texture_desc* cubemaps, uint32_t cubemapCount, brmi_environment_info* env, uint32_t size, hipStream_t s);
int launch_env_prefilter(const brmi_texture_desc* source, const brmi_texture_desc* prefiltered, uint32_t size, uint32_t levels, hipStream_t s);
int launch_debug_env_lookup(const brmi_texture_desc* cubemaps, uint32_t cubemapCount, uint32_t cubemap, const float* dirs, const float* lods, float* outRGBA, uint32_t n, hipStream_t s);
inline StreamArgs stream_args_of(const brmi_pass* p) {
    if (!p->streaming.on) return StreamArgs{nullptr, nullptr, nullptr, 0u, 0u};
    const StreamScratchLayout l = stream_scratch_layout(p->streaming.groupCount);
    uint8_t* scratch = static_cast<uint8_t*>(p->streaming.b.scratch);
    return StreamArgs{p->streaming.b.nonResidentBits, reinterpret_cast<uint32_t*>(scratch + l.touchedBits), reinterpret_cast<unsigned long long*>(scratch + l.requestKeys), p->streaming.activeGroupScanCount, p->streaming.groupCount};
}

}
#endif
```

Baseline: 18200 Mpixels/s.

## Split visibility-buffer clear into slices carried by multiple culling-chain kernels

Replaces the single-carrier visibility clear (either the traversal or the cluster-cull kernel) with a handout that divides the clear's pairs among the traversal, cluster cull, chained scan and scatter launches by configurable weights. Carriers that do not run pass their share on, and scatter takes whatever remains. The default weights still put the whole clear on cluster cull when streams are split and on traversal for a single stream. The intent is to hide the clear's memory traffic behind more of the culling chain, at the cost of extra blocks in each launch, more kernel template variants and more complex bookkeeping.

Result: no change. 18190 Mpixels/s (-0.1%).

```diff
diff --git a/basicrenderer_amd/csrc/brmi_api.hip b/basicrenderer_amd/csrc/brmi_api.hip
--- a/basicrenderer_amd/csrc/brmi_api.hip
+++ b/basicrenderer_amd/csrc/brmi_api.hip
@@ -257,6 +257,9 @@
     p->binSharedSlice = (uint32_t)std::max(32l, tuning("bin_shared_slice", p->binSharedSlice));
     p->binGrid = (uint32_t)std::min(65535l, std::max(1l, tuning("bin_grid", p->binGrid)));
     p->binOverflowPerStripe = (uint32_t)std::max(0l, tuning("bin_overflow", p->binOverflowPerStripe));
+    p->localRankWords = (uint32_t)std::max(0l, std::min(0xFFFFFFFFl, tuning("local_rank_words", 0xFFFFFFFFl)));
+    p->scanChainBlocks = (uint32_t)std::max(0l, std::min(64l, tuning("scan_chain_blocks", p->scanChainBlocks)));
+    if (parse_clear_slices(std::getenv("BRMI_TUNING"), p->clear.weights)) std::memcpy(p->clear.weightsOneStream, p->clear.weights, sizeof p->clear.weights);
     p->binCapacity = (uint32_t)std::min(65536l, std::max(1l, tuning("bin_capacity", p->binCapacity)));
     if (const long v = tuning("big_tri_area", 0)) p->bigTriArea = p->bigTriAreaAlpha = p->bigTriAreaDense = (int)std::max(1l, v);
     compute_sizes(p);
@@ -675,21 +678,19 @@
     p->resolveSetupDone = false; p->depthFinal = false;
     if ((rc = wait_for_frames_in_flight(p, stream))) return rc;
     p->frameWaitsIssued = true;
-    const bool rides = p->constantsSerial != p->updateSerial && p->tables.minLevelWidth <= 1024u  && !p->forceLevelKernels && p->scene.activeDrawCount != 0u;
+    const bool rides = p->constantsSerial != p->updateSerial && p->tables.minLevelWidth <= 1024u  && (p->bandPixelCount & 1ull) == 0ull;
     p->lightGridDone = false;
-    const bool sideRiders = rides && split && (p->bandPixelCount & 1ull) == 0ull;
-    if (sideRiders) {
-        p->clearFrameStateWithConstants = true; p->clearVisibilityWithClusterCull = true;
+    const bool sideRiders = rides && split;
+    if (rides) {
+        p->clearFrameStateWithConstants = true; p->lightGridWithTraversal = !split;
+        p->clear.begin(p->bandPixelCount >> 1, !split);
         rc = brmi_cull(p, 1, stream);
-        p->clearFrameStateWithConstants = false;
-        if (rc == BRMI_OK && p->clearVisibilityWithClusterCull) { p->clearVisibilityWithClusterCull = false; return brmi::fail(p, BRMI_ERR_STATE, "brmi_execute: the cluster culling did not carry the visibility clear"); }
-        if (rc) { p->clearVisibilityWithClusterCull = false; return rc; }
-    } else if (rides) {
-        p->clearFrameStateWithConstants = true; p->clearVisibilityWithTraversal = true;
-        rc = brmi_cull(p, 1, stream);
-        p->clearFrameStateWithConstants = false;
-        if (rc == BRMI_OK && p->clearVisibilityWithTraversal) { p->clearVisibilityWithTraversal = false; return brmi::fail(p, BRMI_ERR_STATE, "brmi_execute: the traversal did not carry the visibility clear"); }
-        if (rc) { p->clearVisibilityWithTraversal = false; return rc; }
+        p->clearFrameStateWithConstants = false; p->lightGridWithTraversal = false;
+        const bool whole = p->clear.done();
+        const unsigned long long handed = p->clear.nextPair;
+        p->clear.end();
+        if (rc) return rc;
+        if (!whole) return brmi::fail(p, BRMI_ERR_STATE, "brmi_execute: the culling chain's launches carried %llu of the visibility clear's %llu pairs", handed, (unsigned long long)(p->bandPixelCount >> 1));
     } else {
     p->fuseFrameClear = true;
     rc = brmi_clear_visibility(p, stream);
diff --git a/basicrenderer_amd/csrc/brmi_clear_slices.h b/basicrenderer_amd/csrc/brmi_clear_slices.h
--- /dev/null
+++ b/basicrenderer_amd/csrc/brmi_clear_slices.h
@@ -0,0 +1,75 @@
+#ifndef BRMI_CLEAR_SLICES_H
+#define BRMI_CLEAR_SLICES_H
+
+#include <cstdint>
+#include <cstdlib>
+#include <cstring>
+
+namespace brmi {
+
+enum ClearCarrier : int { CLEAR_ON_TRAVERSAL = 0, CLEAR_ON_CLUSTER_CULL, CLEAR_ON_SCAN, CLEAR_ON_SCATTER, CLEAR_CARRIERS };
+
+struct ClearSlice { uint64_t firstPair, pairCount; uint32_t blocks; };
+
+struct ClearHandout {
+    uint32_t weights[CLEAR_CARRIERS] = {0, 64, 0, 0};
+    uint32_t weightsOneStream[CLEAR_CARRIERS] = {64, 0, 0, 0};
+    uint64_t totalPairs = 0, nextPair = 0, owed = 0;
+    uint64_t share[CLEAR_CARRIERS] = {0, 0, 0, 0};
+    bool active = false;
+
+    void begin(uint64_t pairs, bool oneStream = false) {
+        const uint32_t* weights = oneStream ? this->weightsOneStream : this->weights;
+        totalPairs = pairs; nextPair = 0; owed = 0; active = true;
+        int last = -1;
+        for (int c = 0; c < CLEAR_CARRIERS; c++) if (weights[c] != 0u) last = c;
+        uint64_t left = pairs;
+        for (int c = 0; c < CLEAR_CARRIERS; c++) {
+            const uint32_t w = weights[c] > 64u ? 64u : weights[c];
+            uint64_t n = c == last ? left : (pairs / 64u) * w + ((pairs % 64u) * w) / 64u;
+            if (n > left) n = left;
+            share[c] = n; left -= n;
+        }
+    }
+    void skip(int carrier) { owed += share[carrier]; share[carrier] = 0; }
+    ClearSlice take(int carrier, uint32_t fullBlocks) {
+        uint64_t n = share[carrier] + owed;
+        if (carrier == CLEAR_ON_SCATTER) n = totalPairs - nextPair;
+        share[carrier] = 0; owed = 0;
+        ClearSlice s{nextPair, n, 0u};
+        if (n != 0u) {
+            const uint64_t b = (n * fullBlocks + totalPairs - 1u) / totalPairs;
+            s.blocks = (uint32_t)(b < 1u ? 1u : b);
+        }
+        nextPair += n;
+        return s;
+    }
+    bool done() const { return nextPair == totalPairs; }
+    void end() { active = false; totalPairs = nextPair = owed = 0; for (int c = 0; c < CLEAR_CARRIERS; c++) share[c] = 0; }
+};
+
+inline bool parse_clear_slices(const char* tuningText, uint32_t out[CLEAR_CARRIERS]) {
+    if (!tuningText) return false;
+    static const char key[] = "clear_slices=";
+    const size_t n = sizeof(key) - 1;
+    for (const char* q = tuningText; (q = std::strstr(q, key)) != nullptr; q += n) {
+        if (q != tuningText && q[-1] != ',' && q[-1] != ' ') continue;
+        const char* v = q + n;
+        uint32_t w[CLEAR_CARRIERS];
+        bool ok = true;
+        for (int c = 0; c < CLEAR_CARRIERS && ok; c++) {
+            if (*v < '0' || *v > '9') { ok = false; break; }
+            char* end = nullptr;
+            const unsigned long x = std::strtoul(v, &end, 10);
+            if (x > 64ul) { ok = false; break; }
+            w[c] = (uint32_t)x; v = end;
+            if (c + 1 < CLEAR_CARRIERS) { if (*v != ',') ok = false; else v++; }
+        }
+        if (ok && (*v == '\0' || *v == ',' || *v == ' ')) { for (int c = 0; c < CLEAR_CARRIERS; c++) out[c] = w[c]; return true; }
+        return false;
+    }
+    return false;
+}
+
+}
+#endif
diff --git a/basicrenderer_amd/csrc/brmi_cull.hip b/basicrenderer_amd/csrc/brmi_cull.hip
--- a/basicrenderer_amd/csrc/brmi_cull.hip
+++ b/basicrenderer_amd/csrc/brmi_cull.hip
@@ -229,10 +229,17 @@
 #endif
 constexpr uint32_t HIER_CAP_MAX = 1024;
 struct NoSide {};
-struct SideJobs { ulonglong2* vis2; uint64_t n2; uint32_t walkBlocks, clearBlocks; ClusterArgs lc; };
+struct SliceClear { ulonglong2* vis2; uint64_t firstPair, pairCount; uint32_t blocks; };
+BRMI_DEV void slice_clear(const SliceClear& c, uint32_t block, uint32_t threads, uint32_t t) {
+    ulonglong2* dst = c.vis2 + c.firstPair;
+    const uint64_t stride = (uint64_t)c.blocks * threads;
+    for (uint64_t i = (uint64_t)block * threads + t; i < c.pairCount; i += stride) dst[i] = make_ulonglong2(BRMI_VIS_EMPTY, BRMI_VIS_EMPTY);
+}
+struct SideJobs { SliceClear clear; uint32_t walkBlocks; ClusterArgs lc; };
 constexpr uint32_t FLAT_WIDE_MAX = 8192;
 struct LcRide { uint32_t mainBlocks; ClusterArgs lc; };
-struct ClearRide { uint32_t mainBlocks; ulonglong2* vis2; uint64_t n2; uint32_t clearBlocks; };
+struct ClearRide { uint32_t mainBlocks; SliceClear clear; };
+struct LcClearRide { uint32_t mainBlocks, lcBlocks; ClusterArgs lc; SliceClear clear; };
 
 BRMI_DEV float4 skinned_meshlet_bounds(const brmi_scene_buffers& sc, const brmi_meshlet_descriptor* desc, const brmi_page_header* hdr, const uint8_t* page, uint32_t slot, float4 staticBounds) {
     const uint32_t boneCount = desc->boneCount;
@@ -398,12 +405,8 @@
     uint32_t walkBlocks = gridDim.x;
     if constexpr (SIDE) {
         walkBlocks = sj.walkBlocks;
-        if (blockIdx.x >= sj.walkBlocks + sj.clearBlocks) { lc_count_wave(sj.lc, blockIdx.x - sj.walkBlocks - sj.clearBlocks, threadIdx.x); return; }
-        if (blockIdx.x >= sj.walkBlocks) {
-            const uint64_t stride = (uint64_t)sj.clearBlocks * 64u;
-            for (uint64_t i = (uint64_t)(blockIdx.x - sj.walkBlocks) * 64u + threadIdx.x; i < sj.n2; i += stride) sj.vis2[i] = make_ulonglong2(BRMI_VIS_EMPTY, BRMI_VIS_EMPTY);
-            return;
-        }
+        if (blockIdx.x >= sj.walkBlocks + sj.clear.blocks) { lc_count_wave(sj.lc, blockIdx.x - sj.walkBlocks - sj.clear.blocks, threadIdx.x); return; }
+        if (blockIdx.x >= sj.walkBlocks) { slice_clear(sj.clear, blockIdx.x - sj.walkBlocks, 64u, threadIdx.x); return; }
     }
     __shared__ uint32_t frontier[2][HIER_CAP];
     __shared__ uint32_t counts[2];
@@ -1075,7 +1078,7 @@
 
 template <int SIDE, typename Residency>
 __global__ void __launch_bounds__(256) k_cull_clusters(CullArgs a, const BucketRecord* buckets, TempVisible* temp, uint32_t* bitmask, uint8_t* blockDirty,
-                                                       typename std::conditional<SIDE == 1, LcRide, typename std::conditional<SIDE == 2, ClearRide, NoSide>::type>::type ride, Residency res) {
+                                                       typename std::conditional<SIDE == 1, LcRide, typename std::conditional<SIDE == 2, ClearRide, typename std::conditional<SIDE == 3, LcClearRide, NoSide>::type>::type>::type ride, Residency res) {
     uint32_t mainBlocks = gridDim.x;
     if constexpr (SIDE == 1) {
         mainBlocks = ride.mainBlocks;
@@ -1083,11 +1086,12 @@
     }
     if constexpr (SIDE == 2) {
         mainBlocks = ride.mainBlocks;
-        if (blockIdx.x >= ride.mainBlocks) {
-            const uint64_t stride = (uint64_t)ride.clearBlocks * 256u;
-            for (uint64_t i = (uint64_t)(blockIdx.x - ride.mainBlocks) * 256u + threadIdx.x; i < ride.n2; i += stride) ride.vis2[i] = make_ulonglong2(BRMI_VIS_EMPTY, BRMI_VIS_EMPTY);
-            return;
-        }
+        if (blockIdx.x >= ride.mainBlocks) { slice_clear(ride.clear, blockIdx.x - ride.mainBlocks, 256u, threadIdx.x); return; }
+    }
+    if constexpr (SIDE == 3) {
+        mainBlocks = ride.mainBlocks;
+        if (blockIdx.x >= ride.mainBlocks + ride.lcBlocks) { slice_clear(ride.clear, blockIdx.x - ride.mainBlocks - ride.lcBlocks, 256u, threadIdx.x); return; }
+        if (blockIdx.x >= ride.mainBlocks) { lc_fill_block(ride.lc, blockIdx.x - ride.mainBlocks, threadIdx.x); return; }
     }
     const brmi_scene_buffers& sc = a.sc;
     const uint32_t bucketCount = min(a.counters[a.bucketCounter], a.recordCapacity);
@@ -1255,7 +1259,9 @@
 
 constexpr uint32_t SCAN_CHAIN_BLOCKS = 64;
 __global__ void __launch_bounds__(256) k_scan_chained(const uint32_t* bitmask, uint32_t totalWords, unsigned long long* agg, uint32_t epoch, uint32_t* wordPrefix,
-                                                     uint32_t* counters, uint32_t outIndex, uint32_t capacity, uint32_t usedIndex, uint32_t* hostFeedback) {
+                                                     uint32_t* counters, uint32_t outIndex, uint32_t capacity, uint32_t usedIndex, uint32_t* hostFeedback, SliceClear clear) {
+    const uint32_t scanBlocks = gridDim.x - clear.blocks;
+    if (blockIdx.x >= scanBlocks) { slice_clear(clear, blockIdx.x - scanBlocks, 256u, threadIdx.x); return; }
     __shared__ uint32_t waveTotals[4];
     __shared__ uint32_t blockPrefix, ticket;
     if (threadIdx.x == 0) ticket = (uint32_t)__hip_atomic_fetch_add(&agg[SCAN_CHAIN_BLOCKS], 1ull, __ATOMIC_RELAXED, __HIP_MEMORY_SCOPE_AGENT);
@@ -1288,7 +1294,7 @@
     uint32_t run = blockPrefix + waveBase + incl - sum;
 #pragma unroll
     for (uint32_t k = 0; k < 8u; k++) { const uint32_t w = base + k; if (w < totalWords) wordPrefix[w] = run; run += pc[k]; }
-    if (block == gridDim.x - 1u && threadIdx.x == 0) {
+    if (block == scanBlocks - 1u && threadIdx.x == 0) {
         __hip_atomic_store(&agg[SCAN_CHAIN_BLOCKS], 0ull, __ATOMIC_RELAXED, __HIP_MEMORY_SCOPE_AGENT);
         const uint32_t placed = min(blockPrefix + blockSum, capacity - (usedIndex == 0xFFFFFFFFu ? 0u : min(counters[usedIndex], capacity)));
         counters[outIndex] = placed;
@@ -1308,7 +1314,9 @@
 template <bool LOCAL_RANK, bool HOLD>
 __global__ void __launch_bounds__(256) k_scatter_visible(const TempVisible* temp, uint32_t* counters, uint32_t tempCountIndex, const uint32_t* bitmask,
                                                         const uint32_t* wordPrefix, uint4* visible, uint32_t baseIndexCounter, uint32_t capacity, uint32_t visibleCapacity,
-                                                        brmi_scene_buffers sc, ClusterSetup* setup, uint32_t resolveCapacity, ClusterUv* clusterUv, LocalRank lr, DrawLists dl) {
+                                                        brmi_scene_buffers sc, ClusterSetup* setup, uint32_t resolveCapacity, ClusterUv* clusterUv, LocalRank lr, DrawLists dl, SliceClear clear) {
+    const uint32_t ownBlocks = gridDim.x - clear.blocks;
+    if (blockIdx.x >= ownBlocks) { slice_clear(clear, blockIdx.x - ownBlocks, 256u, threadIdx.x); return; }
     const uint8_t* const* slabs = sc.slabs;
     const uint32_t n = min(counters[tempCountIndex], visibleCapacity);
     const uint32_t base = baseIndexCounter == 0xFFFFFFFFu ? 0u : counters[baseIndexCounter];
@@ -1342,7 +1350,7 @@
     unsigned long long drawnVT = 0ull;
     if (blockIdx.x == 0u && threadIdx.x == 0u) { const uint32_t room = base < capacity ? capacity - base : 0u; atomicAdd(&counters[CNT_RASTER_CLUSTERS], min(n, room)); if (resolveCapacity == 0u && n != 0u) atomicOr(&counters[CNT_RESOLVE_SPILL], 1u); }
     const uint32_t rounded256 = (n + 255u) & ~255u;
-    for (uint32_t i = blockIdx.x * blockDim.x + threadIdx.x; i < rounded256; i += gridDim.x * blockDim.x) {
+    for (uint32_t i = blockIdx.x * blockDim.x + threadIdx.x; i < rounded256; i += ownBlocks * blockDim.x) {
         uint32_t verts = 0, tris = 0, placed = 0, dst = 0;
         TempVisible t{};
         const uint8_t* slab = nullptr; uint32_t pageOff = 0;
@@ -1499,6 +1507,13 @@
     const uint32_t maxBlocks = 1024;
     bool lightGridRides = false;
     bool flatLevels = false;
+    const bool slices = phase == 1 && p->clear.active;
+    ulonglong2* const visBand = reinterpret_cast<ulonglong2*>(static_cast<unsigned long long*>(p->res[BRMI_RES_VISIBILITY]) + p->bandFirstPixel);
+    auto slice_for = [&](int carrier, uint32_t fullBlocks) {
+        if (!slices) return SliceClear{nullptr, 0ull, 0ull, 0u};
+        const ClearSlice c = p->clear.take(carrier, fullBlocks);
+        return SliceClear{visBand, c.firstPair, c.pairCount, c.blocks};
+    };
     const bool hierarchy = p->tables.minLevelWidth <= HIER_CAP_MAX && !p->forceLevelKernels;
     const bool levelKernels = p->tables.maxLevelWidth > p->tables.spillWidth || p->forceLevelKernels;
     const uint32_t* meshWidth = p->wsPtr<uint32_t>(p->ws.meshLevelWidth);
@@ -1515,10 +1530,7 @@
         const uint32_t draws = p->scene.activeDrawCount, minDraws = std::max(1u, p->flatLevelsMinDraws);
         flatLevels = hierarchy && p->tables.allMeshesFlat && !p->forceLevelKernels && (draws >= minDraws || (p->splitFrame && p->tables.maxLevelWidth > 256u && draws >= std::max(1u, minDraws / 4u)));
         if (flatLevels) {
-            if (p->clearVisibilityWithTraversal && (p->bandPixelCount & 1ull) == 0ull) { p->clearVisibilityWithTraversal = false; p->clearVisibilityWithClusterCull = true; }
-            else if (p->clearVisibilityWithTraversal) flatLevels = false;
-        }
-        if (flatLevels) {
+            p->lightGridWithTraversal = false;
             with_residency([&](auto res) { hipLaunchKernelGGL((k_cull_flat_level<true, decltype(res)>), dim3(grid_for(p->scene.activeDrawCount, 256, 8192)), dim3(256), 0, s, a, 0u, (const NodeRecord*)nullptr, fb, buckets, res); });
             for (uint32_t level = 1; level < p->tables.flatMaxDepth; level++)
                 with_residency([&](auto res) { hipLaunchKernelGGL((k_cull_flat_level<false, decltype(res)>), dim3(2048), dim3(256), 0, s, a, level, (const NodeRecord*)((level & 1u) ? fb : fa), (level & 1u) ? fa : fb, buckets, res); });
@@ -1528,18 +1540,20 @@
         if (hierarchy && !flatLevels) {
             const bool wide = p->tables.maxLevelWidth > 256u;
             const uint32_t widthHi = spillMode ? widthAll : (wide ? HIER_CAP_MAX : 256u);
-            if (p->clearVisibilityWithTraversal) {
-                SideJobs sj{reinterpret_cast<ulonglong2*>(static_cast<unsigned long long*>(p->res[BRMI_RES_VISIBILITY]) + p->bandFirstPixel), p->bandPixelCount >> 1, hgrid.x, p->clearRiderBlocks, cluster_args_of(p)};
-                const dim3 grid(hgrid.x + sj.clearBlocks + p->numLightClusters);
+            const SliceClear walkSlice = slice_for(CLEAR_ON_TRAVERSAL, p->clearRiderBlocks);
+            if (p->lightGridWithTraversal || walkSlice.blocks != 0u) {
+                SideJobs sj{walkSlice, hgrid.x, cluster_args_of(p)};
+                const dim3 grid(hgrid.x + walkSlice.blocks + (p->lightGridWithTraversal ? p->numLightClusters : 0u));
                 if (wide) with_residency([&](auto res) { hipLaunchKernelGGL((k_cull_hierarchy<false, 1024, BRMI_HIER_STAGE_WIDE, true, decltype(res)>), grid, dim3(64), 0, s, a, buckets, meshWidth, 0u, widthHi, spillAbove, fa, sj, res); });
                 else with_residency([&](auto res) { hipLaunchKernelGGL((k_cull_hierarchy<false, 256, 128, true, decltype(res)>), grid, dim3(64), 0, s, a, buckets, meshWidth, 0u, widthHi, spillAbove, fa, sj, res); });
-                p->clearVisibilityWithTraversal = false; lightGridRides = true;
+                lightGridRides = p->lightGridWithTraversal; p->lightGridWithTraversal = false;
             } else if (wide) with_residency([&](auto res) { hipLaunchKernelGGL((k_cull_hierarchy<false, 1024, BRMI_HIER_STAGE_WIDE, false, decltype(res)>), hgrid, dim3(64), 0, s, a, buckets, meshWidth, 0u, widthHi, spillAbove, fa, NoSide{}, res); });
             else with_residency([&](auto res) { hipLaunchKernelGGL((k_cull_hierarchy<false, 256, 128, false, decltype(res)>), hgrid, dim3(64), 0, s, a, buckets, meshWidth, 0u, widthHi, spillAbove, fa, NoSide{}, res); });
         }
         if (a.wideFlat && !flatLevels) with_residency([&](auto res) { hipLaunchKernelGGL((k_cull_flat_wide<decltype(res)>), dim3(std::min(std::max(1u, p->scene.activeDrawCount), 4096u)), dim3(1024), 0, s, a, buckets, res); });
         if (levelKernels && !spillMode && !flatLevels) hipLaunchKernelGGL(k_cull_instances, dim3(grid_for(p->scene.activeDrawCount, 256, maxBlocks)), dim3(256), 0, s, a, fa);
         BRMI_LAUNCH_CHECK(p, "k_cull_instances");
+        if (slices && !(hierarchy && !flatLevels)) p->clear.skip(CLEAR_ON_TRAVERSAL);
     } else {
         if (!p->phase2Seeded) hipLaunchKernelGGL(k_seed_phase2, dim3(1), dim3(128), 0, s, p->counters(), a.recordCapacity);
         p->phase2Seeded = false;
@@ -1562,26 +1576,31 @@
         smallGrid = std::max(smallGrid, grid_for((uint64_t)std::min<uint32_t>(lastBuckets, p->cfg.maxTraversalRecords) * f, 256, 8192));
         scatterGrid = std::max(scatterGrid, grid_for(std::min<uint32_t>(lastVisible, p->cfg.maxVisibleClusters), 256, 8192));
     }
+    const uint32_t clearBlocks = 2048;
+    const SliceClear clusterSlice = slice_for(CLEAR_ON_CLUSTER_CULL, clearBlocks);
     if (lightGridRides) {
-        with_residency([&](auto res) { hipLaunchKernelGGL((k_cull_clusters<1, decltype(res)>), dim3(smallGrid + (p->numLightClusters + 3u) / 4u), dim3(256), 0, s, a, (const BucketRecord*)buckets, temp, bitmask, blockDirty, LcRide{smallGrid, cluster_args_of(p)}, res); });
+        const uint32_t lcBlocks = (p->numLightClusters + 3u) / 4u;
+        if (clusterSlice.blocks != 0u) with_residency([&](auto res) { hipLaunchKernelGGL((k_cull_clusters<3, decltype(res)>), dim3(smallGrid + lcBlocks + clusterSlice.blocks), dim3(256), 0, s, a, (const BucketRecord*)buckets, temp, bitmask, blockDirty, LcClearRide{smallGrid, lcBlocks, cluster_args_of(p), clusterSlice}, res); });
+        else with_residency([&](auto res) { hipLaunchKernelGGL((k_cull_clusters<1, decltype(res)>), dim3(smallGrid + lcBlocks), dim3(256), 0, s, a, (const BucketRecord*)buckets, temp, bitmask, blockDirty, LcRide{smallGrid, cluster_args_of(p)}, res); });
         p->lightGridDone = true;
-    } else if (phase == 1 && p->clearVisibilityWithClusterCull) {
-        const uint32_t clearBlocks = 2048;
-        with_residency([&](auto res) { hipLaunchKernelGGL((k_cull_clusters<2, decltype(res)>), dim3(smallGrid + clearBlocks), dim3(256), 0, s, a, (const BucketRecord*)buckets, temp, bitmask, blockDirty, ClearRide{smallGrid, reinterpret_cast<ulonglong2*>(static_cast<unsigned long long*>(p->res[BRMI_RES_VISIBILITY]) + p->bandFirstPixel), p->bandPixelCount >> 1, clearBlocks}, res); });
-        p->clearVisibilityWithClusterCull = false;
+    } else if (clusterSlice.blocks != 0u) {
+        with_residency([&](auto res) { hipLaunchKernelGGL((k_cull_clusters<2, decltype(res)>), dim3(smallGrid + clusterSlice.blocks), dim3(256), 0, s, a, (const BucketRecord*)buckets, temp, bitmask, blockDirty, ClearRide{smallGrid, clusterSlice}, res); });
     } else with_residency([&](auto res) { hipLaunchKernelGGL((k_cull_clusters<0, decltype(res)>), dim3(smallGrid), dim3(256), 0, s, a, (const BucketRecord*)buckets, temp, bitmask, blockDirty, NoSide{}, res); });
     BRMI_LAUNCH_CHECK(p, "k_cull_clusters");
     const uint32_t outIndex = phase == 1 ? CNT_VISIBLE : CNT_VISIBLE2, usedIndex = phase == 1 ? 0xFFFFFFFFu : (uint32_t)CNT_VISIBLE;
     if (phase == 2 && p->phase2DirectMax != 0u) (void)p->ensureFeedback();
     uint32_t* feedback = phase == 2 ? p->phase2FeedbackDev : (p->phase2FeedbackDev ? p->phase2FeedbackDev + 3 : nullptr);
-    const bool localRank = p->totalWords <= LOCAL_RANK_WORDS && !p->forceLevelKernels;
+    const bool localRank = p->totalWords <= std::min(p->localRankWords, LOCAL_RANK_WORDS) && !p->forceLevelKernels;
     if (localRank) {
+        if (slices) p->clear.skip(CLEAR_ON_SCAN);
     } else {
-        if (p->scanBlocks <= SCAN_CHAIN_BLOCKS) {
+        if (p->scanBlocks <= std::min(p->scanChainBlocks, SCAN_CHAIN_BLOCKS)) {
             if (++p->scanEpoch == 0u) p->scanEpoch = 1u;
-            hipLaunchKernelGGL(k_scan_chained, dim3(p->scanBlocks), dim3(256), 0, s, bitmask, p->totalWords, p->wsPtr<unsigned long long>(p->ws.scanAgg), p->scanEpoch, wordPrefix,
-                               p->counters(), outIndex, p->cfg.maxVisibleClusters, usedIndex, feedback);
+            const SliceClear scanSlice = slice_for(CLEAR_ON_SCAN, clearBlocks);
+            hipLaunchKernelGGL(k_scan_chained, dim3(p->scanBlocks + scanSlice.blocks), dim3(256), 0, s, bitmask, p->totalWords, p->wsPtr<unsigned long long>(p->ws.scanAgg), p->scanEpoch, wordPrefix,
+                               p->counters(), outIndex, p->cfg.maxVisibleClusters, usedIndex, feedback, scanSlice);
         } else {
+            if (slices) p->clear.skip(CLEAR_ON_SCAN);
             hipLaunchKernelGGL(k_scan_reduce, dim3(p->scanBlocks), dim3(256), 0, s, bitmask, p->totalWords, blockSums, blockDirty);
             hipLaunchKernelGGL(k_scan_blocks, dim3(1), dim3(1024), 0, s, blockSums, p->scanBlocks, p->counters(), outIndex, p->cfg.maxVisibleClusters, usedIndex, feedback);
             hipLaunchKernelGGL(k_scan_words, dim3(p->scanBlocks), dim3(256), 0, s, bitmask, p->totalWords, blockSums, wordPrefix, blockDirty);
@@ -1589,13 +1608,14 @@
     }
     if (phase == 1) p->inlineResolve = resolve_inline_frame(p);
     const uint32_t arenaCapacity = p->inlineResolve ? 0u : p->resolveCapacity;
+    const SliceClear scatterSlice = slice_for(CLEAR_ON_SCATTER, clearBlocks);
     auto scatter = [&](auto kernel) {
-        hipLaunchKernelGGL(kernel, dim3(scatterGrid), dim3(256), 0, s, temp, p->counters(), (uint32_t)(phase == 1 ? CNT_TEMP_VISIBLE : CNT_TEMP_VISIBLE2), bitmask, wordPrefix,
+        hipLaunchKernelGGL(kernel, dim3(scatterGrid + scatterSlice.blocks), dim3(256), 0, s, temp, p->counters(), (uint32_t)(phase == 1 ? CNT_TEMP_VISIBLE : CNT_TEMP_VISIBLE2), bitmask, wordPrefix,
                            static_cast<uint4*>(p->res[BRMI_RES_VISIBLE_CLUSTERS]), phase == 1 ? 0xFFFFFFFFu : (uint32_t)CNT_VISIBLE, p->cfg.maxVisibleClusters, p->cfg.maxVisibleClusters, p->scene, p->wsPtr<ClusterSetup>(p->ws.clusterSetup), arenaCapacity,
                            (p->tables.hasTextures || p->tables.hasAlphaTest || p->tables.hasVertexColors) ? p->wsPtr<ClusterUv>(p->ws.clusterUv) : nullptr, LocalRank{p->totalWords, outIndex, usedIndex, feedback},
                            (phase == 1 && p->holdThisFrame) ? DrawLists{p->wsPtr<uint32_t>(p->ws.drawList), p->wsPtr<HeldRecord>(p->ws.heldRecords), 0u, p->wsPtr<MeshletBox>(p->ws.meshletBoxes), p->wsPtr<uint32_t>(p->ws.pageBoxBase),
                                                                       p->wsPtr<float>(p->ws.objConst), p->holdMaxTexels, BoxViewport{(float)p->cfg.width, (float)p->cfg.height, 0.0f, 0.0f, 0, (int)p->bandY0, (int)p->cfg.width - 1, (int)p->bandY1 - 1}, a.hzb}
-                                                          : DrawLists{nullptr, nullptr, p->holdThisFrame ? 1u : 0u, nullptr, nullptr, nullptr, 0u, BoxViewport{}, HzbDesc{}});
+                                                          : DrawLists{nullptr, nullptr, p->holdThisFrame ? 1u : 0u, nullptr, nullptr, nullptr, 0u, BoxViewport{}, HzbDesc{}}, scatterSlice);
     };
     const bool holdLists = phase == 1 && p->holdThisFrame;
     if (localRank) { if (holdLists) scatter(k_scatter_visible<true, true>); else scatter(k_scatter_visible<true, false>); }
diff --git a/basicrenderer_amd/csrc/brmi_internal.h b/basicrenderer_amd/csrc/brmi_internal.h
--- a/basicrenderer_amd/csrc/brmi_internal.h
+++ b/basicrenderer_amd/csrc/brmi_internal.h
@@ -7,6 +7,7 @@
 #include <vector>
 
 #include "brmi.h"
+#include "brmi_clear_slices.h"
 #include "brmi_device.h"
 #include "brmi_scene_tables.h"
 
@@ -263,13 +264,16 @@
     bool frameWaitsIssued = false;
     uint32_t flatLevelsMinDraws = 16384;
     uint32_t scanEpoch = 0;
+    uint32_t localRankWords = 0xFFFFFFFFu;
+    uint32_t scanChainBlocks = 64;
     bool packedFlat = true;
     static constexpr uint32_t shadeGridShared = 10240;
     static constexpr uint32_t gbufferGridShared = 4096;
     bool shadeSharesChip = false;
     bool lightGridDone = false;
-    bool clearVisibilityWithClusterCull = false;
-    bool clearFrameStateWithConstants = false, clearVisibilityWithTraversal = false;
+    brmi::ClearHandout clear;
+    bool clearFrameStateWithConstants = false;
+    bool lightGridWithTraversal = false;
     bool seedInHzbTail = false, phase2Seeded = false;
     bool fuseFrameClear = false, frameStateCleared = false;
     bool forceLevelKernels = false;
```
